# kgutjahr/STiL-TTA

Measured on AMD Instinct MI355X. Metric: training samples/sec (labeled+unlabeled) for DVM STiL, higher is better.
Workload: dtype f32; 1 GPU; config_dvm_STiL ResNet-50 + Transformer tabular, B=256/GPU (32 l + 224 u), 224px + 64 cols, K=286, pseudo-label phase, MI dropout on; global_batch=256, parallelism=dp1, precision=fp32-exact MFMA, launch=eager, split_k=True, input=resident in HBM

## Files before the change

### stil_tta_amd/_lib.py

```python
from __future__ import annotations

import ctypes
import os
import re
import subprocess

_HERE = os.path.dirname(os.path.abspath(__file__))
_ROOT = os.path.dirname(_HERE)
HEADER = os.path.join(_ROOT, "include", "stil_hip.h")
TTA_HEADERS = tuple(os.path.join(_ROOT, "include", f"stil_{n}.h") for n in ("tta", "eata", "bnprior", "infomax", "margent", "deyo", "sar"))
MEMORY_HEADERS = (os.path.join(_HERE, "csrc", "stil_bnmemory.h"),)
READ_HEADERS = (os.path.join(_HERE, "csrc", "stil_read.h"),)
CGPL_HEADERS = (os.path.join(_HERE, "csrc", "stil_cgpl.h"),)
SHIFT_HEADERS = (os.path.join(_HERE, "csrc", "stil_shift.h"),)
ROID_HEADERS = (os.path.join(_HERE, "csrc", "stil_roid.h"),)
ROTTA_HEADERS = (os.path.join(_HERE, "csrc", "stil_rotta.h"),)
LAME_HEADERS = (os.path.join(_HERE, "csrc", "stil_lame.h"),)
LIB_PATH = os.environ.get("STIL_LIB_PATH") or os.path.join(_HERE, "lib", "libstil_hip.so")
CSRC = os.path.join(_HERE, "csrc")

_CTYPES = {
    "int": ctypes.c_int, "long": ctypes.c_long, "long long": ctypes.c_longlong,
    "unsigned long long": ctypes.c_ulonglong, "float": ctypes.c_float, "double": ctypes.c_double,
    "size_t": ctypes.c_size_t,
}


def parse_header(path: str = HEADER):
    src = open(path).read()
    src = re.sub(r"/\*.*?\*/", "", src, flags=re.S)
    protos = {}
    for m in re.finditer(r"(const char\*|int|size_t)\s+(stil_\w+)\s*\(([^)]*)\)\s*;", src):
        ret, name, args = m.group(1), m.group(2), m.group(3)
        restype = {"const char*": ctypes.c_char_p, "int": ctypes.c_int, "size_t": ctypes.c_size_t}[ret]
        argl = []
        args = " ".join(args.split())
        if args and args != "void":
            for a in args.split(","):
                a = a.strip()
                if "*" in a:
                    argl.append((ctypes.c_void_p, a.split("*")[-1].strip()))
                else:
                    toks = a.split()
                    ty = " ".join(toks[:-1])
                    argl.append((_CTYPES[ty], toks[-1]))
        protos[name] = (restype, argl)
    return protos


_HOST_HASHED = ("ops.py", "modules.py", "layouts.py", "stil_model.py", "flat.py", "saint.py")


def source_hash() -> str:
    import hashlib
    h = hashlib.sha256()
    for f in sorted(os.listdir(CSRC)):
        if f.endswith((".hip", ".h")):
            h.update(f.encode())
            h.update(open(os.path.join(CSRC, f), "rb").read())
    for f in _HOST_HASHED:
        h.update(f.encode())
        h.update(open(os.path.join(_HERE, f), "rb").read())
    return h.hexdigest()[:12]


def build(force: bool = False) -> str:
    srcs = [os.path.join(CSRC, f) for f in os.listdir(CSRC) if f.endswith((".hip", ".h"))]
    if (not force) and os.path.exists(LIB_PATH) and all(os.path.getmtime(LIB_PATH) >= os.path.getmtime(s) for s in srcs):
        return LIB_PATH
    r = subprocess.run(["make", "-C", CSRC] + (["-B"] if force else []), capture_output=True, text=True)
    if r.returncode != 0 or not os.path.exists(LIB_PATH):
        raise RuntimeError("building libstil_hip.so failed:\n" + r.stdout + r.stderr)
    return LIB_PATH


class _Lib:
    def __init__(self):
        if not os.path.exists(LIB_PATH):
            raise RuntimeError(f"{LIB_PATH} is missing: run `python -c 'import __graft_entry__ as g; g.build()'` "
                               f"(or `make -C {CSRC}`) first; there is no fallback path")
        self._dll = ctypes.CDLL(LIB_PATH)
        self.protos = parse_header()
        for header in TTA_HEADERS + MEMORY_HEADERS + READ_HEADERS + CGPL_HEADERS + SHIFT_HEADERS + ROID_HEADERS + ROTTA_HEADERS + LAME_HEADERS:
            self.protos.update(parse_header(header))
        for name, (restype, argl) in self.protos.items():
            fn = getattr(self._dll, name)
            fn.restype = restype
            fn.argtypes = [t for t, _ in argl]
        self._dll.stil_last_error.restype = ctypes.c_char_p
        self._prof = None
        self._prof_single = True
        self._prof_only = None

    def begin_profile(self, single_stream: bool = True, only=None):
        self._prof = []
        self._prof_single = bool(single_stream)
        self._prof_only = None if only is None else frozenset(only)

    def end_profile(self):
        import torch
        torch.cuda.synchronize()
        out = [(name, s.elapsed_time(e), meta) for name, s, e, meta in self._prof]
        self._prof = None
        return out

    def last_error(self) -> str:
        return (self._dll.stil_last_error() or b"").decode()

    def __getattr__(self, name):
        fn = getattr(self._dll, "stil_" + name)
        restype = self.protos["stil_" + name][0]
        if restype is not ctypes.c_int or name in ("version", "device_count", "gemm_nt_variant", "gemm_nt_tile_rows", "gemm_nt_config", "weight_layout_job_bytes", "weight_layout_job_blocks", "gemm_nt_bstats_ok", "gemm_nt_force_splits", "reduce_job_bytes", "wgrad_splits", "colsum_chunks", "wgrad_force_splits", "attention_config", "wgrad_config", "gemm_nt_panel"):
            return fn

        def call(*args, meta=None):
            prof = self.__dict__.get("_prof")
            if prof is not None and (self._prof_only is None or name in self._prof_only):
                import torch
                s, e = torch.cuda.Event(enable_timing=True), torch.cuda.Event(enable_timing=True)
                s.record()
                rc = fn(*args)
                e.record()
                prof.append((name, s, e, meta))
            else:
                rc = fn(*args)
            if rc != 0:
                raise RuntimeError(f"stil_{name} failed ({rc}): {self.last_error()}")
            return rc

        self.__dict__[name] = call
        return call


_lib = None


def lib() -> _Lib:
    global _lib
    if _lib is None:
        _lib = _Lib()
    return _lib
```

### stil_tta_amd/csrc/bn.hip

```cpp
#include "common.h"

static inline int pick_ctile(int C) {
  if (C % 256 == 0) return 256;
  if (C % 128 == 0) return 128;
  if (C % 64 == 0) return 64;
  return 0;
}

__global__ __launch_bounds__(256) void bn_pilot_kernel(const float* __restrict__ x, float* __restrict__ K, int M, int C) {
  __shared__ float sh[8 * 32];
  const int cl = threadIdx.x & 31, lane = threadIdx.x >> 5;
  const int c = blockIdx.x * 32 + cl;
  const int n = M < 256 ? M : 256;
  const long stride = M / n;
  float s = 0.f;
  if (c < C)
    for (int j = lane; j < n; j += 8) s += x[(long)j * stride * C + c];
  sh[lane * 32 + cl] = s;
  __syncthreads();
  if (lane == 0 && c < C) {
    float t = 0.f;
    for (int l = 0; l < 8; ++l) t += sh[l * 32 + cl];
    K[c] = t / (float)n;
  }
}

__global__ __launch_bounds__(256) void bn_stats_partial_kernel(const float* __restrict__ x, const float* __restrict__ Kp,
                                                                float* __restrict__ part,
                                                                int M, int C, int ctile, int rows_per_chunk) {
  __shared__ float sh[2 * 1024];
  const int tpr = ctile >> 2, rpb = 256 / tpr;
  const int tc = threadIdx.x % tpr, rl = threadIdx.x / tpr;
  const int c = blockIdx.x * ctile + tc * 4;
  const int m0 = blockIdx.y * rows_per_chunk, m1 = min(M, m0 + rows_per_chunk);
  const float4 K = *reinterpret_cast<const float4*>(Kp + c);
  float4 s1 = make_float4(0.f, 0.f, 0.f, 0.f), s2 = s1;
  for (int m = m0 + rl; m < m1; m += rpb) {
    float4 v = *reinterpret_cast<const float4*>(x + (long)m * C + c);
    float d;
    d = v.x - K.x; s1.x += d; s2.x += d * d;
    d = v.y - K.y; s1.y += d; s2.y += d * d;
    d = v.z - K.z; s1.z += d; s2.z += d * d;
    d = v.w - K.w; s1.w += d; s2.w += d * d;
  }
  float* a = sh + rl * ctile + tc * 4;
  float* b = sh + 1024 + rl * ctile + tc * 4;
  a[0] = s1.x; a[1] = s1.y; a[2] = s1.z; a[3] = s1.w;
  b[0] = s2.x; b[1] = s2.y; b[2] = s2.z; b[3] = s2.w;
  __syncthreads();
  if (threadIdx.x < ctile) {
    float t1 = 0.f, t2 = 0.f;
    for (int r = 0; r < rpb; ++r) { t1 += sh[r * ctile + threadIdx.x]; t2 += sh[1024 + r * ctile + threadIdx.x]; }
    const int cc = blockIdx.x * ctile + threadIdx.x;
    const int nch = gridDim.y;
    part[(long)blockIdx.y * C + cc] = t1;
    part[(long)(nch + blockIdx.y) * C + cc] = t2;
  }
}

template <class Finish>
__global__ __launch_bounds__(256) void bn_fwd_final_kernel(const float* __restrict__ Kp, const float* __restrict__ part, int nch, int M,
                                                            int C, const Finish fin) {
  __shared__ float sh[2 * 8 * 32];
  int c;
  float tot[2];
  if (!chunk_reduce<8, 2>(part, nch, C, sh, c, tot)) return;
  fin.chunk(c, C, M, Kp[c], tot[0], tot[1]);
}

__device__ __forceinline__ void bn_chunk_moments(float K, float s1, float s2, int M, float& mean, float& var) {
  const float invM = 1.f / (float)M;
  const float d = s1 * invM;
  mean = K + d;
  var = s2 * invM - d * d;
  var = fmaxf(var, 0.f);
}

__device__ __forceinline__ bool bn_tile_sums3(const float* __restrict__ ts, int t0, int t1, int tile_rows, int M, int C, double* sh,
                                              int& c, double& a, double& b, double& d) {
  const int cl = threadIdx.x & 31, lane = threadIdx.x >> 5;
  c = blockIdx.x * 32 + cl;
  double s1 = 0.0, s2 = 0.0, s3 = 0.0;
  if (c < C)
    for (int t = t0 + lane; t < t1; t += 8) {
      const double n = (double)min(tile_rows, M - t * tile_rows);
      const double m = (double)ts[((long)t * 2) * C + c];
      s1 += n * m; s2 += n * m * m; s3 += (double)ts[((long)t * 2 + 1) * C + c];
    }
  sh[lane * 32 + cl] = s1; sh[256 + lane * 32 + cl] = s2; sh[512 + lane * 32 + cl] = s3;
  __syncthreads();
  if (lane != 0 || c >= C) return false;
  a = 0.0; b = 0.0; d = 0.0;
  for (int l = 0; l < 8; ++l) { a += sh[l * 32 + cl]; b += sh[256 + l * 32 + cl]; d += sh[512 + l * 32 + cl]; }
  return true;
}

__global__ __launch_bounds__(256) void bn_tiles_stage1_kernel(const float* __restrict__ ts, int nt, int tile_rows, int M, int C,
                                                                int tiles_per_split, double* __restrict__ part) {
  __shared__ double sh[3 * 8 * 32];
  const int t0 = blockIdx.y * tiles_per_split;
  int c;
  double a, b, d;
  if (!bn_tile_sums3(ts, t0, min(nt, t0 + tiles_per_split), tile_rows, M, C, sh, c, a, b, d)) return;
  const int nsplit = gridDim.y;
  part[((long)0 * nsplit + blockIdx.y) * C + c] = a;
  part[((long)1 * nsplit + blockIdx.y) * C + c] = b;
  part[((long)2 * nsplit + blockIdx.y) * C + c] = d;
}

template <class Finish>
__global__ __launch_bounds__(256) void bn_tiles_stage2_kernel(const double* __restrict__ part, int nsplit, int M, int C, const Finish fin) {
  const int c = blockIdx.x * blockDim.x + threadIdx.x;
  if (c >= C) return;
  double s1 = 0.0, s2 = 0.0, s3 = 0.0;
  for (int k = 0; k < nsplit; ++k) {
    s1 += part[((long)0 * nsplit + k) * C + c]; s2 += part[((long)1 * nsplit + k) * C + c]; s3 += part[((long)2 * nsplit + k) * C + c];
  }
  fin.tiles(c, C, M, s1, s2, s3);
}

template <class Finish>
__global__ __launch_bounds__(256) void bn_tiles_fused_kernel(const float* __restrict__ ts, int nt, int tile_rows, int M, int C,
                                                              const Finish fin) {
  __shared__ double sh[3 * 8 * 32];
  int c;
  double a, b, d;
  if (!bn_tile_sums3(ts, 0, nt, tile_rows, M, C, sh, c, a, b, d)) return;
  fin.tiles(c, C, M, a, b, d);
}

__device__ __forceinline__ void bn_tile_moments(double s1, double s2, double s3, int M, double& mean, double& var) {
  mean = s1 / (double)M;
  const double m2 = s3 + (s2 - s1 * mean);
  var = m2 / (double)M;
}

struct BnTrainFwd {
  const float *gamma, *beta;
  float *rmean, *rvar;
  long long* nbt;
  float* stats;
  float eps, momentum;
  __device__ __forceinline__ void write(int c, int C, int M, float mean, float var) const {
    const float g = gamma[c], b = beta[c], rm = rmean ? rmean[c] : 0.f, rv = rmean ? rvar[c] : 0.f;
    if (c == 0 && nbt) *nbt += 1;
    const float rstd = 1.f / sqrtf(var + eps);
    const float a = g * rstd;
    stats[c] = mean; stats[C + c] = rstd; stats[2 * C + c] = a; stats[3 * C + c] = b;
    if (rmean) {
      rmean[c] = (1.f - momentum) * rm + momentum * mean;
      const float unb = (M > 1) ? var * ((float)M / (float)(M - 1)) : var;
      rvar[c] = (1.f - momentum) * rv + momentum * unb;
    }
  }
  __device__ __forceinline__ void chunk(int c, int C, int M, float K, float s1, float s2) const {
    float mean, var;
    bn_chunk_moments(K, s1, s2, M, mean, var);
    write(c, C, M, mean, var);
  }
  __device__ __forceinline__ void tiles(int c, int C, int M, double s1, double s2, double s3) const {
    double mean_d, var_d;
    bn_tile_moments(s1, s2, s3, M, mean_d, var_d);
    write(c, C, M, (float)mean_d, fmaxf((float)var_d, 0.f));
  }
};

__global__ void bn_eval_affine_kernel(const float* __restrict__ gamma, const float* __restrict__ beta,
                                      const float* __restrict__ rmean, const float* __restrict__ rvar,
                                      float* __restrict__ ab, int C, float eps) {
  int c = blockIdx.x * blockDim.x + threadIdx.x;
  if (c >= C) return;
  float a = gamma[c] / sqrtf(rvar[c] + eps);
  ab[c] = a; ab[C + c] = beta[c]; ab[2 * C + c] = rmean[c];
}

__global__ __launch_bounds__(256) void bn_apply_kernel(const float* __restrict__ x, const float* __restrict__ stats,
                                                        const float* __restrict__ resid, const float* __restrict__ rstats,
                                                        float* __restrict__ z, long total4, int C, int relu) {
  const float* A = stats + 2 * C;
  const float* B = stats + 3 * C;
  for (long i = (long)blockIdx.x * blockDim.x + threadIdx.x; i < total4; i += (long)gridDim.x * blockDim.x) {
    const int c = (int)((i * 4) % C);
    float4 v = reinterpret_cast<const float4*>(x)[i];
    const float4 a = *reinterpret_cast<const float4*>(A + c);
    const float4 b = *reinterpret_cast<const float4*>(B + c);
    const float4 mu = *reinterpret_cast<const float4*>(stats + c);
    v.x = (v.x - mu.x) * a.x + b.x; v.y = (v.y - mu.y) * a.y + b.y; v.z = (v.z - mu.z) * a.z + b.z; v.w = (v.w - mu.w) * a.w + b.w;
    if (resid) {
      float4 r = reinterpret_cast<const float4*>(resid)[i];
      if (rstats) {
        const float4 rm = *reinterpret_cast<const float4*>(rstats + c);
        const float4 ra = *reinterpret_cast<const float4*>(rstats + 2 * C + c);
        const float4 rb = *reinterpret_cast<const float4*>(rstats + 3 * C + c);
        r.x = (r.x - rm.x) * ra.x + rb.x; r.y = (r.y - rm.y) * ra.y + rb.y; r.z = (r.z - rm.z) * ra.z + rb.z; r.w = (r.w - rm.w) * ra.w + rb.w;
      }
      v.x += r.x; v.y += r.y; v.z += r.z; v.w += r.w;
    }
    if (relu) { v.x = fmaxf(v.x, 0.f); v.y = fmaxf(v.y, 0.f); v.z = fmaxf(v.z, 0.f); v.w = fmaxf(v.w, 0.f); }
    reinterpret_cast<float4*>(z)[i] = v;
  }
}

__global__ __launch_bounds__(256) void bn_bwd_partial_kernel(const float* __restrict__ dz, const float* __restrict__ z,
                                                              const float* __restrict__ x, const float* __restrict__ stats,
                                                              float* __restrict__ gout, float* __restrict__ part, int M,
                                                              int C, int ctile, int rows_per_chunk, int relu) {
  __shared__ float sh[2 * 1024];
  const int tpr = ctile >> 2, rpb = 256 / tpr;
  const int tc = threadIdx.x % tpr, rl = threadIdx.x / tpr;
  const int c = blockIdx.x * ctile + tc * 4;
  const int m0 = blockIdx.y * rows_per_chunk, m1 = min(M, m0 + rows_per_chunk);
  const float4 mu = *reinterpret_cast<const float4*>(stats + c);
  const float4 rs = *reinterpret_cast<const float4*>(stats + C + c);
  const float4 ap = *reinterpret_cast<const float4*>(stats + 2 * C + c);
  const float4 bp = *reinterpret_cast<const float4*>(stats + 3 * C + c);
  float4 s1 = make_float4(0.f, 0.f, 0.f, 0.f), s2 = s1;
  for (int m = m0 + rl; m < m1; m += rpb) {
    const long o = (long)m * C + c;
    float4 g = *reinterpret_cast<const float4*>(dz + o);
    const float4 v = *reinterpret_cast<const float4*>(x + o);
    if (relu == 1) {
      const float4 zz = *reinterpret_cast<const float4*>(z + o);
      g.x = zz.x > 0.f ? g.x : 0.f; g.y = zz.y > 0.f ? g.y : 0.f;
      g.z = zz.z > 0.f ? g.z : 0.f; g.w = zz.w > 0.f ? g.w : 0.f;
    } else if (relu == 2) {
      g.x = ((v.x - mu.x) * ap.x + bp.x) > 0.f ? g.x : 0.f; g.y = ((v.y - mu.y) * ap.y + bp.y) > 0.f ? g.y : 0.f;
      g.z = ((v.z - mu.z) * ap.z + bp.z) > 0.f ? g.z : 0.f; g.w = ((v.w - mu.w) * ap.w + bp.w) > 0.f ? g.w : 0.f;
    }
    if (gout) *reinterpret_cast<float4*>(gout + o) = g;
    s1.x += g.x; s2.x += g.x * ((v.x - mu.x) * rs.x);
    s1.y += g.y; s2.y += g.y * ((v.y - mu.y) * rs.y);
    s1.z += g.z; s2.z += g.z * ((v.z - mu.z) * rs.z);
    s1.w += g.w; s2.w += g.w * ((v.w - mu.w) * rs.w);
  }
  float* a = sh + rl * ctile + tc * 4;
  float* b = sh + 1024 + rl * ctile + tc * 4;
  a[0] = s1.x; a[1] = s1.y; a[2] = s1.z; a[3] = s1.w;
  b[0] = s2.x; b[1] = s2.y; b[2] = s2.z; b[3] = s2.w;
  __syncthreads();
  if (threadIdx.x < ctile) {
    float t1 = 0.f, t2 = 0.f;
    for (int r = 0; r < rpb; ++r) { t1 += sh[r * ctile + threadIdx.x]; t2 += sh[1024 + r * ctile + threadIdx.x]; }
    const int cc = blockIdx.x * ctile + threadIdx.x;
    const int nch = gridDim.y;
    part[(long)blockIdx.y * C + cc] = t1;
    part[(long)(nch + blockIdx.y) * C + cc] = t2;
  }
}

template <class Finish>
__global__ __launch_bounds__(256) void bn_bwd_final_kernel(const float* __restrict__ part, int nch, int M, int C, const Finish fin) {
  __shared__ float sh[2 * 8 * 32];
  int c;
  float tot[2];
  if (!chunk_reduce<8, 2>(part, nch, C, sh, c, tot)) return;
  fin(c, C, M, tot[0], tot[1]);
}

template <class Finish>
__global__ __launch_bounds__(256) void bn_bwd_final4_kernel(const float* __restrict__ part, int nch, int M, int C, const Finish fin) {
  __shared__ float4 sh[2 * 32 * 8];
  const int cq = threadIdx.x & 7, lane = threadIdx.x >> 3;
  const int c = (blockIdx.x * 8 + cq) * 4;
  float4 a = make_float4(0.f, 0.f, 0.f, 0.f), b = a;
  if (c < C)
    for (int i = lane; i < nch; i += 32) {
      const float4 u = *reinterpret_cast<const float4*>(part + (long)i * C + c);
      const float4 v = *reinterpret_cast<const float4*>(part + (long)(nch + i) * C + c);
      a.x += u.x; a.y += u.y; a.z += u.z; a.w += u.w;
      b.x += v.x; b.y += v.y; b.z += v.z; b.w += v.w;
    }
  sh[lane * 8 + cq] = a; sh[256 + lane * 8 + cq] = b;
  __syncthreads();
  if (lane != 0 || c >= C) return;
  for (int l = 1; l < 32; ++l) {
    const float4 u = sh[l * 8 + cq], v = sh[256 + l * 8 + cq];
    a.x += u.x; a.y += u.y; a.z += u.z; a.w += u.w;
    b.x += v.x; b.y += v.y; b.z += v.z; b.w += v.w;
  }
  const float s1[4] = {a.x, a.y, a.z, a.w}, s2[4] = {b.x, b.y, b.z, b.w};
#pragma unroll
  for (int j = 0; j < 4; ++j) fin(c + j, C, M, s1[j], s2[j]);
}

__device__ __forceinline__ bool bn_tile_sums2(const float* __restrict__ ts, int t0, int t1, int C, double* sh, int& c, double& a,
                                              double& b) {
  const int cl = threadIdx.x & 31, lane = threadIdx.x >> 5;
  c = blockIdx.x * 32 + cl;
  double s1 = 0.0, s2 = 0.0;
  if (c < C)
    for (int t = t0 + lane; t < t1; t += 8) {
      s1 += (double)ts[((long)t * 2) * C + c];
      s2 += (double)ts[((long)t * 2 + 1) * C + c];
    }
  sh[lane * 32 + cl] = s1; sh[256 + lane * 32 + cl] = s2;
  __syncthreads();
  if (lane != 0 || c >= C) return false;
  a = 0.0; b = 0.0;
  for (int l = 0; l < 8; ++l) { a += sh[l * 32 + cl]; b += sh[256 + l * 32 + cl]; }
  return true;
}

__global__ __launch_bounds__(256) void bn_bwd_tiles_stage1_kernel(const float* __restrict__ ts, int nt, int C, int tiles_per_split,
                                                                   double* __restrict__ part) {
  __shared__ double sh[2 * 8 * 32];
  const int t0 = blockIdx.y * tiles_per_split;
  int c;
  double a, b;
  if (!bn_tile_sums2(ts, t0, min(nt, t0 + tiles_per_split), C, sh, c, a, b)) return;
  const int nsplit = gridDim.y;
  part[((long)0 * nsplit + blockIdx.y) * C + c] = a;
  part[((long)1 * nsplit + blockIdx.y) * C + c] = b;
}

template <class Finish>
__global__ __launch_bounds__(256) void bn_bwd_tiles_final_kernel(const double* __restrict__ part, int nsplit, int M, int C,
                                                                  const Finish fin) {
  const int c = blockIdx.x * blockDim.x + threadIdx.x;
  if (c >= C) return;
  double a = 0.0, b = 0.0;
  for (int k = 0; k < nsplit; ++k) { a += part[((long)0 * nsplit + k) * C + c]; b += part[((long)1 * nsplit + k) * C + c]; }
  fin(c, C, M, (float)a, (float)b);
}

template <class Finish>
__global__ __launch_bounds__(256) void bn_bwd_tiles_fused_kernel(const float* __restrict__ ts, int nt, int M, int C, const Finish fin) {
  __shared__ double sh[2 * 8 * 32];
  int c;
  double a, b;
  if (!bn_tile_sums2(ts, 0, nt, C, sh, c, a, b)) return;
  fin(c, C, M, (float)a, (float)b);
}

struct BnTrainBwd {
  const float *gamma, *stats;
  float *dgamma, *dbeta, *coef;
  int accumulate;
  __device__ __forceinline__ void operator()(int c, int C, int M, float s1, float s2) const {
    const float g = gamma[c], rstd = stats[C + c];
    const float b0 = (accumulate && dbeta) ? dbeta[c] : 0.f, g0 = (accumulate && dgamma) ? dgamma[c] : 0.f;
    if (dbeta) dbeta[c] = accumulate ? b0 + s1 : s1;
    if (dgamma) dgamma[c] = accumulate ? g0 + s2 : s2;
    const float invM = 1.f / (float)M;
    coef[c] = g * rstd;
    coef[C + c] = s1 * invM;
    coef[2 * C + c] = s2 * invM;
  }
};

__global__ __launch_bounds__(256) void bn_bwd_dx_kernel(const float* __restrict__ dz, const float* __restrict__ z,
                                                         const float* __restrict__ x, const float* __restrict__ stats,
                                                         const float* __restrict__ coef, float* __restrict__ dx,
                                                         long total4, int C, int relu) {
  for (long i = (long)blockIdx.x * blockDim.x + threadIdx.x; i < total4; i += (long)gridDim.x * blockDim.x) {
    const int c = (int)((i * 4) % C);
    float4 g = reinterpret_cast<const float4*>(dz)[i];
    const float4 v = reinterpret_cast<const float4*>(x)[i];
    const float4 mu = *reinterpret_cast<const float4*>(stats + c);
    if (relu == 1) {
      const float4 zz = reinterpret_cast<const float4*>(z)[i];
      g.x = zz.x > 0.f ? g.x : 0.f; g.y = zz.y > 0.f ? g.y : 0.f;
      g.z = zz.z > 0.f ? g.z : 0.f; g.w = zz.w > 0.f ? g.w : 0.f;
    } else if (relu == 2) {
      const float4 ap = *reinterpret_cast<const float4*>(stats + 2 * C + c);
      const float4 bp = *reinterpret_cast<const float4*>(stats + 3 * C + c);
      g.x = ((v.x - mu.x) * ap.x + bp.x) > 0.f ? g.x : 0.f; g.y = ((v.y - mu.y) * ap.y + bp.y) > 0.f ? g.y : 0.f;
      g.z = ((v.z - mu.z) * ap.z + bp.z) > 0.f ? g.z : 0.f; g.w = ((v.w - mu.w) * ap.w + bp.w) > 0.f ? g.w : 0.f;
    }
    const float4 rs = *reinterpret_cast<const float4*>(stats + C + c);
    const float4 k1 = *reinterpret_cast<const float4*>(coef + c);
    const float4 k2 = *reinterpret_cast<const float4*>(coef + C + c);
    const float4 k3 = *reinterpret_cast<const float4*>(coef + 2 * C + c);
    float4 o;
    o.x = k1.x * (g.x - k2.x - (v.x - mu.x) * rs.x * k3.x);
    o.y = k1.y * (g.y - k2.y - (v.y - mu.y) * rs.y * k3.y);
    o.z = k1.z * (g.z - k2.z - (v.z - mu.z) * rs.z * k3.z);
    o.w = k1.w * (g.w - k2.w - (v.w - mu.w) * rs.w * k3.w);
    reinterpret_cast<float4*>(dx)[i] = o;
  }
}

__global__ __launch_bounds__(256) void maxpool_fwd_kernel(const float* __restrict__ x, float* __restrict__ y, unsigned char* __restrict__ idx,
                                                           int N, int H, int W, int C, int OH, int OW) {
  const int C4 = C >> 2;
  const long total = (long)N * OH * OW * C4;
  for (long i = (long)blockIdx.x * blockDim.x + threadIdx.x; i < total; i += (long)gridDim.x * blockDim.x) {
    const int c = (int)(i % C4) * 4;
    long t = i / C4;
    const int ox = (int)(t % OW); t /= OW;
    const int oy = (int)(t % OH);
    const int n = (int)(t / OH);
    float4 best = make_float4(-INFINITY, -INFINITY, -INFINITY, -INFINITY);
    const int first = (oy == 0 ? 3 : 0) + (ox == 0 ? 1 : 0);
    int b0 = first, b1 = first, b2 = first, b3 = first;
#pragma unroll
    for (int ky = 0; ky < 3; ++ky) {
      const int iy = oy * 2 - 1 + ky;
      if (iy < 0 || iy >= H) continue;
#pragma unroll
      for (int kx = 0; kx < 3; ++kx) {
        const int ix = ox * 2 - 1 + kx;
        if (ix < 0 || ix >= W) continue;
        const float4 v = *reinterpret_cast<const float4*>(x + ((long)(n * H + iy) * W + ix) * C + c);
        const int tap = ky * 3 + kx;
        if (v.x > best.x || v.x != v.x) { best.x = v.x; b0 = tap; }
        if (v.y > best.y || v.y != v.y) { best.y = v.y; b1 = tap; }
        if (v.z > best.z || v.z != v.z) { best.z = v.z; b2 = tap; }
        if (v.w > best.w || v.w != v.w) { best.w = v.w; b3 = tap; }
      }
    }
    const long o = ((long)(n * OH + oy) * OW + ox) * C + c;
    *reinterpret_cast<float4*>(y + o) = best;
    *reinterpret_cast<uchar4*>(idx + o) = make_uchar4((unsigned char)b0, (unsigned char)b1, (unsigned char)b2, (unsigned char)b3);
  }
}

__global__ __launch_bounds__(256) void maxpool_bwd_kernel(const float* __restrict__ dy, const unsigned char* __restrict__ idx,
                                                           float* __restrict__ dx, int N, int H, int W, int C, int OH, int OW) {
  const int C4 = C >> 2;
  const long total = (long)N * H * W * C4;
  for (long i = (long)blockIdx.x * blockDim.x + threadIdx.x; i < total; i += (long)gridDim.x * blockDim.x) {
    const int c = (int)(i % C4) * 4;
    long t = i / C4;
    const int ix = (int)(t % W); t /= W;
    const int iy = (int)(t % H);
    const int n = (int)(t / H);
    float4 s = make_float4(0.f, 0.f, 0.f, 0.f);
    for (int oy = iy / 2; oy <= (iy + 1) / 2; ++oy) {
      if (oy < 0 || oy >= OH) continue;
      const int ky = iy - (oy * 2 - 1);
      if (ky < 0 || ky > 2) continue;
      for (int ox = ix / 2; ox <= (ix + 1) / 2; ++ox) {
        if (ox < 0 || ox >= OW) continue;
        const int kx = ix - (ox * 2 - 1);
        if (kx < 0 || kx > 2) continue;
        const long o = ((long)(n * OH + oy) * OW + ox) * C + c;
        const uchar4 k = *reinterpret_cast<const uchar4*>(idx + o);
        const float4 g = *reinterpret_cast<const float4*>(dy + o);
        const int tap = ky * 3 + kx;
        if (k.x == tap) s.x += g.x;
        if (k.y == tap) s.y += g.y;
        if (k.z == tap) s.z += g.z;
        if (k.w == tap) s.w += g.w;
      }
    }
    *reinterpret_cast<float4*>(dx + ((long)(n * H + iy) * W + ix) * C + c) = s;
  }
}

__global__ __launch_bounds__(256) void im2col_nchw_kernel(const float* __restrict__ x, float* __restrict__ col, int N, int Cin,
                                                           int H, int W, int OH, int OW, int KH, int KW, int stride, int pad,
                                                           int Kp, int rows_per_block) {
  extern __shared__ int ktab[];
  const int K = Cin * KH * KW, Q = Kp >> 2;
  for (int k = threadIdx.x; k < Kp; k += blockDim.x) {
    int v = -1;
    if (k < K) {
      const int c = k / (KH * KW), r = k - c * KH * KW, ky = r / KW, kx = r - ky * KW;
      v = ((c * KH + ky) << 8) | kx;
    }
    ktab[k] = v;
  }
  __syncthreads();
  const long M = (long)N * OH * OW;
  const long m0 = (long)blockIdx.x * rows_per_block;
  const int quads = rows_per_block * Q;
  for (int i = threadIdx.x; i < quads; i += blockDim.x) {
    const int rr = i / Q, q = i - rr * Q;
    const long m = m0 + rr;
    if (m >= M) break;
    const int ox = (int)(m % OW);
    const long t = m / OW;
    const int oy = (int)(t % OH), n = (int)(t / OH);
    const int iy0 = oy * stride - pad, ix0 = ox * stride - pad;
    float v[4];
#pragma unroll
    for (int j = 0; j < 4; ++j) {
      const int e = ktab[q * 4 + j];
      v[j] = 0.f;
      if (e >= 0) {
        const int cky = e >> 8, kx = e & 255, c = cky / KH, ky = cky - c * KH;
        const int iy = iy0 + ky, ix = ix0 + kx;
        if (iy >= 0 && iy < H && ix >= 0 && ix < W) v[j] = x[((long)(n * Cin + c) * H + iy) * W + ix];
      }
    }
    *reinterpret_cast<float4*>(col + m * Kp + q * 4) = make_float4(v[0], v[1], v[2], v[3]);
  }
}

static inline int bn_chunks(int M, int C, int ctile) {
  int colblocks = C / ctile;
  int want = cdiv(1024, colblocks);
  int maxc = cdiv(M, 64);
  int n = want < maxc ? want : maxc;
  return n < 1 ? 1 : n;
}

extern "C" size_t stil_bn_workspace_bytes(int M, int C) {
  int ct = pick_ctile(C);
  if (!ct) return 0;
  return ((size_t)2 * bn_chunks(M, C, ct) + 1) * C * sizeof(float);
}

static inline int bn_tiles_nsplit(int nt) { return cdiv(nt, 256); }
extern "C" size_t stil_bn_tiles_workspace_bytes(int M, int C, int tile_rows) {
  if (M <= 0 || C <= 0 || tile_rows <= 0) return 0;
  return (size_t)3 * bn_tiles_nsplit(cdiv(M, tile_rows)) * C * sizeof(double);
}
extern "C" size_t stil_bn_bwd_tiles_workspace_bytes(int ntiles, int C) {
  if (ntiles <= 0 || C <= 0) return 0;
  return (size_t)2 * bn_tiles_nsplit(ntiles) * C * sizeof(double);
}

static inline int bn_wide_grid(int M, int C, long* total4) {
  *total4 = (long)M * C / 4;
  const long blocks = (*total4 + 255) / 256;
  return (int)(blocks < 8192 ? blocks : 8192);
}

template <class Finish>
static int bn_fwd_two_pass(const char* who, const Finish& fin, const float* x, const float* resid, float* z, const float* stats, int M,
                           int C, int relu, float* workspace, size_t workspace_bytes, hipStream_t s, bool final_only = false) {
  const int ct = pick_ctile(C);
  STIL_REQUIRE(ct != 0, "%s: C=%d must be a multiple of 64", who, C);
  const int nch = bn_chunks(M, C, ct);
  STIL_REQUIRE(workspace_bytes >= ((size_t)2 * nch + 1) * C * sizeof(float), "%s: workspace too small", who);
  float* pilot = workspace + (size_t)2 * nch * C;
  if (!final_only) {
    hipLaunchKernelGGL(bn_pilot_kernel, dim3(cdiv(C, 32)), dim3(256), 0, s, x, pilot, M, C);
    STIL_LAUNCH_CHECK();
    hipLaunchKernelGGL(bn_stats_partial_kernel, dim3(C / ct, nch), dim3(256), 0, s, x, pilot, workspace, M, C, ct, cdiv(M, nch));
    STIL_LAUNCH_CHECK();
  }
  hipLaunchKernelGGL(bn_fwd_final_kernel<Finish>, dim3(cdiv(C, 32)), dim3(256), 0, s, pilot, workspace, nch, M, C, fin);
  STIL_LAUNCH_CHECK();
  if (final_only) return STIL_OK;
  long total4;
  const int grid = bn_wide_grid(M, C, &total4);
  hipLaunchKernelGGL(bn_apply_kernel, dim3(grid), dim3(256), 0, s, x, stats, resid, (const float*)nullptr, z, total4, C, relu);
  STIL_LAUNCH_CHECK();
  return STIL_OK;
}

template <class Finish>
static int bn_fwd_tiles(const char* who, const Finish& fin, const float* x, const float* tilestats, int tile_rows, const float* resid,
                        const float* resid_stats, float* z, const float* stats, int M, int C, int relu, void* workspace,
                        size_t workspace_bytes, hipStream_t s, bool final_only = false) {
  STIL_REQUIRE(z || !resid, "%s: statistics-only call (z == NULL) cannot take a residual", who);
  STIL_REQUIRE(!resid_stats || resid, "%s: resid_stats without resid", who);
  STIL_REQUIRE(tile_rows > 0 && M > 0 && C > 0 && C % 4 == 0, "%s: bad shape M=%d C=%d tile_rows=%d", who, M, C, tile_rows);
  STIL_REQUIRE(workspace_bytes >= stil_bn_tiles_workspace_bytes(M, C, tile_rows) && ((uintptr_t)workspace % 8) == 0,
               "%s: workspace too small or not 8-byte aligned", who);
  const int nt = cdiv(M, tile_rows), nsplit = bn_tiles_nsplit(nt);
  if (nsplit == 1) {
    hipLaunchKernelGGL(bn_tiles_fused_kernel<Finish>, dim3(cdiv(C, 32)), dim3(256), 0, s, tilestats, nt, tile_rows, M, C, fin);
    STIL_LAUNCH_CHECK();
  } else {
    if (!final_only) {
      hipLaunchKernelGGL(bn_tiles_stage1_kernel, dim3(cdiv(C, 32), nsplit), dim3(256), 0, s, tilestats, nt, tile_rows, M, C,
                         cdiv(nt, nsplit), (double*)workspace);
      STIL_LAUNCH_CHECK();
    }
    hipLaunchKernelGGL(bn_tiles_stage2_kernel<Finish>, dim3(cdiv(C, 256)), dim3(256), 0, s, (const double*)workspace, nsplit, M, C, fin);
    STIL_LAUNCH_CHECK();
  }
  if (!z || final_only) return STIL_OK;
  long total4;
  const int grid = bn_wide_grid(M, C, &total4);
  hipLaunchKernelGGL(bn_apply_kernel, dim3(grid), dim3(256), 0, s, x, stats, resid, resid_stats, z, total4, C, relu);
  STIL_LAUNCH_CHECK();
  return STIL_OK;
}

template <class Finish>
static int bn_bwd_two_pass(const char* who, const Finish& fin, const float* dz, const float* z, const float* x, const float* stats,
                           const float* coef, float* dx, float* gout, int M, int C, int relu, float* workspace, size_t workspace_bytes,
                           hipStream_t s) {
  STIL_REQUIRE(relu >= 0 && relu <= 2 && (relu != 1 || z), "%s: relu must be 0, 1 (needs z) or 2", who);
  const int ct = pick_ctile(C);
  STIL_REQUIRE(ct != 0, "%s: C=%d must be a multiple of 64", who, C);
  const int nch = bn_chunks(M, C, ct);
  STIL_REQUIRE(workspace_bytes >= (size_t)2 * nch * C * sizeof(float), "%s: workspace too small", who);
  hipLaunchKernelGGL(bn_bwd_partial_kernel, dim3(C / ct, nch), dim3(256), 0, s, dz, z, x, stats, gout, workspace, M, C, ct,
                     cdiv(M, nch), relu);
  STIL_LAUNCH_CHECK();
  if (((uintptr_t)workspace % 16) == 0)
    hipLaunchKernelGGL(bn_bwd_final4_kernel<Finish>, dim3(cdiv(C, 32)), dim3(256), 0, s, workspace, nch, M, C, fin);
  else
    hipLaunchKernelGGL(bn_bwd_final_kernel<Finish>, dim3(cdiv(C, 32)), dim3(256), 0, s, workspace, nch, M, C, fin);
  STIL_LAUNCH_CHECK();
  long total4;
  const int grid = bn_wide_grid(M, C, &total4);
  hipLaunchKernelGGL(bn_bwd_dx_kernel, dim3(grid), dim3(256), 0, s, gout ? gout : dz, z, x, stats, coef, dx, total4, C, gout ? 0 : relu);
  STIL_LAUNCH_CHECK();
  return STIL_OK;
}

template <class Finish>
static int bn_bwd_tiles(const char* who, const Finish& fin, const float* dz, const float* z, const float* x, const float* stats,
                        const float* tilestats, int ntiles, const float* coef, float* dx, int M, int C, int relu, void* workspace,
                        size_t workspace_bytes, hipStream_t s) {
  STIL_REQUIRE(relu >= 0 && relu <= 2 && (relu != 1 || z), "%s: relu must be 0, 1 (needs z) or 2", who);
  STIL_REQUIRE(ntiles > 0 && M > 0 && C > 0 && C % 4 == 0, "%s: bad shape M=%d C=%d ntiles=%d", who, M, C, ntiles);
  STIL_REQUIRE(workspace_bytes >= stil_bn_bwd_tiles_workspace_bytes(ntiles, C) && ((uintptr_t)workspace % 8) == 0,
               "%s: workspace too small or not 8-byte aligned", who);
  const int nsplit = bn_tiles_nsplit(ntiles);
  if (nsplit == 1) {
    hipLaunchKernelGGL(bn_bwd_tiles_fused_kernel<Finish>, dim3(cdiv(C, 32)), dim3(256), 0, s, tilestats, ntiles, M, C, fin);
    STIL_LAUNCH_CHECK();
  } else {
    hipLaunchKernelGGL(bn_bwd_tiles_stage1_kernel, dim3(cdiv(C, 32), nsplit), dim3(256), 0, s, tilestats, ntiles, C, cdiv(ntiles, nsplit),
                       (double*)workspace);
    STIL_LAUNCH_CHECK();
    hipLaunchKernelGGL(bn_bwd_tiles_final_kernel<Finish>, dim3(cdiv(C, 256)), dim3(256), 0, s, (const double*)workspace, nsplit, M, C, fin);
    STIL_LAUNCH_CHECK();
  }
  long total4;
  const int grid = bn_wide_grid(M, C, &total4);
  hipLaunchKernelGGL(bn_bwd_dx_kernel, dim3(grid), dim3(256), 0, s, dz, z, x, stats, coef, dx, total4, C, relu);
  STIL_LAUNCH_CHECK();
  return STIL_OK;
}

extern "C" int stil_bn_train_fwd(const float* x, const float* gamma, const float* beta, float* running_mean,
                                 float* running_var, long long* num_batches_tracked, const float* resid, float* z,
                                 float* stats, int M, int C, int relu, float eps, float momentum, float* workspace,
                                 size_t workspace_bytes, void* stream) {
  STIL_REQUIRE(x && gamma && beta && z && stats && workspace, "stil_bn_train_fwd: null pointer");
  const BnTrainFwd fin{gamma, beta, running_mean, running_var, num_batches_tracked, stats, eps, momentum};
  return bn_fwd_two_pass("stil_bn_train_fwd", fin, x, resid, z, stats, M, C, relu, workspace, workspace_bytes, (hipStream_t)stream);
}

extern "C" int stil_bn_eval_affine(const float* gamma, const float* beta, const float* running_mean,
                                   const float* running_var, float* ab, int C, float eps, void* stream) {
  STIL_REQUIRE(gamma && beta && running_mean && running_var && ab, "stil_bn_eval_affine: null pointer");
  hipLaunchKernelGGL(bn_eval_affine_kernel, dim3(cdiv(C, 64)), dim3(64), 0, (hipStream_t)stream, gamma, beta,
                     running_mean, running_var, ab, C, eps);
  STIL_LAUNCH_CHECK();
  return STIL_OK;
}

extern "C" int stil_bn_train_fwd_tiles(const float* x, const float* tilestats, int tile_rows, const float* gamma, const float* beta,
                                       float* running_mean, float* running_var, long long* num_batches_tracked,
                                       const float* resid, const float* resid_stats, float* z, float* stats, int M, int C, int relu,
                                       float eps, float momentum, void* workspace, size_t workspace_bytes, void* stream) {
  STIL_REQUIRE(x && tilestats && gamma && beta && stats && workspace, "stil_bn_train_fwd_tiles: null pointer");
  const BnTrainFwd fin{gamma, beta, running_mean, running_var, num_batches_tracked, stats, eps, momentum};
  return bn_fwd_tiles("stil_bn_train_fwd_tiles", fin, x, tilestats, tile_rows, resid, resid_stats, z, stats, M, C, relu, workspace,
                      workspace_bytes, (hipStream_t)stream);
}

extern "C" int stil_bn_train_bwd(const float* dz, const float* z, const float* x, const float* gamma,
                                 const float* stats, float* dx, float* gout, float* dgamma, float* dbeta, float* coef,
                                 int M, int C, int relu, int accumulate, float* workspace, size_t workspace_bytes,
                                 void* stream) {
  STIL_REQUIRE(dz && x && gamma && stats && dx && coef && workspace, "stil_bn_train_bwd: null pointer");
  const BnTrainBwd fin{gamma, stats, dgamma, dbeta, coef, accumulate};
  return bn_bwd_two_pass("stil_bn_train_bwd", fin, dz, z, x, stats, coef, dx, gout, M, C, relu, workspace, workspace_bytes,
                         (hipStream_t)stream);
}

extern "C" int stil_bn_train_bwd_tiles(const float* dz, const float* z, const float* x, const float* gamma, const float* stats,
                                       const float* tilestats, int ntiles, float* dx, float* dgamma, float* dbeta, float* coef,
                                       int M, int C, int relu, int accumulate, void* workspace, size_t workspace_bytes, void* stream) {
  STIL_REQUIRE(dz && x && gamma && stats && tilestats && dx && coef && workspace, "stil_bn_train_bwd_tiles: null pointer");
  const BnTrainBwd fin{gamma, stats, dgamma, dbeta, coef, accumulate};
  return bn_bwd_tiles("stil_bn_train_bwd_tiles", fin, dz, z, x, stats, tilestats, ntiles, coef, dx, M, C, relu, workspace, workspace_bytes,
                      (hipStream_t)stream);
}

extern "C" int stil_maxpool3x3s2_fwd(const float* x, float* y, unsigned char* idx, int N, int H, int W, int C, int OH,
                                     int OW, void* stream) {
  STIL_REQUIRE(x && y && idx, "stil_maxpool3x3s2_fwd: null pointer");
  STIL_REQUIRE(OH == (H + 2 - 3) / 2 + 1 && OW == (W + 2 - 3) / 2 + 1, "stil_maxpool3x3s2_fwd: bad output dims");
  STIL_REQUIRE(C % 4 == 0, "stil_maxpool3x3s2_fwd: C=%d must be a multiple of 4", C);
  long total = (long)N * OH * OW * C / 4;
  int grid = (int)((total + 255) / 256 < 16384 ? (total + 255) / 256 : 16384);
  hipLaunchKernelGGL(maxpool_fwd_kernel, dim3(grid), dim3(256), 0, (hipStream_t)stream, x, y, idx, N, H, W, C, OH, OW);
  STIL_LAUNCH_CHECK();
  return STIL_OK;
}

extern "C" int stil_maxpool3x3s2_bwd(const float* dy, const unsigned char* idx, float* dx, int N, int H, int W, int C,
                                     int OH, int OW, void* stream) {
  STIL_REQUIRE(dy && idx && dx, "stil_maxpool3x3s2_bwd: null pointer");
  STIL_REQUIRE(C % 4 == 0, "stil_maxpool3x3s2_bwd: C=%d must be a multiple of 4", C);
  long total = (long)N * H * W * C / 4;
  int grid = (int)((total + 255) / 256 < 16384 ? (total + 255) / 256 : 16384);
  hipLaunchKernelGGL(maxpool_bwd_kernel, dim3(grid), dim3(256), 0, (hipStream_t)stream, dy, idx, dx, N, H, W, C, OH, OW);
  STIL_LAUNCH_CHECK();
  return STIL_OK;
}

extern "C" int stil_im2col_nchw(const float* x, float* col, int N, int Cin, int H, int W, int OH, int OW, int KH,
                                int KW, int stride, int pad, int Kp, void* stream) {
  STIL_REQUIRE(x && col && Kp >= Cin * KH * KW, "stil_im2col_nchw: null pointer or Kp too small");
  STIL_REQUIRE(Kp % 4 == 0 && Kp <= 4096 && KW < 256 && ((uintptr_t)col % 16) == 0, "stil_im2col_nchw: Kp=%d must be a multiple of 4 (<= 4096), KW < 256, col 16-byte aligned", Kp);
  const long M = (long)N * OH * OW;
  const int rpb = 32;
  hipLaunchKernelGGL(im2col_nchw_kernel, dim3(cdiv(M, rpb)), dim3(256), Kp * sizeof(int), (hipStream_t)stream, x, col, N, Cin, H, W,
                     OH, OW, KH, KW, stride, pad, Kp, rpb);
  STIL_LAUNCH_CHECK();
  return STIL_OK;
}
```

### stil_tta_amd/csrc/gemm.hip

```cpp
#include "common.h"
#include <type_traits>

typedef float f32x16 __attribute__((ext_vector_type(16)));
typedef __bf16 bf16x8 __attribute__((ext_vector_type(8)));
typedef __bf16 bf16x4 __attribute__((ext_vector_type(4)));

__device__ __forceinline__ void split3(float a, __bf16& a1, __bf16& a2, __bf16& a3) {
  a1 = (__bf16)a;
  const float r1 = a - (float)a1;
  a2 = (__bf16)r1;
  const float r2 = r1 - (float)a2;
  a3 = (__bf16)r2;
}

struct ConvGeom {
  int H, W, C;
  int OH, OW;
  int KH, KW, stride, pad_y, pad_x;
  int mode;
};

struct GemmNTArgs {
  const float* A;
  const float* Bw;
  float* C;
  int M, N, K;
  int lda, ldb, ldc;
  ConvGeom g;
  const float* bias;
  const float* sub;
  const float* scale;
  const float* var;
  float var_eps;
  const float* shift;
  const float* resid;
  int ldr;
  float* pre;
  int act;
  float alpha;
  int vecA, vecB;
  int os, opy, opx, oOH, oOW;
  float* colstats;
  const float* abn;
  const float* rmask;
  int ldm;
  int wide;
  const float* bs_y;
  const float* bs_stats;
  float* bstats;
  int ldbs, bs_relu, bs_tile0;
  int splits;
  float* split_slabs;
  int* split_tickets;
  int panel;
};

__device__ __forceinline__ float4 ld4_guard(const float* p, int nvalid, int vec) {
  float4 v = make_float4(0.f, 0.f, 0.f, 0.f);
  if (nvalid >= 4 && vec) {
    v = *reinterpret_cast<const float4*>(p);
  } else {
    if (nvalid > 0) v.x = p[0];
    if (nvalid > 1) v.y = p[1];
    if (nvalid > 2) v.z = p[2];
    if (nvalid > 3) v.w = p[3];
  }
  return v;
}

__device__ __forceinline__ int xcd_remap(int bid, int nwg) {
  int xcd = bid & 7, q = nwg >> 3, r = nwg & 7;
  return (xcd < r ? xcd * (q + 1) : r * (q + 1) + (xcd - r) * q) + (bid >> 3);
}

__device__ __forceinline__ float4 ld4_sel(const float* p, const float* safe, bool ok) {
  const float4 v = *reinterpret_cast<const float4*>(ok ? p : safe);
  return ok ? v : make_float4(0.f, 0.f, 0.f, 0.f);
}

template <int TM, int TN, bool PLAIN>
__device__ __forceinline__ void gemm_nt_epilogue(const GemmNTArgs& p, f32x16 (&acc)[TM][TN], float* red, int tm, int tn, int wm, int wn,
                                                 int li, int lh) {
  constexpr int BM = 64 * TM, BN = 64 * TN;
  const ConvGeom& g = p.g;
  if (p.colstats) {
    const int rows_valid = min(BM, p.M - tm * BM);
    float mean_t[TN];
#pragma unroll
    for (int j = 0; j < TN; ++j) {
      float sacc = 0.f;
#pragma unroll
      for (int i = 0; i < TM; ++i)
#pragma unroll
        for (int r = 0; r < 16; ++r) {
          const int row_m = tm * BM + wm * TM * 32 + i * 32 + (r & 3) + 8 * (r >> 2) + 4 * lh;
          if (row_m < p.M) sacc += acc[i][j][r] * p.alpha;
        }
      sacc += __shfl_xor(sacc, 32, 64);
      if (lh == 0) red[wm * BN + wn * TN * 32 + j * 32 + li] = sacc;
    }
    __syncthreads();
#pragma unroll
    for (int j = 0; j < TN; ++j) {
      const int cs = wn * TN * 32 + j * 32 + li;
      mean_t[j] = (red[cs] + red[BN + cs]) / (float)rows_valid;
    }
    __syncthreads();
#pragma unroll
    for (int j = 0; j < TN; ++j) {
      float q = 0.f;
#pragma unroll
      for (int i = 0; i < TM; ++i)
#pragma unroll
        for (int r = 0; r < 16; ++r) {
          const int row_m = tm * BM + wm * TM * 32 + i * 32 + (r & 3) + 8 * (r >> 2) + 4 * lh;
          const float d = acc[i][j][r] * p.alpha - mean_t[j];
          if (row_m < p.M) q += d * d;
        }
      q += __shfl_xor(q, 32, 64);
      if (lh == 0) red[wm * BN + wn * TN * 32 + j * 32 + li] = q;
    }
    __syncthreads();
    if (wm == 0 && lh == 0) {
#pragma unroll
      for (int j = 0; j < TN; ++j) {
        const int cs = wn * TN * 32 + j * 32 + li, col = tn * BN + cs;
        if (col < p.N) {
          p.colstats[((long)tm * 2) * p.N + col] = mean_t[j];
          p.colstats[((long)tm * 2 + 1) * p.N + col] = red[cs] + red[BN + cs];
        }
      }
    }
  }

  if constexpr (TM == 1 && TN == 1) {
    if (p.wide) {
      constexpr int TS = BN + 4;
      float* T = red;
      __syncthreads();
#pragma unroll
      for (int r = 0; r < 16; ++r)
        T[(wm * 32 + (r & 3) + 8 * (r >> 2) + 4 * lh) * TS + wn * 32 + li] = acc[0][0][r];
      __syncthreads();
      const int tid = threadIdx.x, cq = (tid & 15) * 4, col = tn * BN + cq;
      if (col < p.N) {
        const float4 zero4 = make_float4(0.f, 0.f, 0.f, 0.f), one4 = make_float4(1.f, 1.f, 1.f, 1.f);
        const float4 bia = p.bias ? *reinterpret_cast<const float4*>(p.bias + col) : zero4;
        const float4 sb = p.sub ? *reinterpret_cast<const float4*>(p.sub + col) : zero4;
        float4 sc = p.scale ? *reinterpret_cast<const float4*>(p.scale + col) : one4;
        if (p.var) {
          const float4 vv = *reinterpret_cast<const float4*>(p.var + col);
          sc.x = sc.x / sqrtf(vv.x + p.var_eps); sc.y = sc.y / sqrtf(vv.y + p.var_eps);
          sc.z = sc.z / sqrtf(vv.z + p.var_eps); sc.w = sc.w / sqrtf(vv.w + p.var_eps);
        }
        const float4 sh = p.shift ? *reinterpret_cast<const float4*>(p.shift + col) : zero4;
#pragma unroll
        for (int ps = 0; ps < 4; ++ps) {
          const int rl = ps * 16 + (tid >> 4), row_m = tm * BM + rl;
          if (row_m >= p.M) continue;
          long row = row_m;
          if (!PLAIN && p.os != 1) {
            const int ohw = g.OH * g.OW;
            const int n = row_m / ohw, rem = row_m - n * ohw;
            const int oy = rem / g.OW, ox = rem - oy * g.OW;
            row = ((long)n * p.oOH + oy * p.os + p.opy) * p.oOW + ox * p.os + p.opx;
          }
          float4 v = *reinterpret_cast<const float4*>(T + rl * TS + cq);
          v.x *= p.alpha; v.y *= p.alpha; v.z *= p.alpha; v.w *= p.alpha;
          v.x = (v.x - sb.x) * sc.x + sh.x + bia.x; v.y = (v.y - sb.y) * sc.y + sh.y + bia.y;
          v.z = (v.z - sb.z) * sc.z + sh.z + bia.z; v.w = (v.w - sb.w) * sc.w + sh.w + bia.w;
          if (p.resid) {
            const float4 rr = *reinterpret_cast<const float4*>(p.resid + row * p.ldr + col);
            v.x += rr.x; v.y += rr.y; v.z += rr.z; v.w += rr.w;
          }
          if (p.pre) *reinterpret_cast<float4*>(p.pre + row * p.ldc + col) = v;
          if (p.act == 1) { v.x = fmaxf(v.x, 0.f); v.y = fmaxf(v.y, 0.f); v.z = fmaxf(v.z, 0.f); v.w = fmaxf(v.w, 0.f); }
          else if (p.act == 2) { v.x = gelu_f(v.x); v.y = gelu_f(v.y); v.z = gelu_f(v.z); v.w = gelu_f(v.w); }
          if (p.rmask) {
            const float4 mk = *reinterpret_cast<const float4*>(p.rmask + row * p.ldm + col);
            v.x = mk.x > 0.f ? v.x : 0.f; v.y = mk.y > 0.f ? v.y : 0.f; v.z = mk.z > 0.f ? v.z : 0.f; v.w = mk.w > 0.f ? v.w : 0.f;
          }
          *reinterpret_cast<float4*>(p.C + row * p.ldc + col) = v;
          if (p.bstats) *reinterpret_cast<float4*>(T + rl * TS + cq) = v;
        }
      }
      if (p.bstats) {
        float4 bs1 = make_float4(0.f, 0.f, 0.f, 0.f), bs2 = bs1;
        if (col < p.N) {
          const float4 bmu = *reinterpret_cast<const float4*>(p.bs_stats + col);
          const float4 brs = *reinterpret_cast<const float4*>(p.bs_stats + p.N + col);
          const float4 bap = *reinterpret_cast<const float4*>(p.bs_stats + 2 * p.N + col);
          const float4 bbp = *reinterpret_cast<const float4*>(p.bs_stats + 3 * p.N + col);
#pragma unroll
          for (int ps = 0; ps < 4; ++ps) {
            const int rl = ps * 16 + (tid >> 4), row_m = tm * BM + rl;
            if (row_m >= p.M) continue;
            long row = row_m;
            if (!PLAIN && p.os != 1) {
              const int ohw = g.OH * g.OW;
              const int n = row_m / ohw, rem = row_m - n * ohw;
              const int oy = rem / g.OW, ox = rem - oy * g.OW;
              row = ((long)n * p.oOH + oy * p.os + p.opy) * p.oOW + ox * p.os + p.opx;
            }
            const float4 yy = *reinterpret_cast<const float4*>(p.bs_y + row * p.ldbs + col);
            float4 gg = *reinterpret_cast<const float4*>(T + rl * TS + cq);
            if (p.bs_relu == 2) {
              gg.x = ((yy.x - bmu.x) * bap.x + bbp.x) > 0.f ? gg.x : 0.f; gg.y = ((yy.y - bmu.y) * bap.y + bbp.y) > 0.f ? gg.y : 0.f;
              gg.z = ((yy.z - bmu.z) * bap.z + bbp.z) > 0.f ? gg.z : 0.f; gg.w = ((yy.w - bmu.w) * bap.w + bbp.w) > 0.f ? gg.w : 0.f;
            }
            bs1.x += gg.x; bs2.x += gg.x * ((yy.x - bmu.x) * brs.x);
            bs1.y += gg.y; bs2.y += gg.y * ((yy.y - bmu.y) * brs.y);
            bs1.z += gg.z; bs2.z += gg.z * ((yy.z - bmu.z) * brs.z);
            bs1.w += gg.w; bs2.w += gg.w * ((yy.w - bmu.w) * brs.w);
          }
        }
        __syncthreads();
        float* R1 = red;
        float* R2 = red + 16 * 64;
        const int rt = tid >> 4;
        *reinterpret_cast<float4*>(R1 + rt * 64 + cq) = bs1;
        *reinterpret_cast<float4*>(R2 + rt * 64 + cq) = bs2;
        __syncthreads();
        if (tid < 128) {
          const int c = tid & 63, which = tid >> 6, gc = tn * BN + c;
          const float* R = which ? R2 : R1;
          float t = 0.f;
#pragma unroll
          for (int r = 0; r < 16; ++r) t += R[r * 64 + c];
          if (gc < p.N) p.bstats[((long)(p.bs_tile0 + tm) * 2 + which) * p.N + gc] = t;
        }
      }
      return;
    }
  }

#pragma unroll
  for (int j = 0; j < TN; ++j) {
    const int col = tn * BN + wn * TN * 32 + j * 32 + li;
    if (col >= p.N) continue;
    const float bia = p.bias ? p.bias[col] : 0.f;
    const float sb = p.sub ? p.sub[col] : 0.f;
    float sc = p.scale ? p.scale[col] : 1.f;
    if (p.var) sc = sc / sqrtf(p.var[col] + p.var_eps);
    const float sh = p.shift ? p.shift[col] : 0.f;
#pragma unroll
    for (int i = 0; i < TM; ++i) {
#pragma unroll
      for (int r = 0; r < 16; ++r) {
        const int row_m = tm * BM + wm * TM * 32 + i * 32 + (r & 3) + 8 * (r >> 2) + 4 * lh;
        if (row_m >= p.M) continue;
        long row = row_m;
        if (!PLAIN && p.os != 1) {
          const int ohw = g.OH * g.OW;
          const int n = row_m / ohw, rem = row_m - n * ohw;
          const int oy = rem / g.OW, ox = rem - oy * g.OW;
          row = ((long)n * p.oOH + oy * p.os + p.opy) * p.oOW + ox * p.os + p.opx;
        }
        float v = acc[i][j][r] * p.alpha;
        v = (v - sb) * sc + sh + bia;
        if (p.resid) v += p.resid[row * p.ldr + col];
        if (p.pre) p.pre[row * p.ldc + col] = v;
        if (p.act == 1) v = fmaxf(v, 0.f);
        else if (p.act == 2) v = gelu_f(v);
        if (p.rmask) v = p.rmask[row * p.ldm + col] > 0.f ? v : 0.f;
        p.C[row * p.ldc + col] = v;
      }
    }
  }
}

template <int TM, int TN, int BK, bool VEC, bool ACC2 = false, bool PLAIN = false, bool BNA = false, int NB = 2, bool B3 = false>
__global__ __launch_bounds__(256) __attribute__((amdgpu_waves_per_eu(B3 ? (PLAIN ? 4 : 3) : (((BK == 16 || NB == 1) && VEC) ? (TM * TN == 1 ? ((NB == 1 && ACC2) ? 4 : ((BNA && ACC2 && !PLAIN) ? 5 : 6)) : ((TM * TN == 2 && ACC2 && (PLAIN || TN == 2)) ? 4 : 1)) : 1))))
void gemm_nt_kernel(GemmNTArgs p) {
  static_assert(!B3 || (BK == 32 && NB == 1 && VEC && ACC2), "the bf16x3 mode runs 32-deep k-tiles in one LDS buffer with two-level sums");
  constexpr int BM = 64 * TM, BN = 64 * TN, LS = BK + 4;
  constexpr int KQ = BK / 4, RP = 256 / KQ;
  constexpr int RA = BM / RP, RB = BN / RP;
  constexpr int LSB = 40;
  extern __shared__ __attribute__((aligned(16))) float lds[];
  float* As = lds;
  float* Bs = lds + NB * BM * LS;
  float* tab = B3 ? lds + 3 * (BM + BN) * LSB / 2 : lds + NB * (BM + BN) * LS;
  __bf16* Ap3 = reinterpret_cast<__bf16*>(lds);
  __bf16* Bp3 = Ap3 + 3 * BM * LSB;

  const int nbn = (p.N + BN - 1) / BN, nbm = (p.M + BM - 1) / BM;
  int wg = xcd_remap(blockIdx.x, nbm * nbn * (TM * TN == 1 ? p.splits : 1));
  int split = 0;
  if constexpr (TM * TN == 1) {
    if (p.splits > 1) { split = wg % p.splits; wg /= p.splits; }
  }
  int tm = wg / nbn, tn = wg - tm * nbn;
  if (p.panel > 0) {
    const int per_panel = nbm * p.panel;
    const int pn = wg / per_panel, rem = wg - pn * per_panel;
    tm = rem / p.panel;
    tn = pn * p.panel + (rem - tm * p.panel);
  }
  const int tid = threadIdx.x, kq = tid % KQ, r0 = tid / KQ;
  const ConvGeom g = p.g;

  int a_n[RA], a_oy[RA], a_ox[RA];
  bool a_ok[RA];
#pragma unroll
  for (int i = 0; i < RA; ++i) {
    int m = tm * BM + r0 + RP * i;
    a_ok[i] = m < p.M;
    if constexpr (PLAIN) {
      a_n[i] = a_ok[i] ? m : 0; a_oy[i] = 0; a_ox[i] = 0;
    } else {
      int mm = a_ok[i] ? m : 0;
      int ohw = g.OH * g.OW;
      int n = mm / ohw, rem = mm - n * ohw;
      int oy = rem / g.OW;
      a_n[i] = n; a_oy[i] = oy; a_ox[i] = rem - oy * g.OW;
    }
  }
  const float* b_ptr[RB];
  bool b_ok[RB];
#pragma unroll
  for (int i = 0; i < RB; ++i) {
    int n = tn * BN + r0 + RP * i;
    b_ok[i] = n < p.N;
    b_ptr[i] = p.Bw + (long)(b_ok[i] ? n : 0) * p.ldb + kq * 4;
  }

  float4 ra[RA], rb[RB];
  const float* a_src[RA];
  bool a_val[RA];
  bool ra_ok[RA];
  int ra_c = 0;
  if constexpr (BNA) {
    const int C = p.g.C;
    for (int i = threadIdx.x; i < 3 * C; i += 256) {
      const int r = i / C, c = i - r * C;
      tab[i] = p.abn[(r == 0 ? 0 : r + 1) * C + c];
    }
    __syncthreads();
  }
  auto set_tap = [&](int tap) {
    if constexpr (PLAIN) {
#pragma unroll
      for (int i = 0; i < RA; ++i) {
        a_val[i] = a_ok[i];
        a_src[i] = p.A + (long)a_n[i] * p.lda + kq * 4;
      }
      return;
    }
    const int ky = tap / g.KW, kx = tap - ky * g.KW;
#pragma unroll
    for (int i = 0; i < RA; ++i) {
      int iy, ix;
      bool ok = a_ok[i];
      if (g.mode == 0) {
        iy = a_oy[i] * g.stride - g.pad_y + ky;
        ix = a_ox[i] * g.stride - g.pad_x + kx;
      } else {
        int ty = a_oy[i] + g.pad_y - ky, tx = a_ox[i] + g.pad_x - kx;
        ok = ok && ty >= 0 && tx >= 0;
        iy = ty / g.stride; ix = tx / g.stride;
        ok = ok && (iy * g.stride == ty) && (ix * g.stride == tx);
      }
      ok = ok && iy >= 0 && iy < g.H && ix >= 0 && ix < g.W;
      a_val[i] = ok;
      a_src[i] = ok ? p.A + ((long)(a_n[i] * g.H + iy) * g.W + ix) * p.lda + kq * 4 : p.A;
    }
  };
  const int per_tap = (g.C + BK - 1) / BK;
  const int nk_all = (PLAIN ? 1 : g.KH * g.KW) * per_tap;
  int kt0 = 0, nk = nk_all;
  if constexpr (TM * TN == 1) {
    if (p.splits > 1) {
      int kpt = (nk_all + p.splits - 1) / p.splits;
      kpt = ((kpt + 64 / BK - 1) / (64 / BK)) * (64 / BK);
      kt0 = min(nk_all, split * kpt);
      nk = min(nk_all, kt0 + kpt) - kt0;
    }
  }
  int cur_tap = kt0 / per_tap, c0 = (kt0 - cur_tap * per_tap) * BK, kb = cur_tap * g.C + c0;
  const int ntaps = PLAIN ? 1 : g.KH * g.KW;
  set_tap(cur_tap < ntaps ? cur_tap : 0);
  auto gload = [&]() {
    const int nval = g.C - (c0 + kq * 4);
    if constexpr (BNA) ra_c = c0 + kq * 4;
#pragma unroll
    for (int i = 0; i < RA; ++i) {
      if (VEC) ra[i] = ld4_sel(a_src[i] + c0, p.A, a_val[i] && nval > 0);
      else ra[i] = a_val[i] ? ld4_guard(a_src[i] + c0, nval, 0) : make_float4(0.f, 0.f, 0.f, 0.f);
      if constexpr (BNA) ra_ok[i] = a_val[i] && nval > 0;
    }
#pragma unroll
    for (int i = 0; i < RB; ++i) {
      if (VEC) rb[i] = ld4_sel(b_ptr[i] + kb, p.Bw, b_ok[i] && nval > 0);
      else rb[i] = b_ok[i] ? ld4_guard(b_ptr[i] + kb, nval, 0) : make_float4(0.f, 0.f, 0.f, 0.f);
    }
    c0 += BK; kb += BK;
    if (c0 >= g.C) {
      kb += g.C - c0;
      c0 = 0;
      if (++cur_tap < ntaps) set_tap(cur_tap);
    }
  };
  auto lstore = [&](int buf) {
    if constexpr (BNA) {
      const int C = p.g.C;
      const float4 mu = *reinterpret_cast<const float4*>(tab + ra_c);
      const float4 aa = *reinterpret_cast<const float4*>(tab + C + ra_c);
      const float4 bb = *reinterpret_cast<const float4*>(tab + 2 * C + ra_c);
#pragma unroll
      for (int i = 0; i < RA; ++i) {
        float4 v = ra[i];
        v.x = (v.x - mu.x) * aa.x + bb.x; v.y = (v.y - mu.y) * aa.y + bb.y; v.z = (v.z - mu.z) * aa.z + bb.z; v.w = (v.w - mu.w) * aa.w + bb.w;
        v.x = fmaxf(v.x, 0.f); v.y = fmaxf(v.y, 0.f); v.z = fmaxf(v.z, 0.f); v.w = fmaxf(v.w, 0.f);
        ra[i] = ra_ok[i] ? v : make_float4(0.f, 0.f, 0.f, 0.f);
      }
    }
    if constexpr (B3) {
#pragma unroll
      for (int i = 0; i < RA + RB; ++i) {
        const float4 v = i < RA ? ra[i < RA ? i : 0] : rb[i < RA ? 0 : i - RA];
        const float e[4] = {v.x, v.y, v.z, v.w};
        bf16x4 h1, h2, h3;
#pragma unroll
        for (int q = 0; q < 4; ++q) { __bf16 a1, a2, a3; split3(e[q], a1, a2, a3); h1[q] = a1; h2[q] = a2; h3[q] = a3; }
        __bf16* dst = (i < RA ? Ap3 + (r0 + RP * i) * LSB : Bp3 + (r0 + RP * (i - RA)) * LSB) + kq * 4;
        constexpr int PLA = BM * LSB, PLB = BN * LSB;
        const int PL = i < RA ? PLA : PLB;
        *reinterpret_cast<bf16x4*>(dst) = h1; *reinterpret_cast<bf16x4*>(dst + PL) = h2; *reinterpret_cast<bf16x4*>(dst + 2 * PL) = h3;
      }
      return;
    }
#pragma unroll
    for (int i = 0; i < RA; ++i)
      *reinterpret_cast<float4*>(&As[buf * BM * LS + (r0 + RP * i) * LS + kq * 4]) = ra[i];
#pragma unroll
    for (int i = 0; i < RB; ++i)
      *reinterpret_cast<float4*>(&Bs[buf * BN * LS + (r0 + RP * i) * LS + kq * 4]) = rb[i];
  };

  const int w = tid >> 6, wm = w >> 1, wn = w & 1, lane = tid & 63, li = lane & 31, lh = lane >> 5;
  f32x16 acc[TM][TN];
#pragma unroll
  for (int i = 0; i < TM; ++i)
#pragma unroll
    for (int j = 0; j < TN; ++j)
#pragma unroll
      for (int r = 0; r < 16; ++r) acc[i][j][r] = 0.f;
  constexpr int FLUSH = 64 / BK;

  const bool tap_inside = PLAIN || (g.pad_y == 0 && g.pad_x == 0 && (g.OH - 1) * g.stride < g.H && (g.OW - 1) * g.stride < g.W);
  const bool full = VEC && ntaps == 1 && (PLAIN || g.mode == 0) && tap_inside && (g.C % BK == 0) && (tm + 1) * BM <= p.M && (tn + 1) * BN <= p.N;
  auto mainloop = [&](auto full_tag) {
    constexpr bool FULL = decltype(full_tag)::value;
    auto load = [&]() {
      if constexpr (FULL) {
        if constexpr (BNA) {
          ra_c = c0 + kq * 4;
#pragma unroll
          for (int i = 0; i < RA; ++i) ra_ok[i] = true;
        }
#pragma unroll
        for (int i = 0; i < RA; ++i) ra[i] = *reinterpret_cast<const float4*>(a_src[i] + c0);
#pragma unroll
        for (int i = 0; i < RB; ++i) rb[i] = *reinterpret_cast<const float4*>(b_ptr[i] + c0);
        c0 += BK;
      } else {
        gload();
      }
    };
    auto compute = [&](int buf, f32x16 (&c)[TM][TN], auto fresh_tag) {
      constexpr bool FRESH = decltype(fresh_tag)::value;
      if constexpr (B3) {
        const __bf16* Ab3 = Ap3 + (wm * TM * 32 + li) * LSB + lh * 8;
        const __bf16* Bb3 = Bp3 + (wn * TN * 32 + li) * LSB + lh * 8;
#pragma unroll
        for (int s_ = 0; s_ < 2; ++s_) {
          bf16x8 a[3][TM], b[3][TN];
#pragma unroll
          for (int pl = 0; pl < 3; ++pl) {
#pragma unroll
            for (int i = 0; i < TM; ++i) a[pl][i] = *reinterpret_cast<const bf16x8*>(Ab3 + pl * BM * LSB + i * 32 * LSB + s_ * 16);
// ... 535 lines not shown
__global__ void wgrad_reduce_kernel(const float* __restrict__ P, float* __restrict__ dW, int splits, int N, int K,
                                    int Cin, int taps, int Kdst, int accumulate) {
  long idx = (long)blockIdx.x * blockDim.x + threadIdx.x;
  long total = (long)N * K;
  if (idx >= total) return;
  int n = (int)(idx / K), k = (int)(idx - (long)n * K);
  float s = 0.f;
  for (int zz = 0; zz < splits; ++zz) s += P[(long)zz * total + idx];
  int dst;
  if (taps > 1) {
    int tap = k / Cin, c = k - tap * Cin;
    dst = c * taps + tap;
  } else {
    dst = k;
  }
  if (dst >= Kdst) return;
  long o = (long)n * Kdst + dst;
  dW[o] = accumulate ? dW[o] + s : s;
}
__global__ __launch_bounds__(256) void wgrad_reduce4_kernel(const float* __restrict__ P, float* __restrict__ dW, int splits, int N, int K,
                                                             int Cin, int taps, int Kdst, int accumulate) {
  __shared__ float4 sh[8 * 32];
  const int ql = threadIdx.x & 31, l = threadIdx.x >> 5;
  const long total = (long)N * K;
  const long idx = ((long)blockIdx.x * 32 + ql) * 4;
  float4 s = make_float4(0.f, 0.f, 0.f, 0.f);
  if (idx < total)
    for (int zz = l; zz < splits; zz += 8) {
      const float4 v = *reinterpret_cast<const float4*>(P + (long)zz * total + idx);
      s.x += v.x; s.y += v.y; s.z += v.z; s.w += v.w;
    }
  sh[l * 32 + ql] = s;
  __syncthreads();
  if (l != 0 || idx >= total) return;
  for (int j = 1; j < 8; ++j) { const float4 v = sh[j * 32 + ql]; s.x += v.x; s.y += v.y; s.z += v.z; s.w += v.w; }
  const int n = (int)(idx / K), k = (int)(idx - (long)n * K);
  const float sv[4] = {s.x, s.y, s.z, s.w};
  if (taps > 1) {
    const int tap = k / Cin, c = k - tap * Cin;
#pragma unroll
    for (int j = 0; j < 4; ++j) {
      const int dst = (c + j) * taps + tap;
      if (dst < Kdst) { const long o = (long)n * Kdst + dst; dW[o] = accumulate ? dW[o] + sv[j] : sv[j]; }
    }
  } else {
#pragma unroll
    for (int j = 0; j < 4; ++j) {
      const int dst = k + j;
      if (dst < Kdst) { const long o = (long)n * Kdst + dst; dW[o] = accumulate ? dW[o] + sv[j] : sv[j]; }
    }
  }
}

__global__ __launch_bounds__(256) void colsum_partial_kernel(const float* __restrict__ X, float* __restrict__ part, int M, int N, int ld,
                                      int rows_per_chunk) {
  __shared__ float sh[4 * 64];
  const int cl = threadIdx.x & 63, rl = threadIdx.x >> 6;
  const int c = blockIdx.x * 64 + cl;
  const int m0 = blockIdx.y * rows_per_chunk, m1 = min(M, m0 + rows_per_chunk);
  float s0 = 0.f, s1 = 0.f;
  if (c < N) {
    int m = m0 + rl;
    for (; m + 4 < m1; m += 8) { s0 += X[(long)m * ld + c]; s1 += X[(long)(m + 4) * ld + c]; }
    for (; m < m1; m += 4) s0 += X[(long)m * ld + c];
  }
  sh[rl * 64 + cl] = s0 + s1;
  __syncthreads();
  if (rl == 0 && c < N) part[(long)blockIdx.y * N + c] = sh[cl] + sh[64 + cl] + sh[128 + cl] + sh[192 + cl];
}
__global__ __launch_bounds__(256) void colsum_final_kernel(const float* __restrict__ part, float* __restrict__ out, int nchunks, int N,
                                    int accumulate, float scale) {
  __shared__ float sh[8 * 32];
  int c;
  float tot[1];
  if (!chunk_reduce<8, 1>(part, nchunks, N, sh, c, tot)) return;
  const float s = tot[0] * scale;
  out[c] = accumulate ? out[c] + s : s;
}

#define STIL_REDUCE_BATCH 48
struct ReduceJob {
  const float* P;
  float* dst;
  int splits, N, K, Cin, taps, Kdst, accumulate;
  float scale;
};
struct ReduceBatch {
  int n;
  int first_block[STIL_REDUCE_BATCH + 1];
  ReduceJob job[STIL_REDUCE_BATCH];
};
static inline bool reduce_job_vec(const ReduceJob& j) {
  return j.K % 4 == 0 && (j.taps == 1 || j.Cin % 4 == 0) && ((uintptr_t)j.P % 16) == 0;
}
static inline int reduce_job_blocks(const ReduceJob& j) {
  const long total = (long)j.N * j.K;
  return reduce_job_vec(j) ? cdiv(total / 4, 256) : cdiv(total, 256);
}
__global__ __launch_bounds__(256) void reduce_jobs_kernel(ReduceBatch b) {
  int ji = 0;
  while (ji + 1 < b.n && (int)blockIdx.x >= b.first_block[ji + 1]) ++ji;
  const ReduceJob& j = b.job[ji];
  const int lb = blockIdx.x - b.first_block[ji];
  const long total = (long)j.N * j.K;
  const bool vec = j.K % 4 == 0 && (j.taps == 1 || j.Cin % 4 == 0) && ((uintptr_t)j.P % 16) == 0;
  if (vec) {
    const long idx = ((long)lb * 256 + threadIdx.x) * 4;
    if (idx >= total) return;
    float4 t[8];
#pragma unroll
    for (int l = 0; l < 8; ++l) t[l] = make_float4(0.f, 0.f, 0.f, 0.f);
    const float* src = j.P + idx;
    int zz = 0;
    for (; zz + 8 <= j.splits; zz += 8) {
#pragma unroll
      for (int l = 0; l < 8; ++l) {
        const float4 v = *reinterpret_cast<const float4*>(src + (long)(zz + l) * total);
        t[l].x += v.x; t[l].y += v.y; t[l].z += v.z; t[l].w += v.w;
      }
    }
#pragma unroll
    for (int l = 0; l < 8; ++l)
      if (zz + l < j.splits) {
        const float4 v = *reinterpret_cast<const float4*>(src + (long)(zz + l) * total);
        t[l].x += v.x; t[l].y += v.y; t[l].z += v.z; t[l].w += v.w;
      }
    float4 s = t[0];
#pragma unroll
    for (int q = 1; q < 8; ++q) { s.x += t[q].x; s.y += t[q].y; s.z += t[q].z; s.w += t[q].w; }
    const int n = (int)(idx / j.K), k = (int)(idx - (long)n * j.K);
    const float sv[4] = {s.x * j.scale, s.y * j.scale, s.z * j.scale, s.w * j.scale};
    if (j.taps == 1 && k + 3 < j.Kdst && j.Kdst % 4 == 0 && ((uintptr_t)j.dst % 16) == 0) {
      float4* o = reinterpret_cast<float4*>(j.dst + (long)n * j.Kdst + k);
      float4 r = make_float4(sv[0], sv[1], sv[2], sv[3]);
      if (j.accumulate) { const float4 c = *o; r.x = c.x + sv[0]; r.y = c.y + sv[1]; r.z = c.z + sv[2]; r.w = c.w + sv[3]; }
      *o = r;
      return;
    }
#pragma unroll
    for (int e = 0; e < 4; ++e) {
      int dst = k + e;
      if (j.taps > 1) { const int tap = k / j.Cin, c = k - tap * j.Cin; dst = (c + e) * j.taps + tap; }
      if (dst < j.Kdst) { const long o = (long)n * j.Kdst + dst; j.dst[o] = j.accumulate ? j.dst[o] + sv[e] : sv[e]; }
    }
  } else {
    const long idx = (long)lb * 256 + threadIdx.x;
    if (idx >= total) return;
    const int n = (int)(idx / j.K), k = (int)(idx - (long)n * j.K);
    float s = 0.f;
    for (int zz = 0; zz < j.splits; ++zz) s += j.P[(long)zz * total + idx];
    s *= j.scale;
    int dst = k;
    if (j.taps > 1) { const int tap = k / j.Cin, c = k - tap * j.Cin; dst = c * j.taps + tap; }
    if (dst >= j.Kdst) return;
    const long o = (long)n * j.Kdst + dst;
    j.dst[o] = j.accumulate ? j.dst[o] + s : s;
  }
}
extern "C" int stil_reduce_job_bytes(void) { return (int)sizeof(ReduceJob); }
extern "C" int stil_reduce_jobs(const void* jobs_host, int njobs, void* stream) {
  STIL_REQUIRE(jobs_host && njobs > 0, "stil_reduce_jobs: null pointer or no jobs");
  const ReduceJob* jobs = (const ReduceJob*)jobs_host;
  for (int j0 = 0; j0 < njobs; j0 += STIL_REDUCE_BATCH) {
    ReduceBatch b;
    b.n = njobs - j0 < STIL_REDUCE_BATCH ? njobs - j0 : STIL_REDUCE_BATCH;
    int nb = 0;
    for (int i = 0; i < b.n; ++i) {
      const ReduceJob& j = jobs[j0 + i];
      STIL_REQUIRE(j.P && j.dst && j.splits > 0 && j.N > 0 && j.K > 0 && j.taps > 0 && (j.taps == 1 || j.Cin * j.taps == j.K),
                   "stil_reduce_jobs: bad job %d", j0 + i);
      b.job[i] = j;
      b.first_block[i] = nb;
      nb += reduce_job_blocks(j);
    }
    for (int i = b.n; i <= STIL_REDUCE_BATCH; ++i) b.first_block[i] = nb;
    hipLaunchKernelGGL(reduce_jobs_kernel, dim3(nb), dim3(256), 0, (hipStream_t)stream, b);
    STIL_LAUNCH_CHECK();
  }
  return STIL_OK;
}

static int check_geom(const ConvGeom& g, int vec_required) {
  if (g.KH * g.KW > 1 && (g.C % 16) != 0) {
    stil_set_error("implicit-GEMM conv needs Cin %% 16 == 0 (got %d)", g.C);
    return STIL_EUNSUPPORTED;
  }
  (void)vec_required;
  return STIL_OK;
}

static inline int is_vec(const void* p, int ld) { return (((uintptr_t)p) % 16 == 0) && (ld % 4 == 0); }

static bool g_nt_attr = false;
static int gemm_nt_attr() {
  if (g_nt_attr) return STIL_OK;
  hipError_t e = hipFuncSetAttribute((const void*)gemm_nt_kernel<2, 2, 32, true, false, false>, hipFuncAttributeMaxDynamicSharedMemorySize, 80 * 1024);
  if (e == hipSuccess) e = hipFuncSetAttribute((const void*)gemm_nt_kernel<2, 2, 32, true, true, false>, hipFuncAttributeMaxDynamicSharedMemorySize, 80 * 1024);
  if (e == hipSuccess) e = hipFuncSetAttribute((const void*)gemm_nt_kernel<2, 2, 32, true, false, true>, hipFuncAttributeMaxDynamicSharedMemorySize, 80 * 1024);
  if (e == hipSuccess) e = hipFuncSetAttribute((const void*)gemm_nt_kernel<2, 2, 32, true, true, true>, hipFuncAttributeMaxDynamicSharedMemorySize, 80 * 1024);
  if (e != hipSuccess) { stil_set_error("gemm_nt: hipFuncSetAttribute failed: %s", hipGetErrorString(e)); return STIL_EHIP; }
  g_nt_attr = true;
  return STIL_OK;
}

static bool nt_big_wanted(int M, int N, int K, bool plain, bool vec, int srcC, int tune) {
  static const int env_big = [] { const char* e = getenv("STIL_GEMM_BIG"); return e ? atoi(e) : 0; }();
  static const int env_mink = [] { const char* e = getenv("STIL_GEMM_BIG_MINK"); return e ? atoi(e) : 0; }();
  const int forced = tune % 100;
  if (forced != 44 && !(forced == 0 && env_big > 0)) return false;
  if (!plain || !vec || (M % 128) || (N % 128) || (K % 32) || srcC != K) return false;
  const long tiles = (long)(M / 128) * (N / 128);
  return forced == 44 || (tiles >= env_big && K >= env_mink);
}

extern "C" int stil_gemm_nt_variant(int M, int N, int tune) {
  tune %= 10000;
  const int forced = tune % 100;
  if (forced == 11 || forced == 21 || forced == 22 || forced == 12) return forced;
  (void)M; (void)N;
  return 11;
}

extern "C" int stil_gemm_nt_bstats_ok(const float* C, int N, int ldc, const float* resid, int ldr, const float* relu_mask, int ldm, const float* bs_y) {
  auto al16 = [](const void* q) { return q == nullptr || ((uintptr_t)q % 16) == 0; };
  return (N % 4 == 0) && (ldc % 4 == 0) && (!resid || ldr % 4 == 0) && (!relu_mask || ldm % 4 == 0) && al16(relu_mask) && al16(C) && al16(resid) &&
         al16(bs_y) && bs_y != nullptr ? 1 : 0;
}

extern "C" int stil_gemm_nt_tile_rows(int M, int N, int tune) { const int v = stil_gemm_nt_variant(M, N, tune); return (v == 11 || v == 12) ? 64 : 128; }

static int nt_config(const float* A, const float* W, int M, int N, int K, int lda, int ldb, int srcC, int KH, int KW,
                     int plain, int a_bn, int tune, bool allow_big) {
  const bool want_b3 = tune >= 100000;
  tune %= 10000;
  const int variant = stil_gemm_nt_variant(M, N, tune);
  const int bkd = (tune / 100) % 10;
  const bool bk32 = (bkd == 1 || bkd == 3 || (bkd == 0 && !a_bn)) && (K % 32 == 0) && (KH * KW == 1 || srcC % 32 == 0);
  const bool single = bk32 && (bkd == 3 || bkd == 0);
  const bool acc2 = tune / 1000 == 2 || (tune / 1000 == 0 && K >= 512);
  const bool vec = is_vec(A, lda) && (srcC % 4 == 0) && is_vec(W, ldb) && (K % 4 == 0);
  if (allow_big && !want_b3 && nt_big_wanted(M, N, K, plain && KH * KW == 1, vec, srcC, tune) && (long)cdiv(M, 64) * cdiv(N, 64) >= 256)
    return 44 + 200 + 1000 * (acc2 ? 1 : 0) + 10000 + 100000 + (a_bn ? 1000000 : 0);
  const bool b3 = want_b3 && vec && variant == 11 && K % 32 == 0 && (KH * KW == 1 || srcC % 32 == 0) && (!a_bn || srcC % 32 == 0);
  if (b3)
    return 11 + 200 + 1000 + 10000 + 100000 * ((plain && KH * KW == 1) ? 1 : 0) + (a_bn ? 1000000 : 0) + 10000000;
  if (a_bn)
    return 11 + 1000 * (acc2 ? 1 : 0) + 10000 * (vec ? 1 : 0) + 100000 * ((plain && KH * KW == 1) ? 1 : 0) + 1000000;
  return variant + 100 * ((vec && bk32) ? (single ? 2 : 1) : 0) + 1000 * (acc2 ? 1 : 0) + 10000 * (vec ? 1 : 0) + 100000 * ((plain && KH * KW == 1) ? 1 : 0);
}

extern "C" int stil_gemm_nt_config(const float* A, const float* W, int M, int N, int K, int lda, int ldb, int srcC, int KH, int KW,
                                   int plain, int a_bn, int tune) {
  return nt_config(A, W, M, N, K, lda, ldb, srcC, KH, KW, plain, a_bn, tune, true);
}

#define NT_SPLIT_MAX_TILES 4096
static int g_force_splits = 0;
extern "C" int stil_gemm_nt_force_splits(int s) { const int old = g_force_splits; g_force_splits = s; return old; }
static int nt_splits(int M, int N, int K, int tune) {
  if (stil_gemm_nt_variant(M, N, tune) != 11) return 1;
  const long tiles = (long)cdiv(M, 64) * cdiv(N, 64);
  if (g_force_splits > 0) {
    if (tiles > NT_SPLIT_MAX_TILES || K < 256) return 1;
    int s = g_force_splits;
    if (s > K / 64) s = K / 64;
    return s < 2 ? 1 : s;
  }
  static const int max_tiles = [] { const char* e = getenv("STIL_GEMM_SPLIT_MAXTILES"); return e ? atoi(e) : 1536; }();
  static const int big_target = [] { const char* e = getenv("STIL_GEMM_SPLIT_TARGET"); return e ? atoi(e) : 1536; }();
  if (K < 256 || tiles >= max_tiles) return 1;
  const int kt = K / 32;
  int maxs, target;
  if (tiles < 256) { maxs = kt / 4; target = kt >= 64 ? 1536 : 512; }
  else { if (kt < 36) return 1; maxs = kt / 12; target = big_target; }
  int s = cdiv(target, tiles);
  if (s > maxs) s = maxs;
  if (s > 8) s = 8;
  return s < 2 ? 1 : s;
}
static int nt_panel(int M, int N, int K) {
  static const int forced = [] { const char* e = getenv("STIL_GEMM_PANEL"); return e ? atoi(e) : -1; }();
  const int nbn = cdiv(N, 64);
  int gw = forced;
  if (forced < 0) {
    if (N < 1024 || K > 1024 || (long)N * K * 4 <= (2l << 20)) return 0;
    gw = (int)((1l << 20) / (64l * K * 4));
    if (gw < 4) gw = 4;
  }
  if (gw <= 0 || gw >= nbn) return 0;
  while (gw > 1 && nbn % gw) --gw;
  (void)M;
  return gw > 1 ? gw : 0;
}
extern "C" int stil_gemm_nt_panel(int M, int N, int K) { return nt_panel(M, N, K); }

#define NT_SPLIT_TICKET_BYTES (4 * NT_SPLIT_MAX_TILES)
extern "C" size_t stil_gemm_nt_split_workspace_bytes(int M, int N, int K, int tune) {
  const int s = nt_splits(M, N, K, tune % 10000);
  if (s <= 1) return 0;
  const long tiles = (long)cdiv(M, 64) * cdiv(N, 64);
  return (size_t)NT_SPLIT_TICKET_BYTES + (size_t)tiles * s * 4096 * sizeof(float);
}

extern "C" int stil_gemm_nt(const float* A, const float* W, float* C, int M, int N, int K, int lda, int ldb, int ldc,
                            int srcH, int srcW, int srcC, int OH, int OW, int KH, int KW, int stride, int pad_y,
                            int pad_x, int mode, int out_stride, int out_py, int out_px, int out_OH, int out_OW,
                            const float* bias, const float* sub, const float* scale,
                            const float* shift, const float* resid, int ldr, float* pre, int act, float alpha,
                            float* colstats, const float* a_bn, const float* relu_mask, int ldm,
                            const float* bs_y, const float* bs_stats, float* bstats, int bs_relu, int bs_tile0,
                            const float* scale_var, float var_eps, void* split_ws, size_t split_ws_bytes, int tune_arg, void* stream) {
  const bool want_b3 = tune_arg >= 100000;
  if (want_b3) tune_arg -= 100000;
  const int tune = tune_arg % 10000;
  const bool scalar_epilogue = tune_arg / 10000 == 1;
  STIL_REQUIRE(A && W && C && M > 0 && N > 0 && K > 0, "stil_gemm_nt: null pointer or empty shape (M=%d N=%d K=%d)", M, N, K);
  STIL_REQUIRE(tune_arg >= 0 && tune_arg < 20000 && tune < 3000 && (tune % 100 == 0 || tune % 100 == 11 || tune % 100 == 21 || tune % 100 == 22 || tune % 100 == 12 || tune % 100 == 44) && (tune / 100) % 10 <= 3,
               "stil_gemm_nt: bad tune %d", tune);
  STIL_REQUIRE(KH * KW * srcC == K, "stil_gemm_nt: K=%d != KH*KW*C=%d", K, KH * KW * srcC);
  STIL_REQUIRE(M % (OH * OW) == 0, "stil_gemm_nt: M=%d not a multiple of OH*OW=%d", M, OH * OW);
  GemmNTArgs p;
  p.A = A; p.Bw = W; p.C = C; p.M = M; p.N = N; p.K = K; p.lda = lda; p.ldb = ldb; p.ldc = ldc;
  p.g = ConvGeom{srcH, srcW, srcC, OH, OW, KH, KW, stride, pad_y, pad_x, mode};
  p.os = out_stride < 1 ? 1 : out_stride; p.opy = out_py; p.opx = out_px; p.oOH = out_OH; p.oOW = out_OW;
  p.var = scale_var; p.var_eps = var_eps;
  p.splits = 1; p.split_slabs = nullptr; p.split_tickets = nullptr;
  p.panel = 0;
  {
    const size_t need = stil_gemm_nt_split_workspace_bytes(M, N, K, tune_arg);
    if (split_ws && need > 0 && split_ws_bytes >= need && ((uintptr_t)split_ws % 256) == 0) {
      const long tiles = (long)cdiv(M, 64) * cdiv(N, 64);
      p.splits = nt_splits(M, N, K, tune_arg % 10000);
      p.split_tickets = (int*)split_ws;
      p.split_slabs = (float*)((char*)split_ws + NT_SPLIT_TICKET_BYTES);
      (void)tiles;
    }
  }
  STIL_REQUIRE(!scale_var || scale, "stil_gemm_nt: scale_var divides `scale`, which is missing");
  p.bias = bias; p.sub = sub; p.scale = scale; p.shift = shift; p.resid = resid; p.ldr = ldr; p.pre = pre; p.act = act;
  p.alpha = alpha;
  p.colstats = colstats;
  p.abn = a_bn;
  p.rmask = relu_mask; p.ldm = ldm;
  STIL_REQUIRE(!relu_mask || !colstats, "stil_gemm_nt: relu_mask and colstats exclude each other");
  {
    auto al16 = [](const void* q) { return q == nullptr || ((uintptr_t)q % 16) == 0; };
    p.wide = (N % 4 == 0) && (ldc % 4 == 0) && (!resid || ldr % 4 == 0) && (!relu_mask || ldm % 4 == 0) && al16(relu_mask) && al16(C) && al16(resid) && al16(pre) && al16(bias) && al16(sub) &&
             al16(scale) && al16(scale_var) && al16(shift) && !scalar_epilogue ? 1 : 0;
  }
  p.bs_y = bs_y; p.bs_stats = bs_stats; p.bstats = bstats; p.ldbs = ldc; p.bs_relu = bs_relu; p.bs_tile0 = bs_tile0;
  STIL_REQUIRE(!bstats || (bs_y && bs_stats && (bs_relu == 0 || bs_relu == 2) && bs_tile0 >= 0 && !colstats && !a_bn && p.wide &&
                           ((uintptr_t)bs_y % 16) == 0 && ((uintptr_t)bs_stats % 16) == 0 && (tune % 100 == 0 || tune % 100 == 11 || tune % 100 == 44)),
               "stil_gemm_nt: bstats needs bs_y / bs_stats, bs_relu 0 or 2, the 16-byte epilogue on 64x64 tiles (stil_gemm_nt_bstats_ok) "
               "and excludes colstats / a_bn");
  STIL_REQUIRE(!colstats || (p.os == 1 && !bias && !sub && !scale && !shift && !resid && act == 0),
               "stil_gemm_nt: colstats describes the raw product (no bias / affine / residual / activation / output map)");
  p.vecA = is_vec(A, lda) && (srcC % 4 == 0);
  p.vecB = is_vec(W, ldb);
  int rc = check_geom(p.g, 0);
  if (rc) return rc;
  hipStream_t s = (hipStream_t)stream;
  const bool plain = KH * KW == 1 && stride == 1 && pad_y == 0 && pad_x == 0 && mode == 0 && p.os == 1 && srcH == OH && srcW == OW;
  const int cfg = nt_config(A, W, M, N, K, lda, ldb, srcC, KH, KW, plain ? 1 : 0, a_bn ? 1 : 0, tune, false);
  const int variant = cfg % 100;
  const bool bk32 = (cfg / 100) % 10 >= 1;
  const bool single = (cfg / 100) % 10 == 2;
  const bool acc2 = (cfg / 1000) % 10 == 1;
  const bool vec = (cfg / 10000) % 10 == 1;
  STIL_REQUIRE(!a_bn || (vec && !bk32 && mode == 0 && srcC % 16 == 0 && srcC <= 2048 && (tune % 100 == 0 || tune % 100 == 11 || tune % 100 == 44)),
               "stil_gemm_nt: a_bn runs 64x64 tiles only (tune %% 100 must be 0 or 11: the caller sizes colstats by "
               "stil_gemm_nt_tile_rows) and needs 16-byte aligned operands, a forward gather, Cin %% 16 == 0 and Cin <= 2048 (Cin=%d)", srcC);
  rc = gemm_nt_attr();
  if (rc) return rc;
  if (variant == 11 && p.splits == 1) p.panel = nt_panel(M, N, K);
  if (!want_b3 && variant == 11 && p.splits == 1 && p.wide && !scalar_epilogue && mode == 0 && (!a_bn || srcC <= 2048) &&
      nt_big_wanted(M, N, K, plain, vec, srcC, tune) && (long)cdiv(M, 64) * cdiv(N, 64) >= 256) {
    p.panel = (p.panel > 0 && p.panel % 2 == 0 && (N / 128) % (p.panel / 2) == 0) ? p.panel / 2 : 0;
    const dim3 grid_((M / 128) * (N / 128));
    const size_t lds_ = (size_t)256 * 36 * sizeof(float) + (a_bn ? (size_t)3 * srcC * sizeof(float) : 0);
    static bool attr_ = false;
    if (!attr_) {
      (void)hipFuncSetAttribute((const void*)gemm_nt_big_kernel<true, true>, hipFuncAttributeMaxDynamicSharedMemorySize, 80 * 1024);
      (void)hipFuncSetAttribute((const void*)gemm_nt_big_kernel<false, true>, hipFuncAttributeMaxDynamicSharedMemorySize, 80 * 1024);
      attr_ = true;
    }
    if (acc2 && a_bn) hipLaunchKernelGGL((gemm_nt_big_kernel<true, true>), grid_, dim3(256), lds_, s, p);
    else if (acc2) hipLaunchKernelGGL((gemm_nt_big_kernel<true, false>), grid_, dim3(256), lds_, s, p);
    else if (a_bn) hipLaunchKernelGGL((gemm_nt_big_kernel<false, true>), grid_, dim3(256), lds_, s, p);
    else hipLaunchKernelGGL((gemm_nt_big_kernel<false, false>), grid_, dim3(256), lds_, s, p);
    STIL_LAUNCH_CHECK();
    return STIL_OK;
  }
  if (a_bn) {
    const dim3 grid_(cdiv(M, 64) * cdiv(N, 64) * p.splits);
    if (want_b3 && srcC % 32 == 0 && K % 32 == 0 && !scalar_epilogue) {
      const size_t lds3_ = (size_t)3 * 128 * 40 * 2 + (size_t)3 * srcC * sizeof(float);
      if (plain) hipLaunchKernelGGL((gemm_nt_kernel<1, 1, 32, true, true, true, true, 1, true>), grid_, dim3(256), lds3_, s, p);
      else hipLaunchKernelGGL((gemm_nt_kernel<1, 1, 32, true, true, false, true, 1, true>), grid_, dim3(256), lds3_, s, p);
      STIL_LAUNCH_CHECK();
      return STIL_OK;
    }
    const size_t lds_ = (size_t)2 * 64 * 2 * 20 * sizeof(float) + (size_t)3 * srcC * sizeof(float);
    if (acc2 && plain) hipLaunchKernelGGL((gemm_nt_kernel<1, 1, 16, true, true, true, true>), grid_, dim3(256), lds_, s, p);
    else if (acc2) hipLaunchKernelGGL((gemm_nt_kernel<1, 1, 16, true, true, false, true>), grid_, dim3(256), lds_, s, p);
    else if (plain) hipLaunchKernelGGL((gemm_nt_kernel<1, 1, 16, true, false, true, true>), grid_, dim3(256), lds_, s, p);
    else hipLaunchKernelGGL((gemm_nt_kernel<1, 1, 16, true, false, false, true>), grid_, dim3(256), lds_, s, p);
    STIL_LAUNCH_CHECK();
    return STIL_OK;
  }
#define LAUNCH_NT(TM_, TN_, BK_, V_)                                                                          \
  do {                                                                                                        \
    const dim3 grid_(cdiv(M, 64 * TM_) * cdiv(N, 64 * TN_) * ((TM_) * (TN_) == 1 ? p.splits : 1));              \
    const size_t lds_ = (size_t)2 * 64 * (TM_ + TN_) * (BK_ + 4) * sizeof(float);                             \
    if (acc2 && plain) hipLaunchKernelGGL((gemm_nt_kernel<TM_, TN_, BK_, V_, true, true>), grid_, dim3(256), lds_, s, p);   \
    else if (acc2) hipLaunchKernelGGL((gemm_nt_kernel<TM_, TN_, BK_, V_, true, false>), grid_, dim3(256), lds_, s, p);      \
    else if (plain) hipLaunchKernelGGL((gemm_nt_kernel<TM_, TN_, BK_, V_, false, true>), grid_, dim3(256), lds_, s, p);     \
    else hipLaunchKernelGGL((gemm_nt_kernel<TM_, TN_, BK_, V_, false, false>), grid_, dim3(256), lds_, s, p);               \
  } while (0)
  if (want_b3 && vec && variant == 11 && K % 32 == 0 && (KH * KW == 1 || srcC % 32 == 0) && !scalar_epilogue) {
    const dim3 grid_(cdiv(M, 64) * cdiv(N, 64) * p.splits);
    const size_t lds3_ = (size_t)3 * 128 * 40 * 2;
    if (plain) hipLaunchKernelGGL((gemm_nt_kernel<1, 1, 32, true, true, true, false, 1, true>), grid_, dim3(256), lds3_, s, p);
    else hipLaunchKernelGGL((gemm_nt_kernel<1, 1, 32, true, true, false, false, 1, true>), grid_, dim3(256), lds3_, s, p);
    STIL_LAUNCH_CHECK();
    return STIL_OK;
  }
  if (!vec) {
    if (variant == 11) LAUNCH_NT(1, 1, 16, false); else if (variant == 21) LAUNCH_NT(2, 1, 16, false); else if (variant == 12) LAUNCH_NT(1, 2, 16, false); else LAUNCH_NT(2, 2, 16, false);
  } else if (variant == 11 && single) {
    const dim3 grid_(cdiv(M, 64) * cdiv(N, 64) * p.splits);
    const size_t lds_ = (size_t)64 * 2 * 36 * sizeof(float);
    if (acc2 && plain) hipLaunchKernelGGL((gemm_nt_kernel<1, 1, 32, true, true, true, false, 1>), grid_, dim3(256), lds_, s, p);
    else if (acc2) hipLaunchKernelGGL((gemm_nt_kernel<1, 1, 32, true, true, false, false, 1>), grid_, dim3(256), lds_, s, p);
    else if (plain) hipLaunchKernelGGL((gemm_nt_kernel<1, 1, 32, true, false, true, false, 1>), grid_, dim3(256), lds_, s, p);
    else hipLaunchKernelGGL((gemm_nt_kernel<1, 1, 32, true, false, false, false, 1>), grid_, dim3(256), lds_, s, p);
  } else if (variant == 11) { if (bk32) LAUNCH_NT(1, 1, 32, true); else LAUNCH_NT(1, 1, 16, true); }
  else if (variant == 12) { LAUNCH_NT(1, 2, 16, true); }
  else if (variant == 21) { if (bk32) LAUNCH_NT(2, 1, 32, true); else LAUNCH_NT(2, 1, 16, true); }
  else { if (bk32) LAUNCH_NT(2, 2, 32, true); else LAUNCH_NT(2, 2, 16, true); }
#undef LAUNCH_NT
  STIL_LAUNCH_CHECK();
  return STIL_OK;
}

static inline int tn_variant(int M, int N, int K, int tune) {
  static const int small_m = [] { const char* e = getenv("STIL_WGRAD_SMALLM"); return e ? atoi(e) : 8192; }();
  if (tune == 11 || tune == 22) return tune;
  if (M < small_m || (M < 4 * small_m && (long)N * K < 262144)) return 11;
  if (N > 256) return 22;
  return (N >= 128 && K >= 256 && K <= 1024) ? 22 : 11;
}
static int g_force_wsplits = 0;
extern "C" int stil_wgrad_force_splits(int s) { const int old = g_force_wsplits; g_force_wsplits = s; return old; }
static int wgrad_splits(int M, int N, int K, int tune) {
  if (g_force_wsplits > 0) { const int m = M / 16 > 0 ? M / 16 : 1; const int s = g_force_wsplits < m ? g_force_wsplits : m; return s > 256 ? 256 : s; }
  const int tv = tn_variant(M, N, K, tune);
  int tiles = tv == 11 ? cdiv(N, 64) * cdiv(K, 64) : cdiv(N, N <= 64 ? 64 : 128) * cdiv(K, 128);
  int want = cdiv(tv == 11 ? 2304 : 768, tiles);
  int maxs = M / 256 > 0 ? M / 256 : 1;
  int s = want < maxs ? want : maxs;
  if (s < 1) s = 1;
  if (s > 256) s = 256;
  return s;
}

extern "C" size_t stil_wgrad_workspace_bytes(int M, int N, int K, int tune) {
  return (size_t)wgrad_splits(M, N, K, tune) * N * K * sizeof(float);
}

static int wgrad_config(const float* dY, const float* X, int M, int N, int K, int ldy, int ldx, int srcC, int KH, int KW,
                        int x_bn, const void* workspace, int tune) {
  if (!(tune == 0 || tune == 11 || tune == 22)) return -1;
  const bool vec = is_vec(dY, ldy) && is_vec(X, ldx) && (srcC % 4 == 0) && (N % 4 == 0) && (K % 4 == 0);
  if (x_bn && !vec) return -1;
  const int tile = tn_variant(M, N, K, tune) == 11 ? 11 : (N <= 64 ? 12 : 22);
  const bool reduce4 = K % 4 == 0 && (KH * KW == 1 || srcC % 4 == 0) && ((uintptr_t)workspace % 16) == 0;
  return tile + 100 * (vec ? 1 : 0) + 1000 * (x_bn ? 1 : 0) + 10000 * (reduce4 ? 1 : 0);
}
extern "C" int stil_wgrad_config(const float* dY, const float* X, int M, int N, int K, int ldy, int ldx, int srcC, int KH, int KW,
                                 int x_bn, const void* workspace, int tune) {
  return wgrad_config(dY, X, M, N, K, ldy, ldx, srcC, KH, KW, x_bn, workspace, tune);
}

extern "C" int stil_wgrad_splits(int M, int N, int K, int tune) { return wgrad_splits(M, N, K, tune); }
static int wgrad_tn_impl(const float* dY, const float* X, float* dW, int M, int N, int K, int ldy, int ldx,
                             int srcH, int srcW, int srcC, int OH, int OW, int KH, int KW, int stride, int pad,
                             int Kdst, int accumulate, const float* x_bn, float* workspace, size_t workspace_bytes, int tune, void* stream) {
  STIL_REQUIRE(dY && X && workspace, "stil_wgrad_tn: null pointer");
  STIL_REQUIRE(tune == 0 || tune == 11 || tune == 22, "stil_wgrad_tn: bad tune %d", tune);
  STIL_REQUIRE(KH * KW * srcC == K, "stil_wgrad_tn: K=%d != KH*KW*C=%d", K, KH * KW * srcC);
  STIL_REQUIRE(M % (OH * OW) == 0, "stil_wgrad_tn: M=%d not a multiple of OH*OW", M);
  STIL_REQUIRE(srcC % 4 == 0 || KH * KW == 1, "stil_wgrad_tn: conv needs Cin %% 4 == 0");
  int splits = wgrad_splits(M, N, K, tune);
  STIL_REQUIRE(workspace_bytes >= (size_t)splits * N * K * sizeof(float), "stil_wgrad_tn: workspace too small");
  GemmTNArgs p;
  p.Y = dY; p.X = X; p.P = workspace; p.M = M; p.N = N; p.K = K; p.ldy = ldy; p.ldx = ldx;
  p.g = ConvGeom{srcH, srcW, srcC, OH, OW, KH, KW, stride, pad, pad, 0};
  int mps = cdiv(M, splits);
  mps = ((mps + 15) / 16) * 16;
  p.m_per_split = mps;
  p.vecY = is_vec(dY, ldy);
  p.vecX = is_vec(X, ldx) && (srcC % 4 == 0);
  p.xbn = x_bn;
  hipStream_t s = (hipStream_t)stream;
  const int cfg = wgrad_config(dY, X, M, N, K, ldy, ldx, srcC, KH, KW, x_bn ? 1 : 0, workspace, tune);
  STIL_REQUIRE(cfg >= 0, "stil_wgrad_tn: x_bn needs 16-byte aligned operands and Cin %% 4 == 0");
  const int tile = cfg % 100;
  const bool vec = (cfg / 100) % 10 == 1;
  if (tile == 11) {
    dim3 grid(cdiv(N, 64) * cdiv(K, 64) * splits);
    if (x_bn) hipLaunchKernelGGL((gemm_tn_kernel<1, 1, true, true>), grid, dim3(256), 0, s, p);
    else if (vec) hipLaunchKernelGGL((gemm_tn_kernel<1, 1, true>), grid, dim3(256), 0, s, p);
    else hipLaunchKernelGGL((gemm_tn_kernel<1, 1, false>), grid, dim3(256), 0, s, p);
  } else if (tile == 12) {
    dim3 grid(cdiv(N, 64) * cdiv(K, 128) * splits);
    if (x_bn) hipLaunchKernelGGL((gemm_tn_kernel<1, 2, true, true>), grid, dim3(256), 0, s, p);
    else if (vec) hipLaunchKernelGGL((gemm_tn_kernel<1, 2, true>), grid, dim3(256), 0, s, p);
    else hipLaunchKernelGGL((gemm_tn_kernel<1, 2, false>), grid, dim3(256), 0, s, p);
  } else {
    dim3 grid(cdiv(N, 128) * cdiv(K, 128) * splits);
    if (x_bn) hipLaunchKernelGGL((gemm_tn_kernel<2, 2, true, true>), grid, dim3(256), 0, s, p);
    else if (vec) hipLaunchKernelGGL((gemm_tn_kernel<2, 2, true>), grid, dim3(256), 0, s, p);
    else hipLaunchKernelGGL((gemm_tn_kernel<2, 2, false>), grid, dim3(256), 0, s, p);
  }
  STIL_LAUNCH_CHECK();
  if (!dW) return STIL_OK;
  long total = (long)N * K;
  int taps = KH * KW;
  if (cfg / 10000 == 1)
    hipLaunchKernelGGL(wgrad_reduce4_kernel, dim3(cdiv(total / 4, 32)), dim3(256), 0, s, workspace, dW, splits, N, K, srcC,
                       taps, Kdst, accumulate);
  else
    hipLaunchKernelGGL(wgrad_reduce_kernel, dim3(cdiv(total, 256)), dim3(256), 0, s, workspace, dW, splits, N, K, srcC,
                       taps, Kdst, accumulate);
  STIL_LAUNCH_CHECK();
  return STIL_OK;
}

extern "C" int stil_wgrad_tn(const float* dY, const float* X, float* dW, int M, int N, int K, int ldy, int ldx,
                             int srcH, int srcW, int srcC, int OH, int OW, int KH, int KW, int stride, int pad,
                             int Kdst, int accumulate, const float* x_bn, float* workspace, size_t workspace_bytes, int tune, void* stream) {
  STIL_REQUIRE(dW, "stil_wgrad_tn: null pointer");
  return wgrad_tn_impl(dY, X, dW, M, N, K, ldy, ldx, srcH, srcW, srcC, OH, OW, KH, KW, stride, pad, Kdst, accumulate, x_bn, workspace,
                       workspace_bytes, tune, stream);
}
extern "C" int stil_wgrad_tn_partial(const float* dY, const float* X, int M, int N, int K, int ldy, int ldx,
                                     int srcH, int srcW, int srcC, int OH, int OW, int KH, int KW, int stride, int pad,
                                     const float* x_bn, float* workspace, size_t workspace_bytes, int tune, void* stream) {
  return wgrad_tn_impl(dY, X, nullptr, M, N, K, ldy, ldx, srcH, srcW, srcC, OH, OW, KH, KW, stride, pad, K, 0, x_bn, workspace,
                       workspace_bytes, tune, stream);
}

extern "C" size_t stil_colsum_workspace_bytes(int M, int N) {
  int rpc = 128;
  return (size_t)cdiv(M, rpc) * N * sizeof(float);
}

static int colsum_impl(const float* X, float* out, int M, int N, int ld, int accumulate, float scale,
                       float* workspace, size_t workspace_bytes, void* stream) {
  STIL_REQUIRE(X && workspace && M > 0 && N > 0, "stil_colsum: null pointer or empty shape");
  int rpc = 128, nch = cdiv(M, rpc);
  STIL_REQUIRE(workspace_bytes >= (size_t)nch * N * sizeof(float), "stil_colsum: workspace too small");
  hipStream_t s = (hipStream_t)stream;
  hipLaunchKernelGGL(colsum_partial_kernel, dim3(cdiv(N, 64), nch), dim3(256), 0, s, X, workspace, M, N, ld, rpc);
  STIL_LAUNCH_CHECK();
  if (!out) return STIL_OK;
  hipLaunchKernelGGL(colsum_final_kernel, dim3(cdiv(N, 32)), dim3(256), 0, s, workspace, out, nch, N, accumulate, scale);
  STIL_LAUNCH_CHECK();
  return STIL_OK;
}
extern "C" int stil_colsum(const float* X, float* out, int M, int N, int ld, int accumulate, float scale,
                           float* workspace, size_t workspace_bytes, void* stream) {
  STIL_REQUIRE(out, "stil_colsum: null pointer or empty shape");
  return colsum_impl(X, out, M, N, ld, accumulate, scale, workspace, workspace_bytes, stream);
}
extern "C" int stil_colsum_chunks(int M) { return cdiv(M, 128); }
extern "C" int stil_colsum_partial(const float* X, int M, int N, int ld, float* workspace, size_t workspace_bytes, void* stream) {
  return colsum_impl(X, nullptr, M, N, ld, 0, 1.f, workspace, workspace_bytes, stream);
}
```

### stil_tta_amd/modules.py

```python
from __future__ import annotations

from typing import Dict, List, Optional

import torch
import torch.nn as nn

from . import ops


class TeacherPipe:

    def __init__(self, flat, momentum: float, eman: bool):
        self.flat, self.momentum, self.eman = flat, float(momentum), eman
        self.events = []
        self.i = 0
        self.start = torch.cuda.Event()

    def published(self):
        ev = torch.cuda.Event()
        ev.record(ops.current_stream_obj())
        self.events.append(ev)

    def before_teacher_bn(self, bn: nn.BatchNorm2d):
        ops.current_stream_obj().wait_event(self.events[self.i])
        self.i += 1
        if self.eman:
            f = self.flat
            off = (bn.running_mean.data_ptr() - f.ema.data_ptr()) // 4
            n = (bn.running_var.data_ptr() - bn.running_mean.data_ptr()) // 4
            f.ema_update_range(off, 2 * n, self.momentum)


_PIPE: Optional[TeacherPipe] = None


def set_teacher_pipe(pipe: Optional[TeacherPipe]):
    global _PIPE
    _PIPE = pipe


def _conv_bn(x, conv: nn.Conv2d, bn: nn.BatchNorm2d, relu: bool, train: bool, resid=None, stem=None, passthrough=False, defer=False,
             xstats=None, premask_in=None, premask_out=None, rstats=None, bstat_send=None, bstat_recv=None):
    k, stride, pad = conv.kernel_size[0], conv.stride[0], conv.padding[0]
    pipe = _PIPE
    if train:
        out = ops.ConvBnActFn.apply(x, conv.weight, bn.weight, bn.bias, bn.running_mean, bn.running_var,
                                    bn.num_batches_tracked, resid, k, stride, pad, relu, stem, passthrough, defer, xstats,
                                    premask_in, premask_out, rstats, bstat_send, bstat_recv)
        if pipe is not None:
            pipe.published()
        return out
    assert not defer and xstats is None and rstats is None
    if pipe is not None:
        pipe.before_teacher_bn(bn)
    out = ops.conv_bn_eval(x, conv.weight, bn.weight, bn.bias, bn.running_mean, bn.running_var, resid, k, stride, pad,
                           relu, stem)
    return (out, x) if passthrough else out


class Bottleneck(nn.Module):
    expansion = 4

    def __init__(self, inplanes, planes, stride=1, downsample=None):
        super().__init__()
        self.conv1 = nn.Conv2d(inplanes, planes, 1, bias=False)
        self.bn1 = nn.BatchNorm2d(planes)
        self.conv2 = nn.Conv2d(planes, planes, 3, stride=stride, padding=1, bias=False)
        self.bn2 = nn.BatchNorm2d(planes)
        self.conv3 = nn.Conv2d(planes, planes * 4, 1, bias=False)
        self.bn3 = nn.BatchNorm2d(planes * 4)
        self.downsample = downsample

    def run(self, x, train):
        d1 = train and ops.can_defer_bn(self.conv1.out_channels)
        d2 = train and ops.can_defer_bn(self.conv2.out_channels)
        st1 = st2 = None
        pm = train and ops._PREMASK
        cin = getattr(x, "_stil_premask", None) if pm else None
        cout = {} if pm else None
        bin_ = getattr(x, "_stil_bstat", None) if train else None
        b1, b2, b3 = ({}, {}, {}) if train else (None, None, None)
        if d1:
            out, identity, st1 = _conv_bn(x, self.conv1, self.bn1, True, train, passthrough=True, defer=True, premask_in=cin, bstat_send=bin_, bstat_recv=b1)
        else:
            out, identity = _conv_bn(x, self.conv1, self.bn1, True, train, passthrough=True, premask_in=cin, bstat_send=bin_)
        if d2:
            out, st2 = _conv_bn(out, self.conv2, self.bn2, True, train, defer=True, xstats=st1, bstat_send=b1, bstat_recv=b2)
        else:
            out = _conv_bn(out, self.conv2, self.bn2, True, train, xstats=st1, bstat_send=b1)
        rst = None
        if self.downsample is not None:
            if train and ops.can_defer_bn(self.downsample[0].out_channels):
                identity, rst = _conv_bn(identity, self.downsample[0], self.downsample[1], False, train, defer=True)
            else:
                identity = _conv_bn(identity, self.downsample[0], self.downsample[1], False, train)
        Nb, H, W, C = identity.shape
        out = _conv_bn(out, self.conv3, self.bn3, True, train, resid=identity.reshape(Nb * H * W, C), xstats=st2, premask_out=cout, rstats=rst,
                       bstat_send=b2, bstat_recv=b3)
        if cout is not None:
            out._stil_premask = cout
            out._stil_bstat = b3
        return out


class BasicBlock(nn.Module):
    expansion = 1

    def __init__(self, inplanes, planes, stride=1, downsample=None):
        super().__init__()
        self.conv1 = nn.Conv2d(inplanes, planes, 3, stride=stride, padding=1, bias=False)
        self.bn1 = nn.BatchNorm2d(planes)
        self.conv2 = nn.Conv2d(planes, planes, 3, padding=1, bias=False)
        self.bn2 = nn.BatchNorm2d(planes)
        self.downsample = downsample

    def run(self, x, train):
        st1 = None
        pm = train and ops._PREMASK
        cin = getattr(x, "_stil_premask", None) if pm else None
        cout = {} if pm else None
        bin_ = getattr(x, "_stil_bstat", None) if train else None
        b1, b2 = ({}, {}) if train else (None, None)
        if train and ops.can_defer_bn(self.conv1.out_channels):
            out, identity, st1 = _conv_bn(x, self.conv1, self.bn1, True, train, passthrough=True, defer=True, premask_in=cin, bstat_send=bin_, bstat_recv=b1)
        else:
            out, identity = _conv_bn(x, self.conv1, self.bn1, True, train, passthrough=True, premask_in=cin, bstat_send=bin_)
        rst = None
        if self.downsample is not None:
            if train and ops.can_defer_bn(self.downsample[0].out_channels):
                identity, rst = _conv_bn(identity, self.downsample[0], self.downsample[1], False, train, defer=True)
            else:
                identity = _conv_bn(identity, self.downsample[0], self.downsample[1], False, train)
        Nb, H, W, C = identity.shape
        out = _conv_bn(out, self.conv2, self.bn2, True, train, resid=identity.reshape(Nb * H * W, C), xstats=st1, premask_out=cout, rstats=rst,
                       bstat_send=b1, bstat_recv=b2)
        if cout is not None:
            out._stil_premask = cout
            out._stil_bstat = b2
        return out


class ResNet(nn.Module):

    CFG = {"resnet18": (BasicBlock, [2, 2, 2, 2]), "resnet34": (BasicBlock, [3, 4, 6, 3]),
           "resnet50": (Bottleneck, [3, 4, 6, 3]), "resnet101": (Bottleneck, [3, 4, 23, 3]),
           "resnet152": (Bottleneck, [3, 8, 36, 3])}

    def __init__(self, name: str):
        super().__init__()
        block, layers = self.CFG[name]
        self.inplanes = 64
        self.conv1 = nn.Conv2d(3, 64, 7, stride=2, padding=3, bias=False)
        self.bn1 = nn.BatchNorm2d(64)
        self.layer1 = self._make_layer(block, 64, layers[0])
        self.layer2 = self._make_layer(block, 128, layers[1], 2)
        self.layer3 = self._make_layer(block, 256, layers[2], 2)
        self.layer4 = self._make_layer(block, 512, layers[3], 2)
        self.out_dim = 512 * block.expansion
        for m in self.modules():
            if isinstance(m, nn.Conv2d):
                nn.init.kaiming_normal_(m.weight, mode="fan_out", nonlinearity="relu")

    def _make_layer(self, block, planes, blocks, stride=1):
        downsample = None
        if stride != 1 or self.inplanes != planes * block.expansion:
            downsample = nn.Sequential(nn.Conv2d(self.inplanes, planes * block.expansion, 1, stride=stride, bias=False),
                                       nn.BatchNorm2d(planes * block.expansion))
        layers = [block(self.inplanes, planes, stride, downsample)]
        self.inplanes = planes * block.expansion
        for _ in range(1, blocks):
            layers.append(block(self.inplanes, planes))
        return nn.Sequential(*layers)

    def _stem(self, x_nchw, train: bool, cache: Optional[dict]):
        if cache is not None and "stem_col" in cache:
            col, meta = cache["stem_col"]
        else:
            col, meta = ops.im2col_stem(x_nchw.contiguous(), 7, 2, 3)
            if cache is not None:
                cache["stem_col"] = (col, meta)
        wpad = ops.pad_stem_weight(self.conv1.weight, meta[3])
        x = _conv_bn(col, self.conv1, self.bn1, True, train, stem=(*meta, wpad))
        return ops.MaxPoolFn.apply(x)

    def _blocks(self):
        return [blk for layer in (self.layer1, self.layer2, self.layer3, self.layer4) for blk in layer]

    def run(self, x_nchw, train: bool, cache: Optional[dict] = None):
        x = self._stem(x_nchw, train, cache)
        for blk in self._blocks():
            x = blk.run(x, train)
        Nb, H, W, C = x.shape
        return x.reshape(Nb, H * W, C)

    def run_pair(self, teacher: "ResNet", x_nchw, cache: dict, side: torch.cuda.Stream):
        def on_side(fn, *a):
            with torch.no_grad(), torch.cuda.stream(side):
                return fn(*a)
        xs = self._stem(x_nchw, True, cache)
        xt = on_side(teacher._stem, x_nchw, False, cache)
        for bs, bt in zip(self._blocks(), teacher._blocks()):
            xs = bs.run(xs, True)
            xt = on_side(bt.run, xt, False)
        Nb, H, W, C = xs.shape
        return xs.reshape(Nb, H * W, C), on_side(lambda t: t.reshape(Nb, H * W, C), xt)


class Mlp(nn.Module):
    def __init__(self, in_f, hid, out_f=None):
        super().__init__()
        self.fc1 = nn.Linear(in_f, hid)
        self.fc2 = nn.Linear(hid, out_f or in_f)


class Attention(nn.Module):
    def __init__(self, dim, num_heads=8, qkv_bias=False):
        super().__init__()
        self.num_heads = num_heads
        self.qkv = nn.Linear(dim, dim * 3, bias=qkv_bias)
        self.proj = nn.Linear(dim, dim)


class Block(nn.Module):
    def __init__(self, dim, num_heads=8, mlp_ratio=4.0):
        super().__init__()
        self.norm1 = nn.LayerNorm(dim)
        self.attn = Attention(dim, num_heads)
        self.norm2 = nn.LayerNorm(dim)
        self.mlp = Mlp(dim, int(dim * mlp_ratio))

    def run(self, x):
        B, T, D = x.shape
        a = ops.layernorm(x, self.norm1.weight, self.norm1.bias)
        qkv = ops.linear(a, self.attn.qkv.weight, self.attn.qkv.bias)
        o = ops.attention(qkv, self.attn.num_heads, [(0, T, 0, T)])
        if ops._LINEAR_RESID:
            x = ops.linear(o, self.attn.proj.weight, self.attn.proj.bias, resid=x.contiguous())
        else:
            x = ops.drop_add(ops.linear(o, self.attn.proj.weight, self.attn.proj.bias), resid=x, rowlen=D)
        m = ops.layernorm(x, self.norm2.weight, self.norm2.bias)
        m = ops.linear(m, self.mlp.fc1.weight, self.mlp.fc1.bias, act=2)
        if ops._LINEAR_RESID:
            return ops.linear(m, self.mlp.fc2.weight, self.mlp.fc2.bias, resid=x)
        return ops.drop_add(ops.linear(m, self.mlp.fc2.weight, self.mlp.fc2.bias), resid=x, rowlen=D)


class TabularTransformerEncoder(nn.Module):
    def __init__(self, hp, cat_lengths: List[int], con_lengths: List[int]):
        super().__init__()
        D = hp.tabular_embedding_dim
        self.num_cat, self.num_con = len(cat_lengths), len(con_lengths)
        self.cat_embedding = nn.Embedding(sum(cat_lengths), D)
        self.con_proj = nn.Linear(1, D)
        self.cls_token = nn.Parameter(torch.zeros(1, 1, D))
        self.mask_special_token = nn.Parameter(torch.zeros(1, 1, D))
        self.column_embedding = nn.Embedding(self.num_cat + self.num_con + 1, D)
        self.norm = nn.LayerNorm(D)
        self.transformer_blocks = nn.ModuleList([Block(D) for _ in range(hp.tabular_transformer_num_layers)])
        offs = torch.tensor([0] + list(cat_lengths[:-1]), dtype=torch.int64).cumsum(0).to(torch.int32)
        rowcol = torch.cat([torch.full((c,), j, dtype=torch.int32) for j, c in enumerate(cat_lengths)]) if cat_lengths \
            else torch.zeros(0, dtype=torch.int32)
        self.register_buffer("cat_offsets", offs, persistent=False)
        self.register_buffer("emb_rowcol", rowcol, persistent=False)
        nn.init.trunc_normal_(self.cls_token, std=0.02)
        nn.init.trunc_normal_(self.mask_special_token, std=0.02)
        self.apply(self._init_weights)

    @staticmethod
    def _init_weights(m):
        if isinstance(m, (nn.Linear, nn.Embedding)):
            m.weight.data.normal_(mean=0.0, std=0.02)
        elif isinstance(m, nn.LayerNorm):
            m.bias.data.zero_()
            m.weight.data.fill_(1.0)
        if isinstance(m, nn.Linear) and m.bias is not None:
            m.bias.data.zero_()

    def run(self, x):
        h = ops.TabEmbedFn.apply(x.contiguous(), self.cat_embedding.weight if self.num_cat else None,
                                 self.con_proj.weight if self.num_con else None, self.con_proj.bias if self.num_con else None,
                                 self.cls_token, self.column_embedding.weight, self.cat_offsets, self.emb_rowcol, self.num_cat)
        h = ops.layernorm(h, self.norm.weight, self.norm.bias)
        for blk in self.transformer_blocks:
            h = blk.run(h)
        return h


class MIAttention(nn.Module):
    def __init__(self, dim, num_heads):
        super().__init__()
        self.num_heads = num_heads
        self.qkv = nn.Linear(dim, dim * 3, bias=True)
        self.proj = nn.Linear(dim, dim)


class MITransformerLayer(nn.Module):

    def __init__(self, dim, num_heads=4, p=0.1):
        super().__init__()
        self.p = p
        self.norm1 = nn.LayerNorm(dim)
        self.attn = MIAttention(dim, num_heads)
        self.norm2 = nn.LayerNorm(dim)
        self.mlp = Mlp(dim, dim, dim)

    def run(self, X, Ni, Nt, masks: Optional[Dict[str, torch.Tensor]]):
        B, T, C = X.shape
        p = self.p
        sc = 1.0 / (1.0 - p) if masks is not None else 1.0
        mk = (lambda k: None) if masks is None else (lambda k: masks[k])
        a = ops.layernorm(X, self.norm1.weight, self.norm1.bias)
        qkv = ops.linear(a, self.attn.qkv.weight, self.attn.qkv.bias)
        windows = [(1, Ni, 1, Ni), (1 + Ni, Nt, 1 + Ni, Nt), (0, 1, 0, T)]
        am = None if masks is None else [masks["attn_i"], masks["attn_t"], masks["attn_c"]]
        o = ops.attention(qkv, self.attn.num_heads, windows, am, p if masks is not None else 0.0)
        pr = ops.linear(o, self.attn.proj.weight, self.attn.proj.bias)
        pr = ops.drop_add(pr, emask=mk("proj"), rowlen=C, scale=sc)
        X = ops.drop_add(pr, resid=X, rmask=mk("dp1"), rowlen=C, scale=sc)
        m = ops.layernorm(X, self.norm2.weight, self.norm2.bias)
        m = ops.linear(m, self.mlp.fc1.weight, self.mlp.fc1.bias, act=2)
        m = ops.drop_add(m, emask=mk("fc1"), rowlen=C, scale=sc)
        m = ops.linear(m, self.mlp.fc2.weight, self.mlp.fc2.bias)
        m = ops.drop_add(m, emask=mk("fc2"), rowlen=C, scale=sc)
        return ops.drop_add(m, resid=X, rmask=mk("dp2"), rowlen=C, scale=sc)


def fuse_mi_masks(m: Dict[str, torch.Tensor], device) -> Dict[str, torch.Tensor]:
    u8 = lambda t: t.to(device=device, dtype=torch.uint8).contiguous()
    Ni, Nt = m["proj_i"].shape[1], m["proj_t"].shape[1]
    out = {"attn_i": u8(m["attn_i"]), "attn_t": u8(m["attn_t"]), "attn_c": u8(m["attn_c"])}
    for k in ("proj", "fc1", "fc2"):
        out[k] = u8(torch.cat([m[k + "_c"], m[k + "_i"], m[k + "_t"]], dim=1))
    for k in ("dp1", "dp2"):
        out[k] = u8(torch.cat([m[k + "_c"][:, None], m[k + "_i"][:, None].expand(-1, Ni), m[k + "_t"][:, None].expand(-1, Nt)], dim=1))
    return out


_stream_idx_cache = {}


def random_mi_masks(B, Ni, Nt, C, H, p, seed, offset, device, step=None) -> Dict[str, torch.Tensor]:
    T = 1 + Ni + Nt
    o = [offset]

    def draw(*shape):
        n = 1
        for s in shape:
            n *= s
        t = ops.rng_mask(shape, p, seed, o[0], device, step)
        o[0] += n
        return t

    out = {"attn_i": draw(B, H, Ni, Ni), "attn_t": draw(B, H, Nt, Nt), "attn_c": draw(B, H, 1, T),
           "proj": draw(B, T, C), "fc1": draw(B, T, C), "fc2": draw(B, T, C)}
    idx = _stream_idx_cache.get((Ni, Nt, str(device)))
    if idx is None:
        idx = torch.cat([torch.zeros(1, dtype=torch.long), torch.ones(Ni, dtype=torch.long), torch.full((Nt,), 2, dtype=torch.long)]).to(device)
        _stream_idx_cache[(Ni, Nt, str(device))] = idx
    for k in ("dp1", "dp2"):
        out[k] = draw(B, 3)[:, idx].contiguous()
    return out


class MLP(nn.Module):
    def __init__(self, in_dim, hidden_dim, out_dim):
        super().__init__()
        self.model = nn.Sequential(nn.Linear(in_dim, hidden_dim), nn.ReLU(inplace=True), nn.Linear(hidden_dim, out_dim))

    def run(self, x):
        h = ops.linear(x, self.model[0].weight, self.model[0].bias, act=1)
        return ops.linear(h, self.model[2].weight, self.model[2].bias)


def split_field_lengths(field_lengths):
    cat = [int(v) for v in field_lengths if int(v) != 1]
    con = [int(v) for v in field_lengths if int(v) == 1]
    return cat, con


class DisCoAttentionBackbone(nn.Module):

    def __init__(self, hp, field_lengths):
        super().__init__()
        self.encoder_imaging = ResNet(hp.model)
        cat, con = split_field_lengths(field_lengths)
        self.encoder_tabular = TabularTransformerEncoder(hp, cat, con)
        pooled, C, Dt = hp.embedding_dim, hp.multimodal_embedding_dim, hp.tabular_embedding_dim
        self.projection_si = MLP(pooled, C, C)
        self.projection_ai = MLP(pooled, C, C)
        self.projection_st = MLP(Dt, Dt, C)
        self.projection_at = MLP(Dt, Dt, C)
        self.reduce = nn.Linear(C * 2, C)
        self.transformer = nn.ModuleList([MITransformerLayer(C, 4, 0.1) for _ in range(hp.multimodal_transformer_num_layers)])
        self.classifier_multimodal = nn.Linear(C * 3, hp.num_classes)
        self.classifier_imaging = nn.Linear(C * 2, hp.num_classes)
        self.classifier_tabular = nn.Linear(C * 2, hp.num_classes)

    def tabular_tokens(self, x_tab, train: bool, mi_masks=None):
        return self.encoder_tabular.run(x_tab)

    def forward_all(self, x, train: Optional[bool] = None, mi_masks=None, cache=None, x_i=None, x_t=None):
        train = self.training if train is None else train
        x_img, x_tab = x[0], x[1]
        if x_i is None:
            x_i = self.encoder_imaging.run(x_img, train, cache)
        if x_t is None:
            x_t = self.tabular_tokens(x_tab, train, mi_masks)
        x_si = self.projection_si.run(x_i)
        x_ai = self.projection_ai.run(ops.tokmean(x_i))
        x_st = self.projection_st.run(x_t[:, 1:, :].contiguous())
        x_at = self.projection_at.run(x_t[:, 0, :].contiguous())
        x_c = ops.linear(torch.cat([x_ai, x_at], dim=1), self.reduce.weight, self.reduce.bias)
        Ni, Nt = x_si.shape[1], x_st.shape[1]
        X = torch.cat([x_c.unsqueeze(1), x_si, x_st], dim=1)
        for li, layer in enumerate(self.transformer):
            mk = None if (mi_masks is None or not train) else mi_masks[li]
            X = layer.run(X, Ni, Nt, mk)
        e_c = X[:, 0, :].contiguous()
        e_si = ops.tokmean(X[:, 1:1 + Ni, :])
        e_st = ops.tokmean(X[:, 1 + Ni:, :])
        out_m = ops.linear(torch.cat([e_si, e_c, e_st], dim=1), self.classifier_multimodal.weight, self.classifier_multimodal.bias)
        out_i = ops.linear(torch.cat([e_si, x_ai], dim=1), self.classifier_imaging.weight, self.classifier_imaging.bias)
        out_t = ops.linear(torch.cat([e_st, x_at], dim=1), self.classifier_tabular.weight, self.classifier_tabular.bias)
        return out_m, out_i, out_t, e_si, ops.tokmean(x_si), x_ai, e_st, ops.tokmean(x_st), x_at, e_c

    def forward(self, x, train: Optional[bool] = None):
        o = self.forward_all(x, train)
        return o[0], o[1], o[2], o[3], o[5], o[6], o[8], o[9]
```

### stil_tta_amd/ops.py

```python
from __future__ import annotations

import ctypes
import math
from typing import NamedTuple, Optional

import torch

from ._lib import lib

_vp = ctypes.c_void_p


def _p(t: Optional[torch.Tensor]):
    return None if t is None else t.data_ptr()


_raw_current_stream = getattr(torch._C, "_cuda_getCurrentRawStream", None)
_current_device = getattr(torch._C, "_cuda_getDevice", None)


def _raw_stream(device=None) -> int:
    if _raw_current_stream is None or _current_device is None:
        return torch.cuda.current_stream(device).cuda_stream
    if device is None:
        idx = _current_device()
    elif isinstance(device, int):
        idx = device
    else:
        idx = device.index if device.index is not None else _current_device()
    return _raw_current_stream(idx)


def _stream():
    return _raw_stream()


_STREAM_OBJS = {}


def current_stream_obj(device=None) -> "torch.cuda.Stream":
    if _raw_current_stream is None or _current_device is None:
        return torch.cuda.current_stream(device)
    idx = _current_device() if device is None else (device if isinstance(device, int) else (device.index if device.index is not None else _current_device()))
    key = (idx, _raw_current_stream(idx))
    st = _STREAM_OBJS.get(key)
    if st is None:
        st = _STREAM_OBJS[key] = torch.cuda.current_stream(idx)
    return st


def _chk(*ts):
    for t in ts:
        if t is None:
            continue
        if not t.is_cuda:
            raise RuntimeError("stil_tta_amd ops need CUDA(HIP) tensors: there is no CPU fallback")
        if not t.is_contiguous():
            raise RuntimeError("stil_tta_amd ops need contiguous tensors")


class _Workspace:
    zero = False

    def __init__(self):
        self.buf = {}
        self.captured = set()
        self.pinned = []

    def get(self, nbytes: int, device, stream=None) -> torch.Tensor:
        nbytes = max(int(nbytes), 256)
        key = (device, _raw_stream(device) if stream is None else stream.cuda_stream)
        b = self.buf.get(key)
        capturing = torch.cuda.is_current_stream_capturing()
        if b is None or b.numel() < nbytes:
            if b is not None and key in self.captured:
                self.pinned.append(b)
                self.captured.discard(key)
            n = int(nbytes * (1.5 if self.zero else 1.25)) + 4096
            if stream is None:
                b = (torch.zeros if self.zero else torch.empty)(n, dtype=torch.uint8, device=device)
            else:
                with torch.cuda.stream(stream):
                    b = (torch.zeros if self.zero else torch.empty)(n, dtype=torch.uint8, device=device)
            self.buf[key] = b
        if capturing:
            self.captured.add(key)
        return b


_ws = _Workspace()


class _SplitWorkspace(_Workspace):
    zero = True


_split_ws = _SplitWorkspace()
_SPLITK = __import__("os").environ.get("STIL_SPLITK", "1") != "0"

TUNE = {"gemm": int(__import__("os").environ.get("STIL_GEMM_TUNE", "0")), "wgrad": int(__import__("os").environ.get("STIL_WGRAD_TUNE", "0"))}
B3_FLAG = 100000
if __import__("os").environ.get("STIL_PRECISION", "fp32") == "bf16x3":
    TUNE["gemm"] += B3_FLAG


class _SideStream:

    def __init__(self):
        import os
        self.enabled = os.environ.get("STIL_WGRAD_STREAM", "1") != "0"
        self.in_capture = os.environ.get("STIL_GRAPH_SIDE", "0") != "0"
        self.streams = {}
        self.use_branch = os.environ.get("STIL_BRANCH_STREAM", "0") != "0"
        self.branch = {}
        self.keep = []

    def retire(self, everything=False):
        k = self.keep
        if torch.cuda.is_current_stream_capturing():
            if everything:
                del k[:]
            return
        i = 0
        while i < len(k) and (everything or k[i][0].query()):
            i += 1
        del k[:i]

    def get(self, device):
        st = self.streams.get(device)
        if st is None:
            st = self.streams[device] = torch.cuda.Stream(device)
        return st

    def get_branch(self, device):
        st = self.branch.get(device)
        if st is None:
            st = self.branch[device] = torch.cuda.Stream(device)
        return st

    def all_streams(self):
        return list(self.streams.values()) + list(self.branch.values())


_side = _SideStream()


def join_side():
    _defer.flush()
    for st in _side.all_streams():
        torch.cuda.current_stream(st.device).wait_stream(st)
    _side.retire(everything=True)


def branch_stream(device):
    if not _side.use_branch or side_stream(device) is None or torch.cuda.is_current_stream_capturing():
        return None
    return _side.get_branch(device)


def side_stream(device):
    if not _side.enabled or _prof_active():
        return None
    if not _side.in_capture and torch.cuda.is_current_stream_capturing():
        return None
    return _side.get(device)


_trace = None


_exchange = None


def _touch(param):
    param._stil_touched = True
    if _exchange is not None:
        _exchange.note(param)


def cached_layout(param, attr: str, key=None):
    plan = getattr(param, "_stil_layouts", None)
    if plan is None or not plan.current(param):
        return None
    if plan.event is not None:
        dev_ = plan.slab.device
        sk = (dev_.index, _raw_stream(dev_))
        if sk not in plan.waited:
            current_stream_obj(dev_).wait_event(plan.event)
            plan.waited.add(sk)
    v = getattr(param, attr, None)
    if v is None or key is None:
        return v
    return v.get(key)


def _grad_into(param: torch.Tensor, writer):
    slot = getattr(param, "_gslot", None)
    if slot is not None:
        writer(slot, 1, True)
        _touch(param)
        return None
    g = torch.empty_like(param)
    writer(g, 0, False)
    return g


class _DeferredReduce:
    _JOB = __import__("struct").Struct("<QQ7if")

    def __init__(self):
        self.mode = __import__("os").environ.get("STIL_REDUCE_DEFER", "auto")
        self.forced = 0
        self.ws = _Workspace()
        self.st = {}
        self.high = {}

    def active(self) -> bool:
        if _exchange is not None or self.mode == "0":
            return False
        return self.mode == "1" or self.forced > 0

    def _state(self, device):
        key = (device, _raw_stream(device))
        d = self.st.get(key)
        if d is None:
            st = torch.cuda.current_stream(device)
            d = self.st[key] = dict(stream=st, device=device, size=max(256 << 20, int(1.25 * self.high.get(device, 0))), off=0, jobs=[], dsts=set())
        return d

    def alloc(self, nbytes: int, device) -> int:
        d = self._state(device)
        n = (int(nbytes) + 255) & ~255
        if d["off"] + n > d["size"]:
            self._flush_one(d)
            d["size"] = max(d["size"], 2 * n, int(1.25 * self.high.get(device, 0)))
        buf = self.ws.get(d["size"], device)
        assert buf.numel() >= d["size"]
        a = buf.data_ptr() + d["off"]
        a += (-a) % 256
        d["off"] = a - buf.data_ptr() + n
        self.high[device] = max(self.high.get(device, 0), d["off"])
        return a

    def add(self, device, P: int, dst: torch.Tensor, splits, N, K, Cin, taps, Kdst, accumulate, scale):
        d = self._state(device)
        if dst.data_ptr() in d["dsts"]:
            self._flush_one(d, reset_off=False)
        d["dsts"].add(dst.data_ptr())
        d["jobs"].append(self._JOB.pack(P, dst.data_ptr(), splits, N, K, Cin, taps, Kdst, accumulate, float(scale)))

    def _flush_one(self, d, reset_off=True):
        if d["jobs"]:
            L = lib()
            assert L.reduce_job_bytes() == self._JOB.size, "StilReduceJob layout changed"
            blob = b"".join(d["jobs"])
            with torch.cuda.stream(d["stream"]):
                L.reduce_jobs(blob, len(d["jobs"]), d["stream"].cuda_stream)
        d["jobs"], d["dsts"] = [], set()
        if reset_off:
            d["off"] = 0

    def flush(self):
        for d in self.st.values():
            self._flush_one(d)


_defer = _DeferredReduce()


class deferring:

    def __enter__(self):
        _defer.forced += 1

    def __exit__(self, *exc):
        _defer.forced -= 1


_POLICY = []
for _r in __import__("os").environ.get("STIL_GEMM_POLICY", "").split(","):
    if _r.strip():
        _k, _t = _r.strip().split(":")
        _POLICY.append((int(_k[1:]), int(_t)))
_POLICY.sort(reverse=True)


def _shape_tune(M, N, K, a_bn, has_tile_stats):
    t = TUNE["gemm"]
    if t % B3_FLAG or a_bn or not _POLICY:
        return t
    for mink, tune in _POLICY:
        if K >= mink:
            if tune % 100 not in (0, 11, 44) and (has_tile_stats or M % 128 or N % 128):
                return t
            return tune
    return t


def gemm_nt(A, W, M, N, K, *, lda=None, ldb=None, out=None, ldc=None, geom=None, bias=None, sub=None, scale=None, shift=None,
            resid=None, pre=None, act=0, alpha=1.0, pads=None, outmap=None, out_rows=None, colstats=None, a_bn=None, relu_mask=None,
            bstats=None, scale_var=None, var_eps=0.0):
    if geom is None:
        geom = (1, 1, K, 1, 1, 1, 1, 1, 0, 0)
    pads = (geom[8], geom[8]) if pads is None else pads
    outmap = (1, 0, 0, geom[3], geom[4]) if outmap is None else outmap
    lda = geom[2] if lda is None else lda
    ldb = K if ldb is None else ldb
    ldc = N if ldc is None else ldc
    if out is None:
        out = torch.empty((M if out_rows is None else out_rows, N), dtype=torch.float32, device=A.device)
    L = lib()
    meta = None
    tune = _shape_tune(M, N, K, a_bn is not None, bstats is not None or colstats is not None)
    if L._prof is not None:
        s2 = geom[7] * geom[7] if geom[9] == 1 else 1
        src = (M // (geom[3] * geom[4])) * geom[0] * geom[1] * geom[2]
        nbytes = 4.0 * (src + N * K + M * N * (1 + (resid is not None) + (pre is not None) + (relu_mask is not None) + (bstats is not None)))
        plain = int(geom[5] * geom[6] == 1 and geom[7] == 1 and pads == (0, 0) and geom[9] == 0 and outmap[0] == 1
                    and geom[0] == geom[3] and geom[1] == geom[4])
        cfg = L.gemm_nt_config(_p(A), _p(W), M, N, K, lda, ldb, geom[2], geom[5], geom[6], plain, int(a_bn is not None), tune)
        meta = (cfg, 2.0 * M * N * K / s2, (M, N, K, geom[5], geom[7], geom[9]), nbytes)
    sw, swn = None, 0
    if _SPLITK:
        swn = L.gemm_nt_split_workspace_bytes(M, N, K, tune)
        if swn:
            sw = _split_ws.get(swn, A.device)
    L.gemm_nt(_p(A), _p(W), _p(out), M, N, K, lda, ldb, ldc, *geom[:8], pads[0], pads[1], geom[9], *outmap,
              _p(bias), _p(sub), _p(scale), _p(shift), _p(resid),
              (ldc if resid is not None else 0), _p(pre), act, float(alpha), _p(colstats), _p(a_bn), _p(relu_mask),
              (ldc if relu_mask is not None else 0), *((_p(bstats[0]), _p(bstats[1]), _p(bstats[2]), int(bstats[3]), int(bstats[4]))
                                                       if bstats is not None else (None, None, None, 0, 0)),
              _p(scale_var), float(var_eps), _p(sw), (sw.numel() if sw is not None else 0), tune, _stream(), meta=meta)
    return out


def wgrad_tn(dY, X, dW, M, N, K, *, ldy=None, ldx=None, geom=None, Kdst=None, accumulate=0, x_bn=None, slot=False, stream=None):
    if geom is None:
        geom = (1, 1, K, 1, 1, 1, 1, 1, 0)
    ldy = N if ldy is None else ldy
    ldx = geom[2] if ldx is None else ldx
    Kdst = K if Kdst is None else Kdst
    L = lib()
    nb = L.wgrad_workspace_bytes(M, N, K, TUNE["wgrad"])
    meta = (0, 2.0 * M * N * K, (M, N, K, geom[5], geom[7], 2)) if L._prof is not None else None
    if slot and _defer.active():
        a = _defer.alloc(nb, dY.device)
        L.wgrad_tn_partial(_p(dY), _p(X), M, N, K, ldy, ldx, *geom, _p(x_bn), a, nb, TUNE["wgrad"], _stream(), meta=meta)
        _defer.add(dY.device, a, dW, L.wgrad_splits(M, N, K, TUNE["wgrad"]), N, K, geom[2], geom[5] * geom[6], Kdst, accumulate, 1.0)
        return
    w = _ws.get(nb, dY.device, stream)
    L.wgrad_tn(_p(dY), _p(X), _p(dW), M, N, K, ldy, ldx, *geom, Kdst, accumulate, _p(x_bn), _p(w), nb, TUNE["wgrad"],
               _stream() if stream is None else stream.cuda_stream, meta=meta)


_WGRAD_SIDE = __import__("os").environ.get("STIL_WGRAD_SIDE", "1") != "0"


def wgrad_param(param, dY, X, M, N, K, **kw):
    slot = getattr(param, "_gslot", None)
    side = side_stream(dY.device) if (slot is not None and _WGRAD_SIDE) else None
    if side is None:
        return _grad_into(param, lambda dst, acc, slot_: wgrad_tn(dY, X, dst, M, N, K, accumulate=acc, slot=slot_, **kw))
    main = current_stream_obj(dY.device)
    _side.retire()
    if main.cuda_stream == side.cuda_stream or _defer.active():
        if main != side:
            side.wait_stream(main)
        with torch.cuda.stream(side):
            wgrad_tn(dY, X, slot, M, N, K, accumulate=1, slot=True, **kw)
            if main != side:
                ev = torch.cuda.Event()
                ev.record(side)
                _side.keep.append((ev, (dY, X, kw.get("x_bn"))))
    else:
        fork = torch.cuda.Event()
        fork.record(main)
        side.wait_event(fork)
        wgrad_tn(dY, X, slot, M, N, K, accumulate=1, slot=True, stream=side, **kw)
        ev = torch.cuda.Event()
        ev.record(side)
        _side.keep.append((ev, (dY, X, kw.get("x_bn"))))
    _touch(param)
    return None


def _prof_active():
    L = lib()
    return L._prof is not None and L._prof_single


def colsum(X, out, M, N, *, ld=None, accumulate=0, scale=1.0, slot=False):
    L = lib()
    nb = L.colsum_workspace_bytes(M, N)
    if slot and _defer.active():
        a = _defer.alloc(nb, X.device)
        L.colsum_partial(_p(X), M, N, N if ld is None else ld, a, nb, _stream())
        _defer.add(X.device, a, out, L.colsum_chunks(M), 1, N, N, 1, N, accumulate, scale)
        return
    w = _ws.get(nb, X.device)
    L.colsum(_p(X), _p(out), M, N, N if ld is None else ld, accumulate, float(scale), _p(w), nb, _stream())


def transpose(x2d):
    R, C = x2d.shape
    out = torch.empty((C, R), dtype=torch.float32, device=x2d.device)
    lib().transpose(_p(x2d), _p(out), R, C, _stream())
    return out


def axpby(x, y, a, b, out=None):
    out = torch.empty_like(x) if out is None else out
    lib().axpby(_p(x), _p(y), _p(out), x.numel(), float(a), float(b), _stream())
    return out


def rng_mask(shape, p, seed, offset, device, step=None):
    out = torch.empty(shape, dtype=torch.uint8, device=device)
    lib().rng_mask(_p(out), out.numel(), int(seed), int(offset), float(p), _p(step), _stream())
    return out


class LinearFn(torch.autograd.Function):

    @staticmethod
    def forward(ctx, x, weight, bias, act, resid=None):
        _chk(x, weight, bias, resid)
        K = x.shape[-1]
        N = weight.shape[0]
        x2 = x.reshape(-1, K)
        M = x2.shape[0]
        assert resid is None or (act == 0 and resid.numel() == M * N), "LinearFn: a residual needs act == 0 and the output's shape"
        pre = torch.empty((M, N), dtype=torch.float32, device=x.device) if act == 2 else None
        y = gemm_nt(x2, weight, M, N, K, bias=bias, pre=pre, act=act, resid=None if resid is None else resid.reshape(M, N))
        ctx.act = act
        ctx.has_bias = bias is not None
        ctx.has_resid = resid is not None
        if _trace is not None and act == 1 and any(ctx.needs_input_grad):
            _trace["relu"][id(weight)] = y.view(*x.shape[:-1], N)
        ctx.save_for_backward(x2, weight, bias, pre if act == 2 else (y if act == 1 else None))
        ctx.xshape = x.shape
        return y.reshape(*x.shape[:-1], N)

    @staticmethod
    def backward(ctx, gy):
        x2, weight, bias, ref = ctx.saved_tensors
        M, K = x2.shape
        N = weight.shape[0]
        g = gy.contiguous().reshape(M, N)
        if ctx.act:
            gp = torch.empty_like(g)
            lib().act_bwd(_p(g), _p(ref), _p(gp), g.numel(), ctx.act, _stream())
            g = gp
        dx = None
        if ctx.needs_input_grad[0]:
            wt = cached_layout(weight, "_stil_wd")
            if wt is None:
                wt = transpose(weight)
            dx = gemm_nt(g, wt, M, K, N).reshape(ctx.xshape)
        dw = wgrad_param(weight, g, x2, M, N, K) if ctx.needs_input_grad[1] else None
        db = None
        if ctx.has_bias and ctx.needs_input_grad[2]:
            db = _grad_into(bias, lambda dst, acc, slot_: colsum(g, dst, M, N, accumulate=acc, slot=slot_))
        dres = gy if (ctx.has_resid and ctx.needs_input_grad[4]) else None
        return dx, dw, db, None, dres


def linear(x, weight, bias=None, act=0, resid=None):
    return LinearFn.apply(x, weight, bias, act, resid)


class MatmulNTFn(torch.autograd.Function):

    @staticmethod
    def forward(ctx, A, B, alpha):
        _chk(A, B)
        M, K = A.shape
        N = B.shape[0]
        ctx.save_for_backward(A, B)
        ctx.alpha = alpha
        return gemm_nt(A, B, M, N, K, alpha=alpha)

    @staticmethod
    def backward(ctx, gZ):
        A, B = ctx.saved_tensors
        M, K = A.shape
        N = B.shape[0]
        gZ = gZ.contiguous()
        dA = gemm_nt(gZ, transpose(B), M, K, N, alpha=ctx.alpha) if ctx.needs_input_grad[0] else None
        dB = gemm_nt(transpose(gZ), transpose(A), N, K, M, alpha=ctx.alpha) if ctx.needs_input_grad[1] else None
        return dA, dB, None


def _conv_geom_fwd(H, W, C, OH, OW, k, stride, pad):
    return (H, W, C, OH, OW, k, k, stride, pad, 0)


_BN_EPILOGUE_STATS = __import__("os").environ.get("STIL_BN_EPILOGUE_STATS", "1") != "0"


_BN_DEFER = __import__("os").environ.get("STIL_BN_DEFER", "1") != "0"
_PREMASK = __import__("os").environ.get("STIL_PREMASK", "1") != "0"
_BN_BWD_EPILOGUE = __import__("os").environ.get("STIL_BN_BWD_EPILOGUE", "1") != "0"
_LINEAR_RESID = __import__("os").environ.get("STIL_LINEAR_RESID", "1") != "0"


def can_defer_bn(Cout: int) -> bool:
    return _BN_DEFER and _BN_EPILOGUE_STATS and Cout % 16 == 0 and Cout <= 2048


_bn_frozen = False


class frozen_bn_stats:

    def __enter__(self):
        global _bn_frozen
        self.prev, _bn_frozen = _bn_frozen, True

    def __exit__(self, *exc):
        global _bn_frozen
        _bn_frozen = self.prev


_bn_prior = None


class bn_prior:

    def __init__(self, N, B):
        N, B = float(N), int(B)
        if not (math.isfinite(N) and N >= 0.0) or B < 1:
            raise ValueError(f"ops.bn_prior: N={N!r} must be finite and >= 0, B={B!r} >= 1")
        self.rho = B / (N + B)

    def __enter__(self):
        global _bn_prior
        self.prev, _bn_prior = _bn_prior, self.rho

    def __exit__(self, *exc):
        global _bn_prior
        _bn_prior = self.prev


_bn_memory = None


class bn_memory:

    def __init__(self, mem, rho, alpha, unbiased=False, update=True):
        rho, alpha = float(rho), float(alpha)
        if not (0.0 <= rho <= 1.0 and 0.0 <= alpha <= 1.0):
            raise ValueError(f"ops.bn_memory: rho={rho!r} and alpha={alpha!r} must lie in [0, 1]")
        self.mem, self.rho, self.alpha, self.unbiased, self.update = mem, rho, alpha, bool(unbiased), bool(update)

    def __enter__(self):
        global _bn_memory
        if _bn_prior is not None:
            raise RuntimeError("ops.bn_memory takes the place of ops.bn_prior: the two scopes do not nest")
        self.prev, _bn_memory = _bn_memory, self

    def __exit__(self, *exc):
        global _bn_memory
        _bn_memory = self.prev


class _BnRule(NamedTuple):
    family: str
    rho: object = None
    src: tuple = ()
    out: tuple = (None, None)
    alpha: float = 0.0
    unbiased: bool = False
    delta: object = None


def _bn_rule(rmean, rvar, nbt, C, dev) -> _BnRule:
    if _bn_memory is not None:
        if not _bn_frozen or rmean is None or _bn_prior is not None:
            raise RuntimeError("ops.bn_memory belongs inside ops.frozen_bn_stats, without ops.bn_prior, and needs the layer's running_mean")
        mem = _bn_memory
        src_mean, src_var, out_mean, out_var = mem.mem.layer(rmean)
        return _BnRule("memory", mem.rho, (src_mean, src_var), (out_mean, out_var) if mem.update else (None, None), mem.alpha,
                       mem.unbiased, torch.empty((C,), dtype=torch.float32, device=dev))
    if _bn_prior is not None:
        if not _bn_frozen or rmean is None or rvar is None:
            raise RuntimeError("ops.bn_prior belongs inside ops.frozen_bn_stats and needs the layer's running statistics")
        return _BnRule("prior", _bn_prior, (rmean, rvar), delta=torch.empty((C,), dtype=torch.float32, device=dev))
    if _bn_frozen:
        return _BnRule("train", src=(None, None, None))
    return _BnRule("train", src=(rmean, rvar, nbt))


def _bn_fwd_call(rule, tiles, y, ts, tile_rows, gamma, beta, resid, rstats, z, stats, M, C, relu):
    L = lib()
    assert tiles or rstats is None
    nb = L.bn_tiles_workspace_bytes(M, C, tile_rows) if tiles else L.bn_workspace_bytes(M, C)
    ws = _ws.get(nb, y.device)
    head = (_p(y), _p(ts), tile_rows, _p(gamma), _p(beta)) if tiles else (_p(y), _p(gamma), _p(beta))
    res = (_p(resid), _p(rstats)) if tiles else (_p(resid),)
    src = tuple(_p(t) for t in rule.src)
    sfx = "_tiles" if tiles else ""
    if rule.family == "train":
        getattr(L, "bn_train_fwd" + sfx)(*head, *src, *res, _p(z), _p(stats), M, C, 1 if relu else 0, 1e-5, 0.1, _p(ws), nb, _stream())
        return
    if rule.family == "memory":
        fn, src = getattr(L, "bn_memory_fwd" + sfx), src + (_p(rule.out[0]), _p(rule.out[1]), rule.alpha, int(rule.unbiased))
    else:
        fn = getattr(L, "bn_prior_fwd" + sfx)
    fn(*head, *src, rule.rho, *res, _p(z), _p(stats), _p(rule.delta), M, C, 1 if relu else 0, 1e-5, _p(ws), nb, _stream())


def _bn_bwd_call(rho, delta, tiles, gz, z, y, gamma, stats, dy, gres, dgamma, dbeta, coef, M, C, relu_mode, acc):
    L = lib()
    nb = L.bn_workspace_bytes(M, C)
    ws = _ws.get(nb, gz.device)
    fam = "bn_train_bwd" if rho is None else "bn_prior_bwd"
    head = (_p(gz), _p(z), _p(y), _p(gamma), _p(stats)) + (() if rho is None else (_p(delta), rho))
    if tiles is not None:
        part, nt = tiles
        nb = L.bn_bwd_tiles_workspace_bytes(nt, C)
        ws = _ws.get(nb + 8, gz.device)
        getattr(L, fam + "_tiles")(*head, _p(part), nt, _p(dy), _p(dgamma), _p(dbeta), _p(coef), M, C, relu_mode, acc, _p(ws), nb, _stream())
    else:
        getattr(L, fam)(*head, _p(dy), _p(gres), _p(dgamma), _p(dbeta), _p(coef), M, C, relu_mode, acc, _p(ws), nb, _stream())


class ConvBnActFn(torch.autograd.Function):

    @staticmethod
    def forward(ctx, x, w, gamma, beta, rmean, rvar, nbt, resid, k, stride, pad, relu, stem, passthrough=False, defer=False, xstats=None,
                premask_in=None, premask_out=None, rstats=None, bstat_send=None, bstat_recv=None):
        _chk(x, w, gamma, beta, resid)
        ctx.set_materialize_grads(False)
        assert not defer or resid is None, "a layer with a residual input cannot defer its BatchNorm"
        Cout = w.shape[0]
        dev = x.device
        fused = _BN_EPILOGUE_STATS and Cout % 4 == 0
        if stem is not None:
            Nb, OH, OW, Kp, wpad = stem
            M = Nb * OH * OW
        else:
            Nb, H, W_, Cin = x.shape
            OH = (H + 2 * pad - k) // stride + 1
            OW = (W_ + 2 * pad - k) // stride + 1
            M = Nb * OH * OW
        ts = tile_rows = None
        if fused:
            tile_rows = lib().gemm_nt_tile_rows(M, Cout, TUNE["gemm"])
            ts = torch.empty((2 * ((M + tile_rows - 1) // tile_rows), Cout), dtype=torch.float32, device=dev)
        if stem is not None:
            y = gemm_nt(x, wpad, M, Cout, Kp, colstats=ts)
            wf = None
            geom = None
        else:
            if k == 1:
                wf = w.reshape(Cout, Cin)
            else:
                wf = cached_layout(w, "_stil_wf")
                if wf is None:
                    wf = torch.empty((Cout, k * k * Cin), dtype=torch.float32, device=dev)
                    lib().conv_weight_layout(_p(w), _p(wf), None, Cout, Cin, k, k, _stream())
            geom = _conv_geom_fwd(H, W_, Cin, OH, OW, k, stride, pad)
            y = gemm_nt(x, wf, M, Cout, k * k * Cin, geom=geom, colstats=ts, a_bn=xstats)
        stats = torch.empty((4, Cout), dtype=torch.float32, device=dev)
        assert fused or not defer, "deferred BatchNorm needs the epilogue statistics (can_defer_bn)"
        z = None if (defer and _trace is None) else torch.empty((M, Cout), dtype=torch.float32, device=dev)
        rule = _bn_rule(rmean, rvar, nbt, Cout, dev)
        rho, delta = rule.rho, rule.delta
        _bn_fwd_call(rule, fused, y, ts, tile_rows, gamma, beta, resid, rstats, z, stats, M, Cout, relu)
        if _trace is not None and relu:
            _trace["relu"][id(gamma)] = z.view(Nb, OH, OW, Cout)
        ctx.save_for_backward(x, w, gamma, beta, y, None if defer else z, stats, xstats, delta)
        ctx.rho = rho
        ctx.cfg = (k, stride, pad, relu, stem is not None, resid is not None, geom, (Nb, OH, OW), stem)
        ctx.has_alias = bool(passthrough)
        ctx.premask_in = premask_in if (stem is None and stride == 1) else None
        ctx.premask_out = premask_out if (relu and resid is not None and not defer) else None
        ctx.bstat_send = bstat_send if (_BN_BWD_EPILOGUE and stem is None) else None
        ctx.bstat_recv = None
        if _BN_BWD_EPILOGUE and bstat_recv is not None and Cout % 4 == 0:
            if defer and relu and resid is None:
                bstat_recv.update(y=y, stats=stats, mode=2)
                ctx.bstat_recv = bstat_recv
            elif relu and resid is not None and not defer and premask_out is not None:
                bstat_recv.update(y=y, stats=stats, mode=0, premask=premask_out)
                ctx.bstat_recv = bstat_recv
        out = (y if defer else z).view(Nb, OH, OW, Cout)
        if defer:
            ctx.mark_non_differentiable(stats)
            return (out, x, stats) if passthrough else (out, stats)
        if passthrough:
            return out, x
        return out

    @staticmethod
    def backward(ctx, gz, *more):
        x, w, gamma, beta, y, z, stats, xstats, delta = ctx.saved_tensors
        rho = ctx.rho
        gx_alias = more[0] if (len(more) and ctx.has_alias) else None
        k, stride, pad, relu, is_stem, has_res, geom, (Nb, OH, OW), stem = ctx.cfg
        dev = x.device
        Cout = w.shape[0]
        M = Nb * OH * OW
        gz = gz.contiguous()
        dy = torch.empty((M, Cout), dtype=torch.float32, device=dev)
        premasked = ctx.premask_out is not None and ctx.premask_out.get("masked", False)
        gres = torch.empty((M, Cout), dtype=torch.float32, device=dev) if (has_res and relu and not premasked) else None
        coef = torch.empty((3, Cout), dtype=torch.float32, device=dev)
        gslot, bslot = getattr(gamma, "_gslot", None), getattr(beta, "_gslot", None)
        dgamma = gslot if gslot is not None else torch.empty_like(gamma)
        dbeta = bslot if bslot is not None else torch.empty_like(beta)
        acc = 1 if gslot is not None else 0
        relu_mode = 0 if premasked else ((1 if has_res else 2) if relu else 0)
        cell = ctx.bstat_recv
        part = cell.get("part") if cell is not None else None
        tiles = part is not None and gres is None and tuple(part.shape) == (2 * cell["nt"], Cout) and (cell["mode"] == 2) == (relu_mode == 2) \
            and (cell["mode"] != 0 or premasked)
        _bn_bwd_call(rho, delta, (part, cell["nt"]) if tiles else None, gz, z, y, gamma, stats, dy, gres, dgamma, dbeta, coef, M, Cout,
                     relu_mode, acc)
        if gslot is not None:
            _touch(gamma)
            _touch(beta)
        if has_res:
            dres = gres if (relu and not premasked) else gz.view(M, Cout)
        else:
            dres = None
        dx = None
        want_dw = ctx.needs_input_grad[1]
        if is_stem:
            Kp = stem[3]
            Kreal = w.shape[1] * k * k
            dw = wgrad_param(w, dy, x, M, Cout, Kp, Kdst=Kreal) if want_dw else None
        else:
            _, H, W_, Cin = x.shape
            if ctx.needs_input_grad[0]:
                ga = None if gx_alias is None else gx_alias.contiguous().view(Nb * H * W_, Cin)
                cell = ctx.premask_in if (ctx.premask_in is not None and xstats is None and Cin % 4 == 0 and stride == 1) else None
                zmask = x.view(Nb * H * W_, Cin) if cell is not None else None
                if cell is not None:
                    cell["masked"] = True
                bs = None
                sc_ = ctx.bstat_send
                Min = Nb * H * W_
                if sc_ is not None and "y" in sc_ and Cin % 4 == 0 and _bstats_tune_ok() and (sc_["mode"] == 2 or (zmask is not None and sc_.get("premask") is cell)) \
                        and (stride == 1 or ga is None) and tuple(sc_["y"].shape) == (Min, Cin) \
                        and lib().gemm_nt_bstats_ok(None, Cin, Cin, _p(ga), Cin, _p(zmask), Cin, _p(sc_["y"])):
                    nt_ = _bstat_tiles(Nb, H, W_, k, stride, pad)
                    bs = (sc_["y"], sc_["stats"], torch.empty((2 * nt_, Cin), dtype=torch.float32, device=dev), sc_["mode"], 0)
                if k == 1 and stride == 1:
                    wd = cached_layout(w, "_stil_wd")
                    if wd is None:
                        wd = transpose(w.reshape(Cout, Cin))
                    dx = gemm_nt(dy, wd, M, Cin, Cout, resid=ga, relu_mask=zmask, bstats=bs).view(Nb, H, W_, Cin)
                elif stride == 1:
                    wd = cached_layout(w, "_stil_wd")
                    if wd is None:
                        wd = torch.empty((Cin, k * k * Cout), dtype=torch.float32, device=dev)
                        lib().conv_weight_layout(_p(w), None, _p(wd), Cout, Cin, k, k, _stream())
                    g2 = (OH, OW, Cout, H, W_, k, k, stride, pad, 1)
                    dx = gemm_nt(dy, wd, Nb * H * W_, Cin, k * k * Cout, geom=g2, resid=ga, relu_mask=zmask, bstats=bs).view(Nb, H, W_, Cin)
                else:
                    dx = strided_dgrad(dy, w, Nb, H, W_, Cin, OH, OW, Cout, k, stride, pad, bstats=bs)
                    if ga is not None:
                        axpby(dx.view(-1), ga.view(-1), 1.0, 1.0, out=dx.view(-1))
                if bs is not None:
                    sc_["part"], sc_["nt"] = bs[2], bs[2].shape[0] // 2
            elif gx_alias is not None:
                dx = gx_alias
            gw = geom[:9]
            dw = wgrad_param(w, dy, x, M, Cout, k * k * Cin, geom=gw, x_bn=xstats) if want_dw else None
        return (dx, dw, (None if gslot is not None else dgamma), (None if bslot is not None else dbeta), None, None, None,
                dres, None, None, None, None, None, None, None, None, None, None, None, None, None)


def _bstats_tune_ok() -> bool:
    t = TUNE["gemm"] % B3_FLAG
    return t < 10000 and t % 100 in (0, 11, 44)


def _bstat_tiles(Nb, H, W_, k, stride, pad):
    if stride == 1:
        return (Nb * H * W_ + 63) // 64
    n = 0
    for py in range(stride):
        if len(range((py + pad) % stride, k, stride)) == 0 or len(range(py, H, stride)) == 0:
            continue
        for px in range(stride):
            if len(range((px + pad) % stride, k, stride)) == 0 or len(range(px, W_, stride)) == 0:
                continue
            n += (Nb * len(range(py, H, stride)) * len(range(px, W_, stride)) + 63) // 64
    return n


def strided_dgrad(dy, w, Nb, H, W_, Cin, OH, OW, Cout, k, stride, pad, bstats=None):
    dev = dy.device
    all_covered = all(len(range((p_ + pad) % stride, k, stride)) > 0 for p_ in range(stride))
    dx = (torch.empty if all_covered else torch.zeros)((Nb * H * W_, Cin), dtype=torch.float32, device=dev)
    tile0 = 0
    for py in range(stride):
        ky0 = (py + pad) % stride
        KHs = len(range(ky0, k, stride))
        Hs = len(range(py, H, stride))
        if KHs == 0 or Hs == 0:
            continue
        dy0 = (py + pad - ky0) // stride
        for px in range(stride):
            kx0 = (px + pad) % stride
            KWs = len(range(kx0, k, stride))
            Ws = len(range(px, W_, stride))
            if KWs == 0 or Ws == 0:
                continue
            dx0 = (px + pad - kx0) // stride
            wsub = cached_layout(w, "_stil_wphase", (py, px))
            if wsub is None:
                wsub = torch.empty((Cin, KHs * KWs * Cout), dtype=torch.float32, device=dev)
                lib().conv_weight_layout_phase(_p(w), _p(wsub), Cout, Cin, k, k, stride, ky0, kx0, KHs, KWs, _stream())
            geom = (OH, OW, Cout, Hs, Ws, KHs, KWs, 1, 0, 0)
            gemm_nt(dy, wsub, Nb * Hs * Ws, Cin, KHs * KWs * Cout, geom=geom, out=dx, pads=(KHs - 1 - dy0, KWs - 1 - dx0),
                    outmap=(stride, py, px, H, W_), bstats=None if bstats is None else (*bstats[:4], tile0))
            tile0 += (Nb * Hs * Ws + 63) // 64
    return dx.view(Nb, H, W_, Cin)


def conv_bn_eval(x, w, gamma, beta, rmean, rvar, resid, k, stride, pad, relu, stem=None):
    Cout = w.shape[0]
    dev = x.device
    bn = dict(sub=rmean, scale=gamma, scale_var=rvar, var_eps=1e-5, shift=beta)
    if stem is not None:
        Nb, OH, OW, Kp, wpad = stem
        M = Nb * OH * OW
        z = gemm_nt(x, wpad, M, Cout, Kp, resid=resid, act=1 if relu else 0, **bn)
        return z.view(Nb, OH, OW, Cout)
    Nb, H, W_, Cin = x.shape
    OH = (H + 2 * pad - k) // stride + 1
    OW = (W_ + 2 * pad - k) // stride + 1
    M = Nb * OH * OW
    if k == 1:
        wf = w.reshape(Cout, Cin)
    else:
        wf = cached_layout(w, "_stil_wf")
        if wf is None:
            wf = torch.empty((Cout, k * k * Cin), dtype=torch.float32, device=dev)
            lib().conv_weight_layout(_p(w), _p(wf), None, Cout, Cin, k, k, _stream())
    z = gemm_nt(x, wf, M, Cout, k * k * Cin, geom=_conv_geom_fwd(H, W_, Cin, OH, OW, k, stride, pad), resid=resid, act=1 if relu else 0, **bn)
    return z.view(Nb, OH, OW, Cout)


def im2col_stem(x_nchw, k, stride, pad):
    _chk(x_nchw)
    Nb, Cin, H, W_ = x_nchw.shape
    OH = (H + 2 * pad - k) // stride + 1
    OW = (W_ + 2 * pad - k) // stride + 1
    Kp = ((Cin * k * k + 15) // 16) * 16
    col = torch.empty((Nb * OH * OW, Kp), dtype=torch.float32, device=x_nchw.device)
    lib().im2col_nchw(_p(x_nchw), _p(col), Nb, Cin, H, W_, OH, OW, k, k, stride, pad, Kp, _stream())
    return col, (Nb, OH, OW, Kp)


def pad_stem_weight(w, Kp):
    Cout = w.shape[0]
    wp = torch.zeros((Cout, Kp), dtype=torch.float32, device=w.device)
    wp[:, : w[0].numel()] = w.detach().reshape(Cout, -1)
    return wp


class MaxPoolFn(torch.autograd.Function):

    @staticmethod
    def forward(ctx, x):
        _chk(x)
        Nb, H, W_, C = x.shape
        OH, OW = (H + 2 - 3) // 2 + 1, (W_ + 2 - 3) // 2 + 1
        y = torch.empty((Nb, OH, OW, C), dtype=torch.float32, device=x.device)
        idx = torch.empty((Nb, OH, OW, C), dtype=torch.uint8, device=x.device)
        lib().maxpool3x3s2_fwd(_p(x), _p(y), _p(idx), Nb, H, W_, C, OH, OW, _stream())
        if _trace is not None and ctx.needs_input_grad[0]:
            _trace["pool"]["maxpool"] = (idx, H, W_)
        ctx.save_for_backward(idx)
        ctx.shape = (Nb, H, W_, C, OH, OW)
        return y

    @staticmethod
    def backward(ctx, gy):
        (idx,) = ctx.saved_tensors
        Nb, H, W_, C, OH, OW = ctx.shape
        gy = gy.contiguous()
        dx = torch.empty((Nb, H, W_, C), dtype=torch.float32, device=gy.device)
        lib().maxpool3x3s2_bwd(_p(gy), _p(idx), _p(dx), Nb, H, W_, C, OH, OW, _stream())
        return dx


class LayerNormFn(torch.autograd.Function):
    @staticmethod
    def forward(ctx, x, gamma, beta):
        _chk(x, gamma, beta)
        D = x.shape[-1]
        rows = x.numel() // D
        y = torch.empty_like(x)
        mr = torch.empty((rows, 2), dtype=torch.float32, device=x.device)
        lib().layernorm_fwd(_p(x), _p(gamma), _p(beta), _p(y), _p(mr), rows, D, 1e-5, _stream())
        ctx.save_for_backward(x, gamma, beta, mr)
        return y

    @staticmethod
    def backward(ctx, gy):
        x, gamma, beta, mr = ctx.saved_tensors
        D = x.shape[-1]
        rows = x.numel() // D
        gy = gy.contiguous()
        dx = torch.empty_like(x)
        nb = lib().layernorm_bwd_workspace_bytes(rows, D)
        ws = _ws.get(nb, x.device)
        gslot, bslot = getattr(gamma, "_gslot", None), getattr(beta, "_gslot", None)
        dg = gslot if gslot is not None else torch.empty_like(gamma)
        db = bslot if bslot is not None else torch.empty_like(beta)
        lib().layernorm_bwd(_p(gy), _p(x), _p(gamma), _p(mr), _p(dx), _p(dg), _p(db), rows, D, 1 if gslot is not None else 0,
                            _p(ws), nb, _stream())
        if gslot is not None:
            _touch(gamma)
            _touch(beta)
            return dx, None, None
        return dx, dg, db


def layernorm(x, gamma, beta):
    return LayerNormFn.apply(x, gamma, beta)


class AttentionFn(torch.autograd.Function):

    @staticmethod
    def forward(ctx, qkv, H, windows, masks, drop_p, needs_bwd=True):
        _chk(qkv)
        B, T, three = qkv.shape
        d = three // (3 * H)
        scale = d ** -0.5
        if needs_bwd and qkv.requires_grad:
            for qo, Sq, ko, Skv in windows:
                if lib().attention_config(Sq, Skv, d, 1) < 0:
                    raise RuntimeError(f"stil_attention_bwd would refuse this window (no backward kernel fits 160 KiB of LDS, or a bad "
                                       f"shape): Sq={Sq} Skv={Skv} d={d}; run it under torch.no_grad() if no gradient is needed")
        covered = sum(w_[1] for w_ in windows) == T
        out = (torch.empty if covered else torch.zeros)((B, T, H * d), dtype=torch.float32, device=qkv.device)
        probs = []
        for wi, (qo, Sq, ko, Skv) in enumerate(windows):
            pr = torch.empty((B, H, Sq, Skv), dtype=torch.float32, device=qkv.device)
            mk = None if masks is None else masks[wi]
            _chk(mk)
            lib().attention_fwd(_p(qkv), _p(out), _p(pr), _p(mk), B, T, H, d, qo, Sq, ko, Skv, scale, drop_p, _stream())
            probs.append(pr)
        ctx.save_for_backward(qkv, *probs)
        ctx.cfg = (H, d, windows, masks, drop_p, scale)
        return out

    @staticmethod
    def backward(ctx, gout):
        qkv, *probs = ctx.saved_tensors
        H, d, windows, masks, drop_p, scale = ctx.cfg
        B, T, _ = qkv.shape
        gout = gout.contiguous()
        dqkv = torch.zeros_like(qkv)
        for wi, (qo, Sq, ko, Skv) in enumerate(windows):
            mk = None if masks is None else masks[wi]
            lib().attention_bwd(_p(gout), _p(qkv), _p(probs[wi]), _p(mk), _p(dqkv), B, T, H, d, qo, Sq, ko, Skv, scale,
                                drop_p, _stream())
        return dqkv, None, None, None, None, None


def attention(qkv, H, windows, masks=None, drop_p=0.0):
    return AttentionFn.apply(qkv, H, tuple(windows), masks, drop_p, torch.is_grad_enabled())


class DropAddFn(torch.autograd.Function):

    @staticmethod
    def forward(ctx, x, resid, emask, rmask, rowlen, scale):
        _chk(x, resid, emask, rmask)
        out = torch.empty_like(x)
        lib().drop_add(_p(x), _p(resid), _p(emask), _p(rmask), _p(out), x.numel(), rowlen, scale, _stream())
        ctx.masks = (emask, rmask, rowlen, scale)
        ctx.has_res = resid is not None
        return out

    @staticmethod
    def backward(ctx, g):
        emask, rmask, rowlen, scale = ctx.masks
        g = g.contiguous()
        if emask is None and rmask is None and scale == 1.0:
            dx = g
        else:
            dx = torch.empty_like(g)
            lib().drop_add(_p(g), None, _p(emask), _p(rmask), _p(dx), g.numel(), rowlen, scale, _stream())
        return dx, (g if ctx.has_res else None), None, None, None, None


def drop_add(x, resid=None, emask=None, rmask=None, rowlen=1, scale=1.0):
    if resid is None and emask is None and rmask is None and scale == 1.0:
        return x
    return DropAddFn.apply(x, resid, emask, rmask, rowlen, float(scale))


class TabEmbedFn(torch.autograd.Function):

    @staticmethod
    def forward(ctx, x, cat_emb, con_w, con_b, cls, colemb, offs, rowcol, ncat):
        _chk(x, cat_emb, con_w, con_b, cls, colemb)
        B, ncols = x.shape
        D = cls.shape[-1]
        h = torch.empty((B, ncols + 1, D), dtype=torch.float32, device=x.device)
        lib().tab_embed_fwd(_p(x), _p(offs), _p(cat_emb), _p(con_w), _p(con_b), _p(cls), _p(colemb), _p(h), B, ncols, ncat, D,
                            _stream())
        ctx.save_for_backward(x, cat_emb, con_w, con_b, cls, colemb)
        ctx.cfg = (offs, rowcol, ncat)
        return h

    @staticmethod
    def backward(ctx, g):
        x, cat_emb, con_w, con_b, cls, colemb = ctx.saved_tensors
        offs, rowcol, ncat = ctx.cfg
        B, ncols = x.shape
        D = cls.shape[-1]
        g = g.contiguous()
        params = [cat_emb, con_w, con_b, cls, colemb]
        slots = [getattr(p_, "_gslot", None) if p_ is not None else None for p_ in params]
        use_slab = slots[3] is not None
        outs = [(s if use_slab else (torch.zeros_like(p_) if p_ is not None else None)) for p_, s in zip(params, slots)]
        nb = lib().tab_embed_bwd_workspace_bytes(ncols, D)
        ws = _ws.get(nb, x.device)
        nrows = 0 if cat_emb is None else cat_emb.shape[0]
        lib().tab_embed_bwd(_p(g), _p(x), _p(offs), _p(rowcol), nrows if ncat else 0, _p(outs[0]), _p(outs[1]), _p(outs[2]),
                            _p(outs[3]), _p(outs[4]), B, ncols, ncat, D, 1 if use_slab else 0, _p(ws), nb, _stream())
        if use_slab:
            for p_ in params:
                if p_ is not None:
                    _touch(p_)
            return (None,) * 9
        return (None, outs[0], outs[1], outs[2], outs[3], outs[4], None, None, None)


class TokMeanFn(torch.autograd.Function):
    @staticmethod
    def forward(ctx, x):
        _chk(x)
        B, T, D = x.shape
        y = torch.empty((B, D), dtype=torch.float32, device=x.device)
        lib().tokmean_fwd(_p(x), _p(y), B, T, D, _stream())
        ctx.shape = (B, T, D)
        return y

    @staticmethod
    def backward(ctx, g):
        B, T, D = ctx.shape
        g = g.contiguous()
        dx = torch.empty((B, T, D), dtype=torch.float32, device=g.device)
        lib().tokmean_bwd(_p(g), _p(dx), B, T, D, _stream())
        return dx


def tokmean(x):
    return TokMeanFn.apply(x.contiguous())


class L2NormFn(torch.autograd.Function):

    @staticmethod
    def forward(ctx, x):
        _chk(x)
        R, D = x.shape
        y = torch.empty_like(x)
        n = torch.empty((R,), dtype=torch.float32, device=x.device)
        lib().l2norm_fwd(_p(x), _p(y), _p(n), R, D, _stream())
        ctx.save_for_backward(y, n)
        return y

    @staticmethod
    def backward(ctx, g):
        y, n = ctx.saved_tensors
        g = g.contiguous()
        dx = torch.empty_like(g)
        lib().l2norm_bwd(_p(g), _p(y), _p(n), _p(dx), y.shape[0], y.shape[1], _stream())
        return dx


def l2norm(x):
    return L2NormFn.apply(x.contiguous())


def _scale_by(unit, g, c=1.0):
    out = torch.empty_like(unit)
    lib().scale_dev(_p(unit), _p(g.contiguous()), float(c), _p(out), unit.numel(), _stream())
    return out


class CEHardFn(torch.autograd.Function):

    @staticmethod
    def forward(ctx, logits, labels):
        _chk(logits, labels)
        R, K = logits.shape
        rl = torch.empty((R,), dtype=torch.float32, device=logits.device)
# ... 327 lines not shown
```

Before: 2147 samples/s.

## Pack ReLU masks to bits and fuse strided shortcut dgrad into block input gradient

The BN forward apply kernel now also writes a 1-bit-per-channel ReLU mask beside z. The backward dgrad GEMM epilogue reads that packed mask instead of the full fp32 activation, cutting mask read traffic by 32x. The strided 1x1 downsample shortcut dgrad is computed as a small GEMM on the subsampled grid, and its result is scattered as a residual (row map with zeros off-stride) inside the main-path dgrad epilogue. This removes the zero-filled strided dgrad buffer and a separate axpby pass. The cost is extra index arithmetic in the epilogue, an extra byte write in the forward pass, and added constraints that force the 64x64 tile path.

```diff
diff --git a/stil_tta_amd/_lib.py b/stil_tta_amd/_lib.py
--- a/stil_tta_amd/_lib.py
+++ b/stil_tta_amd/_lib.py
@@ -16,6 +16,7 @@
 ROID_HEADERS = (os.path.join(_HERE, "csrc", "stil_roid.h"),)
 ROTTA_HEADERS = (os.path.join(_HERE, "csrc", "stil_rotta.h"),)
 LAME_HEADERS = (os.path.join(_HERE, "csrc", "stil_lame.h"),)
+TRUNK_HEADERS = (os.path.join(_HERE, "csrc", "stil_trunk.h"),)
 LIB_PATH = os.environ.get("STIL_LIB_PATH") or os.path.join(_HERE, "lib", "libstil_hip.so")
 CSRC = os.path.join(_HERE, "csrc")
 
@@ -81,7 +82,7 @@
                                f"(or `make -C {CSRC}`) first; there is no fallback path")
         self._dll = ctypes.CDLL(LIB_PATH)
         self.protos = parse_header()
-        for header in TTA_HEADERS + MEMORY_HEADERS + READ_HEADERS + CGPL_HEADERS + SHIFT_HEADERS + ROID_HEADERS + ROTTA_HEADERS + LAME_HEADERS:
+        for header in TTA_HEADERS + MEMORY_HEADERS + READ_HEADERS + CGPL_HEADERS + SHIFT_HEADERS + ROID_HEADERS + ROTTA_HEADERS + LAME_HEADERS + TRUNK_HEADERS:
             self.protos.update(parse_header(header))
         for name, (restype, argl) in self.protos.items():
             fn = getattr(self._dll, name)
@@ -113,15 +114,17 @@
         if restype is not ctypes.c_int or name in ("version", "device_count", "gemm_nt_variant", "gemm_nt_tile_rows", "gemm_nt_config", "weight_layout_job_bytes", "weight_layout_job_blocks", "gemm_nt_bstats_ok", "gemm_nt_force_splits", "reduce_job_bytes", "wgrad_splits", "colsum_chunks", "wgrad_force_splits", "attention_config", "wgrad_config", "gemm_nt_panel"):
             return fn
 
+        pname = _PROF_ALIAS.get(name, name)
+
         def call(*args, meta=None):
             prof = self.__dict__.get("_prof")
-            if prof is not None and (self._prof_only is None or name in self._prof_only):
+            if prof is not None and (self._prof_only is None or pname in self._prof_only):
                 import torch
                 s, e = torch.cuda.Event(enable_timing=True), torch.cuda.Event(enable_timing=True)
                 s.record()
                 rc = fn(*args)
                 e.record()
-                prof.append((name, s, e, meta))
+                prof.append((pname, s, e, meta))
             else:
                 rc = fn(*args)
             if rc != 0:
@@ -132,6 +135,8 @@
         return call
 
 
+_PROF_ALIAS = {"gemm_nt_ex": "gemm_nt"}
+
 _lib = None
 
 
diff --git a/stil_tta_amd/csrc/bn.hip b/stil_tta_amd/csrc/bn.hip
--- a/stil_tta_amd/csrc/bn.hip
+++ b/stil_tta_amd/csrc/bn.hip
@@ -176,7 +176,8 @@
 
 __global__ __launch_bounds__(256) void bn_apply_kernel(const float* __restrict__ x, const float* __restrict__ stats,
                                                         const float* __restrict__ resid, const float* __restrict__ rstats,
-                                                        float* __restrict__ z, long total4, int C, int relu) {
+                                                        float* __restrict__ z, long total4, int C, int relu,
+                                                        unsigned char* __restrict__ zbits = nullptr) {
   const float* A = stats + 2 * C;
   const float* B = stats + 3 * C;
   for (long i = (long)blockIdx.x * blockDim.x + threadIdx.x; i < total4; i += (long)gridDim.x * blockDim.x) {
@@ -198,6 +199,11 @@
     }
     if (relu) { v.x = fmaxf(v.x, 0.f); v.y = fmaxf(v.y, 0.f); v.z = fmaxf(v.z, 0.f); v.w = fmaxf(v.w, 0.f); }
     reinterpret_cast<float4*>(z)[i] = v;
+    if (zbits) {
+      const int nib = (v.x > 0.f ? 1 : 0) | (v.y > 0.f ? 2 : 0) | (v.z > 0.f ? 4 : 0) | (v.w > 0.f ? 8 : 0);
+      const int other = __shfl_xor(nib, 1, 64);
+      if ((threadIdx.x & 1) == 0) zbits[i >> 1] = (unsigned char)(nib | (other << 4));
+    }
   }
 }
 
@@ -537,7 +543,8 @@
   if (final_only) return STIL_OK;
   long total4;
   const int grid = bn_wide_grid(M, C, &total4);
-  hipLaunchKernelGGL(bn_apply_kernel, dim3(grid), dim3(256), 0, s, x, stats, resid, (const float*)nullptr, z, total4, C, relu);
+  hipLaunchKernelGGL(bn_apply_kernel, dim3(grid), dim3(256), 0, s, x, stats, resid, (const float*)nullptr, z, total4, C, relu,
+                     (unsigned char*)nullptr);
   STIL_LAUNCH_CHECK();
   return STIL_OK;
 }
@@ -545,8 +552,9 @@
 template <class Finish>
 static int bn_fwd_tiles(const char* who, const Finish& fin, const float* x, const float* tilestats, int tile_rows, const float* resid,
                         const float* resid_stats, float* z, const float* stats, int M, int C, int relu, void* workspace,
-                        size_t workspace_bytes, hipStream_t s, bool final_only = false) {
+                        size_t workspace_bytes, hipStream_t s, bool final_only = false, unsigned char* zbits = nullptr) {
   STIL_REQUIRE(z || !resid, "%s: statistics-only call (z == NULL) cannot take a residual", who);
+  STIL_REQUIRE(!zbits || (z && !final_only && C % 8 == 0), "%s: zbits is written beside z and needs C %% 8 == 0 (C=%d)", who, C);
   STIL_REQUIRE(!resid_stats || resid, "%s: resid_stats without resid", who);
   STIL_REQUIRE(tile_rows > 0 && M > 0 && C > 0 && C % 4 == 0, "%s: bad shape M=%d C=%d tile_rows=%d", who, M, C, tile_rows);
   STIL_REQUIRE(workspace_bytes >= stil_bn_tiles_workspace_bytes(M, C, tile_rows) && ((uintptr_t)workspace % 8) == 0,
@@ -567,7 +575,7 @@
   if (!z || final_only) return STIL_OK;
   long total4;
   const int grid = bn_wide_grid(M, C, &total4);
-  hipLaunchKernelGGL(bn_apply_kernel, dim3(grid), dim3(256), 0, s, x, stats, resid, resid_stats, z, total4, C, relu);
+  hipLaunchKernelGGL(bn_apply_kernel, dim3(grid), dim3(256), 0, s, x, stats, resid, resid_stats, z, total4, C, relu, zbits);
   STIL_LAUNCH_CHECK();
   return STIL_OK;
 }
@@ -650,6 +658,17 @@
                       workspace_bytes, (hipStream_t)stream);
 }
 
+extern "C" int stil_bn_train_fwd_tiles_bits(const float* x, const float* tilestats, int tile_rows, const float* gamma, const float* beta,
+                                            float* running_mean, float* running_var, long long* num_batches_tracked,
+                                            const float* resid, const float* resid_stats, float* z, unsigned char* zbits, float* stats,
+                                            int M, int C, int relu, float eps, float momentum, void* workspace, size_t workspace_bytes,
+                                            void* stream) {
+  STIL_REQUIRE(x && tilestats && gamma && beta && z && zbits && stats && workspace, "stil_bn_train_fwd_tiles_bits: null pointer");
+  const BnTrainFwd fin{gamma, beta, running_mean, running_var, num_batches_tracked, stats, eps, momentum};
+  return bn_fwd_tiles("stil_bn_train_fwd_tiles_bits", fin, x, tilestats, tile_rows, resid, resid_stats, z, stats, M, C, relu, workspace,
+                      workspace_bytes, (hipStream_t)stream, false, zbits);
+}
+
 extern "C" int stil_bn_train_bwd(const float* dz, const float* z, const float* x, const float* gamma,
                                  const float* stats, float* dx, float* gout, float* dgamma, float* dbeta, float* coef,
                                  int M, int C, int relu, int accumulate, float* workspace, size_t workspace_bytes,
diff --git a/stil_tta_amd/csrc/gemm.hip b/stil_tta_amd/csrc/gemm.hip
--- a/stil_tta_amd/csrc/gemm.hip
+++ b/stil_tta_amd/csrc/gemm.hip
@@ -1,4 +1,5 @@
 #include "common.h"
+#include "stil_trunk.h"
 #include <type_traits>
 
 typedef float f32x16 __attribute__((ext_vector_type(16)));
@@ -53,6 +54,9 @@
   float* split_slabs;
   int* split_tickets;
   int panel;
+  const unsigned char* rbits;
+  int ldbits;
+  int rs, rOH, rOW;
 };
 
 __device__ __forceinline__ float4 ld4_guard(const float* p, int nvalid, int vec) {
@@ -170,13 +174,28 @@
           v.x = (v.x - sb.x) * sc.x + sh.x + bia.x; v.y = (v.y - sb.y) * sc.y + sh.y + bia.y;
           v.z = (v.z - sb.z) * sc.z + sh.z + bia.z; v.w = (v.w - sb.w) * sc.w + sh.w + bia.w;
           if (p.resid) {
-            const float4 rr = *reinterpret_cast<const float4*>(p.resid + row * p.ldr + col);
+            float4 rr;
+            if (p.rs > 1) {
+              const int ohw = g.OH * g.OW;
+              const int n = row_m / ohw, rem = row_m - n * ohw;
+              const int y = rem / g.OW, x = rem - y * g.OW;
+              const int ry = y / p.rs, rx = x / p.rs;
+              const bool has = ry * p.rs == y && rx * p.rs == x;
+              const long rrow = has ? ((long)n * p.rOH + ry) * p.rOW + rx : 0;
+              rr = *reinterpret_cast<const float4*>(p.resid + rrow * p.ldr + col);
+              rr.x = has ? rr.x : 0.f; rr.y = has ? rr.y : 0.f; rr.z = has ? rr.z : 0.f; rr.w = has ? rr.w : 0.f;
+            } else {
+              rr = *reinterpret_cast<const float4*>(p.resid + row * p.ldr + col);
+            }
             v.x += rr.x; v.y += rr.y; v.z += rr.z; v.w += rr.w;
           }
           if (p.pre) *reinterpret_cast<float4*>(p.pre + row * p.ldc + col) = v;
           if (p.act == 1) { v.x = fmaxf(v.x, 0.f); v.y = fmaxf(v.y, 0.f); v.z = fmaxf(v.z, 0.f); v.w = fmaxf(v.w, 0.f); }
           else if (p.act == 2) { v.x = gelu_f(v.x); v.y = gelu_f(v.y); v.z = gelu_f(v.z); v.w = gelu_f(v.w); }
-          if (p.rmask) {
+          if (p.rbits) {
+            const unsigned nib = (unsigned)p.rbits[row * p.ldbits + (col >> 3)] >> (col & 4);
+            v.x = (nib & 1u) ? v.x : 0.f; v.y = (nib & 2u) ? v.y : 0.f; v.z = (nib & 4u) ? v.z : 0.f; v.w = (nib & 8u) ? v.w : 0.f;
+          } else if (p.rmask) {
             const float4 mk = *reinterpret_cast<const float4*>(p.rmask + row * p.ldm + col);
             v.x = mk.x > 0.f ? v.x : 0.f; v.y = mk.y > 0.f ? v.y : 0.f; v.z = mk.z > 0.f ? v.z : 0.f; v.w = mk.w > 0.f ? v.w : 0.f;
           }
@@ -1318,14 +1337,15 @@
   return (size_t)NT_SPLIT_TICKET_BYTES + (size_t)tiles * s * 4096 * sizeof(float);
 }
 
-extern "C" int stil_gemm_nt(const float* A, const float* W, float* C, int M, int N, int K, int lda, int ldb, int ldc,
-                            int srcH, int srcW, int srcC, int OH, int OW, int KH, int KW, int stride, int pad_y,
-                            int pad_x, int mode, int out_stride, int out_py, int out_px, int out_OH, int out_OW,
-                            const float* bias, const float* sub, const float* scale,
-                            const float* shift, const float* resid, int ldr, float* pre, int act, float alpha,
-                            float* colstats, const float* a_bn, const float* relu_mask, int ldm,
-                            const float* bs_y, const float* bs_stats, float* bstats, int bs_relu, int bs_tile0,
-                            const float* scale_var, float var_eps, void* split_ws, size_t split_ws_bytes, int tune_arg, void* stream) {
+static int gemm_nt_impl(const float* A, const float* W, float* C, int M, int N, int K, int lda, int ldb, int ldc,
+                        int srcH, int srcW, int srcC, int OH, int OW, int KH, int KW, int stride, int pad_y,
+                        int pad_x, int mode, int out_stride, int out_py, int out_px, int out_OH, int out_OW,
+                        const float* bias, const float* sub, const float* scale,
+                        const float* shift, const float* resid, int ldr, float* pre, int act, float alpha,
+                        float* colstats, const float* a_bn, const float* relu_mask, int ldm,
+                        const float* bs_y, const float* bs_stats, float* bstats, int bs_relu, int bs_tile0,
+                        const float* scale_var, float var_eps, const unsigned char* rbits, int ldbits, int resid_stride, int resid_OH,
+                        int resid_OW, void* split_ws, size_t split_ws_bytes, int tune_arg, void* stream) {
   const bool want_b3 = tune_arg >= 100000;
   if (want_b3) tune_arg -= 100000;
   const int tune = tune_arg % 10000;
@@ -1358,12 +1378,20 @@
   p.colstats = colstats;
   p.abn = a_bn;
   p.rmask = relu_mask; p.ldm = ldm;
+  p.rbits = rbits; p.ldbits = ldbits;
+  p.rs = resid_stride > 1 ? resid_stride : 1; p.rOH = resid_OH; p.rOW = resid_OW;
   STIL_REQUIRE(!relu_mask || !colstats, "stil_gemm_nt: relu_mask and colstats exclude each other");
+  STIL_REQUIRE(!rbits || (!relu_mask && !colstats), "stil_gemm_nt_ex: rbits excludes relu_mask and colstats");
+  STIL_REQUIRE(!rbits || (N % 8 == 0 && ldbits >= N / 8), "stil_gemm_nt_ex: rbits needs N %% 8 == 0 and ldbits >= N / 8 (N=%d ldbits=%d)", N, ldbits);
+  STIL_REQUIRE(p.rs == 1 || (resid && resid_OH > 0 && resid_OW > 0 && (out_stride <= 1) && (OH - 1) / p.rs + 1 == resid_OH && (OW - 1) / p.rs + 1 == resid_OW),
+               "stil_gemm_nt_ex: a residual row map needs resid, an identity output map and resid_OH x resid_OW = ceil(OH / s) x ceil(OW / s)");
   {
     auto al16 = [](const void* q) { return q == nullptr || ((uintptr_t)q % 16) == 0; };
     p.wide = (N % 4 == 0) && (ldc % 4 == 0) && (!resid || ldr % 4 == 0) && (!relu_mask || ldm % 4 == 0) && al16(relu_mask) && al16(C) && al16(resid) && al16(pre) && al16(bias) && al16(sub) &&
              al16(scale) && al16(scale_var) && al16(shift) && !scalar_epilogue ? 1 : 0;
   }
+  STIL_REQUIRE((!rbits && p.rs == 1) || (p.wide && !want_b3 && (tune % 100 == 0 || tune % 100 == 11)),
+               "stil_gemm_nt_ex: rbits / the residual row map need the 16-byte epilogue on 64x64 tiles (tune %% 100 in {0, 11}, no scalar epilogue)");
   p.bs_y = bs_y; p.bs_stats = bs_stats; p.bstats = bstats; p.ldbs = ldc; p.bs_relu = bs_relu; p.bs_tile0 = bs_tile0;
   STIL_REQUIRE(!bstats || (bs_y && bs_stats && (bs_relu == 0 || bs_relu == 2) && bs_tile0 >= 0 && !colstats && !a_bn && p.wide &&
                            ((uintptr_t)bs_y % 16) == 0 && ((uintptr_t)bs_stats % 16) == 0 && (tune % 100 == 0 || tune % 100 == 11 || tune % 100 == 44)),
@@ -1389,7 +1417,7 @@
   rc = gemm_nt_attr();
   if (rc) return rc;
   if (variant == 11 && p.splits == 1) p.panel = nt_panel(M, N, K);
-  if (!want_b3 && variant == 11 && p.splits == 1 && p.wide && !scalar_epilogue && mode == 0 && (!a_bn || srcC <= 2048) &&
+  if (!want_b3 && variant == 11 && p.splits == 1 && p.wide && !scalar_epilogue && mode == 0 && (!a_bn || srcC <= 2048) && !rbits && p.rs == 1 &&
       nt_big_wanted(M, N, K, plain, vec, srcC, tune) && (long)cdiv(M, 64) * cdiv(N, 64) >= 256) {
     p.panel = (p.panel > 0 && p.panel % 2 == 0 && (N / 128) % (p.panel / 2) == 0) ? p.panel / 2 : 0;
     const dim3 grid_((M / 128) * (N / 128));
@@ -1457,6 +1485,32 @@
 #undef LAUNCH_NT
   STIL_LAUNCH_CHECK();
   return STIL_OK;
+}
+
+extern "C" int stil_gemm_nt(const float* A, const float* W, float* C, int M, int N, int K, int lda, int ldb, int ldc,
+                            int srcH, int srcW, int srcC, int OH, int OW, int KH, int KW, int stride, int pad_y,
+                            int pad_x, int mode, int out_stride, int out_py, int out_px, int out_OH, int out_OW,
+                            const float* bias, const float* sub, const float* scale,
+                            const float* shift, const float* resid, int ldr, float* pre, int act, float alpha,
+                            float* colstats, const float* a_bn, const float* relu_mask, int ldm,
+                            const float* bs_y, const float* bs_stats, float* bstats, int bs_relu, int bs_tile0,
+                            const float* scale_var, float var_eps, void* split_ws, size_t split_ws_bytes, int tune_arg, void* stream) {
+  return gemm_nt_impl(A, W, C, M, N, K, lda, ldb, ldc, srcH, srcW, srcC, OH, OW, KH, KW, stride, pad_y, pad_x, mode, out_stride, out_py, out_px,
+                      out_OH, out_OW, bias, sub, scale, shift, resid, ldr, pre, act, alpha, colstats, a_bn, relu_mask, ldm, bs_y, bs_stats, bstats,
+                      bs_relu, bs_tile0, scale_var, var_eps, nullptr, 0, 1, 0, 0, split_ws, split_ws_bytes, tune_arg, stream);
+}
+extern "C" int stil_gemm_nt_ex(const float* A, const float* W, float* C, int M, int N, int K, int lda, int ldb, int ldc,
+                               int srcH, int srcW, int srcC, int OH, int OW, int KH, int KW, int stride, int pad_y,
+                               int pad_x, int mode, int out_stride, int out_py, int out_px, int out_OH, int out_OW,
+                               const float* bias, const float* sub, const float* scale,
+                               const float* shift, const float* resid, int ldr, float* pre, int act, float alpha,
+                               float* colstats, const float* a_bn, const float* relu_mask, int ldm,
+                               const float* bs_y, const float* bs_stats, float* bstats, int bs_relu, int bs_tile0,
+                               const float* scale_var, float var_eps, const unsigned char* rbits, int ldbits, int resid_stride, int resid_OH,
+                               int resid_OW, void* split_ws, size_t split_ws_bytes, int tune_arg, void* stream) {
+  return gemm_nt_impl(A, W, C, M, N, K, lda, ldb, ldc, srcH, srcW, srcC, OH, OW, KH, KW, stride, pad_y, pad_x, mode, out_stride, out_py, out_px,
+                      out_OH, out_OW, bias, sub, scale, shift, resid, ldr, pre, act, alpha, colstats, a_bn, relu_mask, ldm, bs_y, bs_stats, bstats,
+                      bs_relu, bs_tile0, scale_var, var_eps, rbits, ldbits, resid_stride, resid_OH, resid_OW, split_ws, split_ws_bytes, tune_arg, stream);
 }
 
 static inline int tn_variant(int M, int N, int K, int tune) {
diff --git a/stil_tta_amd/csrc/stil_trunk.h b/stil_tta_amd/csrc/stil_trunk.h
--- /dev/null
+++ b/stil_tta_amd/csrc/stil_trunk.h
@@ -0,0 +1,24 @@
+#pragma once
+#include <stddef.h>
+
+#ifdef __cplusplus
+extern "C" {
+#endif
+
+int stil_bn_train_fwd_tiles_bits(const float* x, const float* tilestats, int tile_rows, const float* gamma, const float* beta,
+                                 float* running_mean, float* running_var, long long* num_batches_tracked,
+                                 const float* resid, const float* resid_stats, float* z, unsigned char* zbits, float* stats, int M, int C,
+                                 int relu, float eps, float momentum, void* workspace, size_t workspace_bytes, void* stream);
+
+int stil_gemm_nt_ex(const float* A, const float* W, float* C, int M, int N, int K, int lda, int ldb, int ldc,
+                    int srcH, int srcW, int srcC, int OH, int OW, int KH, int KW, int stride, int pad_y, int pad_x,
+                    int mode, int out_stride, int out_py, int out_px, int out_OH, int out_OW,
+                    const float* bias, const float* sub, const float* scale, const float* shift, const float* resid,
+                    int ldr, float* pre, int act, float alpha, float* colstats, const float* a_bn, const float* relu_mask, int ldm,
+                    const float* bs_y, const float* bs_stats, float* bstats, int bs_relu, int bs_tile0,
+                    const float* scale_var, float var_eps, const unsigned char* rbits, int ldbits, int resid_stride, int resid_OH,
+                    int resid_OW, void* split_ws, size_t split_ws_bytes, int tune, void* stream);
+
+#ifdef __cplusplus
+}
+#endif
diff --git a/stil_tta_amd/modules.py b/stil_tta_amd/modules.py
--- a/stil_tta_amd/modules.py
+++ b/stil_tta_amd/modules.py
@@ -40,13 +40,13 @@
 
 
 def _conv_bn(x, conv: nn.Conv2d, bn: nn.BatchNorm2d, relu: bool, train: bool, resid=None, stem=None, passthrough=False, defer=False,
-             xstats=None, premask_in=None, premask_out=None, rstats=None, bstat_send=None, bstat_recv=None):
+             xstats=None, premask_in=None, premask_out=None, rstats=None, bstat_send=None, bstat_recv=None, sgrad=None):
     k, stride, pad = conv.kernel_size[0], conv.stride[0], conv.padding[0]
     pipe = _PIPE
     if train:
         out = ops.ConvBnActFn.apply(x, conv.weight, bn.weight, bn.bias, bn.running_mean, bn.running_var,
                                     bn.num_batches_tracked, resid, k, stride, pad, relu, stem, passthrough, defer, xstats,
-                                    premask_in, premask_out, rstats, bstat_send, bstat_recv)
+                                    premask_in, premask_out, rstats, bstat_send, bstat_recv, sgrad)
         if pipe is not None:
             pipe.published()
         return out
@@ -80,10 +80,12 @@
         cout = {} if pm else None
         bin_ = getattr(x, "_stil_bstat", None) if train else None
         b1, b2, b3 = ({}, {}, {}) if train else (None, None, None)
+        sg = {} if (train and self.downsample is not None and self.downsample[0].stride[0] > 1) else None
         if d1:
-            out, identity, st1 = _conv_bn(x, self.conv1, self.bn1, True, train, passthrough=True, defer=True, premask_in=cin, bstat_send=bin_, bstat_recv=b1)
+            out, identity, st1 = _conv_bn(x, self.conv1, self.bn1, True, train, passthrough=True, defer=True, premask_in=cin, bstat_send=bin_, bstat_recv=b1,
+                                          sgrad=sg)
         else:
-            out, identity = _conv_bn(x, self.conv1, self.bn1, True, train, passthrough=True, premask_in=cin, bstat_send=bin_)
+            out, identity = _conv_bn(x, self.conv1, self.bn1, True, train, passthrough=True, premask_in=cin, bstat_send=bin_, sgrad=sg)
         if d2:
             out, st2 = _conv_bn(out, self.conv2, self.bn2, True, train, defer=True, xstats=st1, bstat_send=b1, bstat_recv=b2)
         else:
@@ -91,9 +93,9 @@
         rst = None
         if self.downsample is not None:
             if train and ops.can_defer_bn(self.downsample[0].out_channels):
-                identity, rst = _conv_bn(identity, self.downsample[0], self.downsample[1], False, train, defer=True)
+                identity, rst = _conv_bn(identity, self.downsample[0], self.downsample[1], False, train, defer=True, sgrad=sg)
             else:
-                identity = _conv_bn(identity, self.downsample[0], self.downsample[1], False, train)
+                identity = _conv_bn(identity, self.downsample[0], self.downsample[1], False, train, sgrad=sg)
         Nb, H, W, C = identity.shape
         out = _conv_bn(out, self.conv3, self.bn3, True, train, resid=identity.reshape(Nb * H * W, C), xstats=st2, premask_out=cout, rstats=rst,
                        bstat_send=b2, bstat_recv=b3)
@@ -121,16 +123,18 @@
         cout = {} if pm else None
         bin_ = getattr(x, "_stil_bstat", None) if train else None
         b1, b2 = ({}, {}) if train else (None, None)
+        sg = {} if (train and self.downsample is not None and self.downsample[0].stride[0] > 1) else None
         if train and ops.can_defer_bn(self.conv1.out_channels):
-            out, identity, st1 = _conv_bn(x, self.conv1, self.bn1, True, train, passthrough=True, defer=True, premask_in=cin, bstat_send=bin_, bstat_recv=b1)
+            out, identity, st1 = _conv_bn(x, self.conv1, self.bn1, True, train, passthrough=True, defer=True, premask_in=cin, bstat_send=bin_, bstat_recv=b1,
+                                          sgrad=sg)
         else:
-            out, identity = _conv_bn(x, self.conv1, self.bn1, True, train, passthrough=True, premask_in=cin, bstat_send=bin_)
+            out, identity = _conv_bn(x, self.conv1, self.bn1, True, train, passthrough=True, premask_in=cin, bstat_send=bin_, sgrad=sg)
         rst = None
         if self.downsample is not None:
             if train and ops.can_defer_bn(self.downsample[0].out_channels):
-                identity, rst = _conv_bn(identity, self.downsample[0], self.downsample[1], False, train, defer=True)
+                identity, rst = _conv_bn(identity, self.downsample[0], self.downsample[1], False, train, defer=True, sgrad=sg)
             else:
-                identity = _conv_bn(identity, self.downsample[0], self.downsample[1], False, train)
+                identity = _conv_bn(identity, self.downsample[0], self.downsample[1], False, train, sgrad=sg)
         Nb, H, W, C = identity.shape
         out = _conv_bn(out, self.conv2, self.bn2, True, train, resid=identity.reshape(Nb * H * W, C), xstats=st1, premask_out=cout, rstats=rst,
                        bstat_send=b1, bstat_recv=b2)
diff --git a/stil_tta_amd/ops.py b/stil_tta_amd/ops.py
--- a/stil_tta_amd/ops.py
+++ b/stil_tta_amd/ops.py
@@ -284,6 +284,9 @@
         _POLICY.append((int(_k[1:]), int(_t)))
 _POLICY.sort(reverse=True)
 
+GEMM_NT_FORMS = __import__("collections").Counter()
+DGRAD_ZERO_FILLS = __import__("collections").Counter()
+
 
 def _shape_tune(M, N, K, a_bn, has_tile_stats):
     t = TUNE["gemm"]
@@ -299,7 +302,10 @@
 
 def gemm_nt(A, W, M, N, K, *, lda=None, ldb=None, out=None, ldc=None, geom=None, bias=None, sub=None, scale=None, shift=None,
             resid=None, pre=None, act=0, alpha=1.0, pads=None, outmap=None, out_rows=None, colstats=None, a_bn=None, relu_mask=None,
-            bstats=None, scale_var=None, var_eps=0.0):
+            bstats=None, scale_var=None, var_eps=0.0, relu_bits=None, resid_map=None):
+    GEMM_NT_FORMS["relu_mask" if relu_mask is not None else "relu_bits" if relu_bits is not None else "no_mask",
+                  "resid_map" if resid_map is not None else "resid" if resid is not None else "no_resid",
+                  "outmap" if outmap is not None and outmap[0] != 1 else "identity"] += 1
     if geom is None:
         geom = (1, 1, K, 1, 1, 1, 1, 1, 0, 0)
     pads = (geom[8], geom[8]) if pads is None else pads
@@ -315,7 +321,9 @@
     if L._prof is not None:
         s2 = geom[7] * geom[7] if geom[9] == 1 else 1
         src = (M // (geom[3] * geom[4])) * geom[0] * geom[1] * geom[2]
-        nbytes = 4.0 * (src + N * K + M * N * (1 + (resid is not None) + (pre is not None) + (relu_mask is not None) + (bstats is not None)))
+        rrows = M if resid_map is None else (M // (geom[3] * geom[4])) * resid_map[1] * resid_map[2]
+        nbytes = 4.0 * (src + N * K + M * N * (1 + (pre is not None) + (relu_mask is not None) + (bstats is not None))
+                        + (rrows * N if resid is not None else 0)) + (M * N / 8.0 if relu_bits is not None else 0.0)
         plain = int(geom[5] * geom[6] == 1 and geom[7] == 1 and pads == (0, 0) and geom[9] == 0 and outmap[0] == 1
                     and geom[0] == geom[3] and geom[1] == geom[4])
         cfg = L.gemm_nt_config(_p(A), _p(W), M, N, K, lda, ldb, geom[2], geom[5], geom[6], plain, int(a_bn is not None), tune)
@@ -325,12 +333,18 @@
         swn = L.gemm_nt_split_workspace_bytes(M, N, K, tune)
         if swn:
             sw = _split_ws.get(swn, A.device)
-    L.gemm_nt(_p(A), _p(W), _p(out), M, N, K, lda, ldb, ldc, *geom[:8], pads[0], pads[1], geom[9], *outmap,
-              _p(bias), _p(sub), _p(scale), _p(shift), _p(resid),
-              (ldc if resid is not None else 0), _p(pre), act, float(alpha), _p(colstats), _p(a_bn), _p(relu_mask),
-              (ldc if relu_mask is not None else 0), *((_p(bstats[0]), _p(bstats[1]), _p(bstats[2]), int(bstats[3]), int(bstats[4]))
-                                                       if bstats is not None else (None, None, None, 0, 0)),
-              _p(scale_var), float(var_eps), _p(sw), (sw.numel() if sw is not None else 0), tune, _stream(), meta=meta)
+    head = (_p(A), _p(W), _p(out), M, N, K, lda, ldb, ldc, *geom[:8], pads[0], pads[1], geom[9], *outmap,
+            _p(bias), _p(sub), _p(scale), _p(shift), _p(resid),
+            (ldc if resid is not None else 0), _p(pre), act, float(alpha), _p(colstats), _p(a_bn), _p(relu_mask),
+            (ldc if relu_mask is not None else 0), *((_p(bstats[0]), _p(bstats[1]), _p(bstats[2]), int(bstats[3]), int(bstats[4]))
+                                                     if bstats is not None else (None, None, None, 0, 0)),
+            _p(scale_var), float(var_eps))
+    tail = (_p(sw), (sw.numel() if sw is not None else 0), tune, _stream())
+    if relu_bits is None and resid_map is None:
+        L.gemm_nt(*head, *tail, meta=meta)
+    else:
+        rs, roh, row_ = (1, 0, 0) if resid_map is None else resid_map
+        L.gemm_nt_ex(*head, _p(relu_bits), (relu_bits.shape[1] if relu_bits is not None else 0), int(rs), int(roh), int(row_), *tail, meta=meta)
     return out
 
 
@@ -502,6 +516,12 @@
 _PREMASK = __import__("os").environ.get("STIL_PREMASK", "1") != "0"
 _BN_BWD_EPILOGUE = __import__("os").environ.get("STIL_BN_BWD_EPILOGUE", "1") != "0"
 _LINEAR_RESID = __import__("os").environ.get("STIL_LINEAR_RESID", "1") != "0"
+_TRUNK_BYTES = __import__("os").environ.get("STIL_TRUNK_BYTES", "1") != "0"
+
+
+def _trunk_tune_ok() -> bool:
+    t = TUNE["gemm"]
+    return t < 10000 and t % 100 in (0, 11) and not _POLICY
 
 
 def can_defer_bn(Cout: int) -> bool:
@@ -591,15 +611,19 @@
     return _BnRule("train", src=(rmean, rvar, nbt))
 
 
-def _bn_fwd_call(rule, tiles, y, ts, tile_rows, gamma, beta, resid, rstats, z, stats, M, C, relu):
+def _bn_fwd_call(rule, tiles, y, ts, tile_rows, gamma, beta, resid, rstats, z, stats, M, C, relu, zbits=None):
     L = lib()
     assert tiles or rstats is None
+    assert zbits is None or (tiles and rule.family == "train")
     nb = L.bn_tiles_workspace_bytes(M, C, tile_rows) if tiles else L.bn_workspace_bytes(M, C)
     ws = _ws.get(nb, y.device)
     head = (_p(y), _p(ts), tile_rows, _p(gamma), _p(beta)) if tiles else (_p(y), _p(gamma), _p(beta))
     res = (_p(resid), _p(rstats)) if tiles else (_p(resid),)
     src = tuple(_p(t) for t in rule.src)
     sfx = "_tiles" if tiles else ""
+    if rule.family == "train" and zbits is not None:
+        L.bn_train_fwd_tiles_bits(*head, *src, *res, _p(z), _p(zbits), _p(stats), M, C, 1 if relu else 0, 1e-5, 0.1, _p(ws), nb, _stream())
+        return
     if rule.family == "train":
         getattr(L, "bn_train_fwd" + sfx)(*head, *src, *res, _p(z), _p(stats), M, C, 1 if relu else 0, 1e-5, 0.1, _p(ws), nb, _stream())
         return
@@ -629,7 +653,7 @@
 
     @staticmethod
     def forward(ctx, x, w, gamma, beta, rmean, rvar, nbt, resid, k, stride, pad, relu, stem, passthrough=False, defer=False, xstats=None,
-                premask_in=None, premask_out=None, rstats=None, bstat_send=None, bstat_recv=None):
+                premask_in=None, premask_out=None, rstats=None, bstat_send=None, bstat_recv=None, sgrad=None):
         _chk(x, w, gamma, beta, resid)
         ctx.set_materialize_grads(False)
         assert not defer or resid is None, "a layer with a residual input cannot defer its BatchNorm"
@@ -667,7 +691,12 @@
         z = None if (defer and _trace is None) else torch.empty((M, Cout), dtype=torch.float32, device=dev)
         rule = _bn_rule(rmean, rvar, nbt, Cout, dev)
         rho, delta = rule.rho, rule.delta
-        _bn_fwd_call(rule, fused, y, ts, tile_rows, gamma, beta, resid, rstats, z, stats, M, Cout, relu)
+        zbits = None
+        if (_TRUNK_BYTES and premask_out is not None and relu and resid is not None and not defer and fused and rule.family == "train"
+                and not _bn_frozen and _trace is None and Cout % 8 == 0):
+            zbits = torch.empty((M, Cout // 8), dtype=torch.uint8, device=dev)
+            premask_out["bits"] = zbits
+        _bn_fwd_call(rule, fused, y, ts, tile_rows, gamma, beta, resid, rstats, z, stats, M, Cout, relu, zbits)
         if _trace is not None and relu:
             _trace["relu"][id(gamma)] = z.view(Nb, OH, OW, Cout)
         ctx.save_for_backward(x, w, gamma, beta, y, None if defer else z, stats, xstats, delta)
@@ -677,6 +706,9 @@
         ctx.premask_in = premask_in if (stem is None and stride == 1) else None
         ctx.premask_out = premask_out if (relu and resid is not None and not defer) else None
         ctx.bstat_send = bstat_send if (_BN_BWD_EPILOGUE and stem is None) else None
+        ctx.sgrad = sgrad if (_TRUNK_BYTES and stem is None) else None
+        if ctx.sgrad is not None and passthrough:
+            sgrad["accept"] = stride == 1 and Cin % 4 == 0
         ctx.bstat_recv = None
         if _BN_BWD_EPILOGUE and bstat_recv is not None and Cout % 4 == 0:
             if defer and relu and resid is None:
@@ -735,30 +767,47 @@
             _, H, W_, Cin = x.shape
             if ctx.needs_input_grad[0]:
                 ga = None if gx_alias is None else gx_alias.contiguous().view(Nb * H * W_, Cin)
+                rmap = None
+                sg = ctx.sgrad if ctx.has_alias else None
+                if sg is not None and "g" in sg:
+                    assert ga is None and stride == 1
+                    ga, rmap = sg.pop("g"), sg.pop("map")
                 cell = ctx.premask_in if (ctx.premask_in is not None and xstats is None and Cin % 4 == 0 and stride == 1) else None
                 zmask = x.view(Nb * H * W_, Cin) if cell is not None else None
+                zbits = None
                 if cell is not None:
                     cell["masked"] = True
+                    if _TRUNK_BYTES and cell.get("bits") is not None and Cin % 8 == 0 and _trunk_tune_ok() and (ga is None or ga.data_ptr() % 16 == 0):
+                        zbits = cell["bits"]
                 bs = None
                 sc_ = ctx.bstat_send
                 Min = Nb * H * W_
                 if sc_ is not None and "y" in sc_ and Cin % 4 == 0 and _bstats_tune_ok() and (sc_["mode"] == 2 or (zmask is not None and sc_.get("premask") is cell)) \
                         and (stride == 1 or ga is None) and tuple(sc_["y"].shape) == (Min, Cin) \
-                        and lib().gemm_nt_bstats_ok(None, Cin, Cin, _p(ga), Cin, _p(zmask), Cin, _p(sc_["y"])):
+                        and lib().gemm_nt_bstats_ok(None, Cin, Cin, _p(ga), Cin, _p(None if zbits is not None else zmask), Cin, _p(sc_["y"])):
                     nt_ = _bstat_tiles(Nb, H, W_, k, stride, pad)
                     bs = (sc_["y"], sc_["stats"], torch.empty((2 * nt_, Cin), dtype=torch.float32, device=dev), sc_["mode"], 0)
                 if k == 1 and stride == 1:
                     wd = cached_layout(w, "_stil_wd")
                     if wd is None:
                         wd = transpose(w.reshape(Cout, Cin))
-                    dx = gemm_nt(dy, wd, M, Cin, Cout, resid=ga, relu_mask=zmask, bstats=bs).view(Nb, H, W_, Cin)
+                    dx = gemm_nt(dy, wd, M, Cin, Cout, geom=None if rmap is None else (H, W_, Cout, H, W_, 1, 1, 1, 0, 0), resid=ga,
+                                 relu_mask=None if zbits is not None else zmask, relu_bits=zbits, resid_map=rmap, bstats=bs).view(Nb, H, W_, Cin)
                 elif stride == 1:
                     wd = cached_layout(w, "_stil_wd")
                     if wd is None:
                         wd = torch.empty((Cin, k * k * Cout), dtype=torch.float32, device=dev)
                         lib().conv_weight_layout(_p(w), None, _p(wd), Cout, Cin, k, k, _stream())
                     g2 = (OH, OW, Cout, H, W_, k, k, stride, pad, 1)
-                    dx = gemm_nt(dy, wd, Nb * H * W_, Cin, k * k * Cout, geom=g2, resid=ga, relu_mask=zmask, bstats=bs).view(Nb, H, W_, Cin)
+                    dx = gemm_nt(dy, wd, Nb * H * W_, Cin, k * k * Cout, geom=g2, resid=ga, relu_mask=None if zbits is not None else zmask,
+                                 relu_bits=zbits, resid_map=rmap, bstats=bs).view(Nb, H, W_, Cin)
+                elif (k == 1 and pad == 0 and bs is None and ga is None and not ctx.has_alias and ctx.sgrad is not None and ctx.sgrad.get("accept")
+                      and Cin % 4 == 0 and _trunk_tune_ok()):
+                    wd = cached_layout(w, "_stil_wphase", (0, 0))
+                    if wd is None:
+                        wd = torch.empty((Cin, Cout), dtype=torch.float32, device=dev)
+                        lib().conv_weight_layout_phase(_p(w), _p(wd), Cout, Cin, 1, 1, stride, 0, 0, 1, 1, _stream())
+                    ctx.sgrad["g"], ctx.sgrad["map"] = gemm_nt(dy, wd, M, Cin, Cout), (stride, OH, OW)
                 else:
                     dx = strided_dgrad(dy, w, Nb, H, W_, Cin, OH, OW, Cout, k, stride, pad, bstats=bs)
                     if ga is not None:
@@ -770,7 +819,7 @@
             gw = geom[:9]
             dw = wgrad_param(w, dy, x, M, Cout, k * k * Cin, geom=gw, x_bn=xstats) if want_dw else None
         return (dx, dw, (None if gslot is not None else dgamma), (None if bslot is not None else dbeta), None, None, None,
-                dres, None, None, None, None, None, None, None, None, None, None, None, None, None)
+                dres, None, None, None, None, None, None, None, None, None, None, None, None, None, None)
 
 
 def _bstats_tune_ok() -> bool:
@@ -796,6 +845,8 @@
     dev = dy.device
     all_covered = all(len(range((p_ + pad) % stride, k, stride)) > 0 for p_ in range(stride))
     dx = (torch.empty if all_covered else torch.zeros)((Nb * H * W_, Cin), dtype=torch.float32, device=dev)
+    if not all_covered:
+        DGRAD_ZERO_FILLS[(Nb * H * W_, Cin)] += 1
     tile0 = 0
     for py in range(stride):
         ky0 = (py + pad) % stride
```

Result: no change. 2146 samples/s (-0.1%).
